# big-nacho/patolette

Measured on AMD Instinct MI355X. Metric: Mpixels/sec quantized (256-color ICtCp + KMeans) at 1 GPU; palette ΔE vs ref, higher is better.
Workload: dtype f64

## Files before the change

### patolette_amd/csrc/kmeans.h

```cpp
#pragma once

#include "common.h"
#include "devutil.h"

namespace pamd {

constexpr int kKMeansMaxK = 4096;

struct KmSamples { float *x, *y, *z, *w; };

struct KMeansWork {
    DevBuf<float> sx, sy, sz, sw;
    DevBuf<int> assign;
    DevBuf<float4> sorted;
    DevBuf<unsigned int> table, rowtot, ticket;
    DevBuf<unsigned int> flags;
    DevBuf<unsigned int> rowbase;
    DevBuf<float> hs;
    DevBuf<float> cent, hassign;
    DevBuf<float4> c4;
    DevBuf<int> perm;
    DevBuf<struct DevMT> mt;
    bool mt_seeded = false;
    DevBuf<unsigned char> lut, grid, clist;
    DevBuf<unsigned int> mid;
    DevBuf<unsigned int> bkeys;
    DevBuf<unsigned long long> fsum;
    void reserve(size_t nx, int k);
};

void kmeans_gather(const double *d_planar, size_t N, bool weighted, const int *d_perm, size_t nx, KMeansWork &w, hipStream_t s);
void kmeans_gather_slice(const double *d_planar, size_t n_local, bool weighted, const int *d_perm, size_t nx, size_t begin,
                         KMeansWork &w, hipStream_t s);
struct KmSums { double bound_x, bound_w; };
void kmeans_iterate(KMeansWork &w, size_t nx, int k, bool weighted, int niter, hipStream_t s, size_t expect_longest = 0,
                    const KmSums *sums = nullptr);

}
```

### patolette_amd/csrc/kmeans.hip

```cpp
#include "kmeans.h"

namespace pamd {

typedef __attribute__((address_space(1))) const void gvoid_t;
typedef __attribute__((address_space(3))) void lvoid_t;

template <bool W>
__global__ __launch_bounds__(256) void k_km_gather(const double *__restrict__ planar, size_t N, const int *__restrict__ perm,
                                                   size_t nx, KmSamples s) {
    const size_t stride = (size_t)gridDim.x * blockDim.x;
    for (size_t i = (size_t)blockIdx.x * blockDim.x + threadIdx.x; i < nx; i += stride) {
        size_t p = perm ? (size_t)perm[i] : i;
        s.x[i] = (float)planar[p]; s.y[i] = (float)planar[N + p]; s.z[i] = (float)planar[2 * N + p];
        if constexpr (W) s.w[i] = (float)planar[3 * N + p];
    }
}

template <bool W>
__global__ __launch_bounds__(256) void k_km_gather_slice(const double *__restrict__ planar, size_t n_local, const int *__restrict__ perm,
                                                         size_t nx, size_t begin, KmSamples s) {
    const size_t stride = (size_t)gridDim.x * blockDim.x;
    for (size_t i = (size_t)blockIdx.x * blockDim.x + threadIdx.x; i < nx; i += stride) {
        const size_t g = perm ? (size_t)perm[i] : i;
        const bool mine = g >= begin && g - begin < n_local;
        const size_t p = mine ? g - begin : 0;
        s.x[i] = mine ? (float)planar[p] : 0.0f; s.y[i] = mine ? (float)planar[n_local + p] : 0.0f;
        s.z[i] = mine ? (float)planar[2 * n_local + p] : 0.0f;
        if constexpr (W) s.w[i] = mine ? (float)planar[3 * n_local + p] : 0.0f;
    }
}

__device__ __forceinline__ float4 make_c4(float v0, float v1, float v2) {
    return make_float4(v0, v1, v2, __builtin_fmaf(v2, v2, __builtin_fmaf(v0, v0, v1 * v1)));
}

__device__ __forceinline__ void km_store_c4(float4 *c4, const int k, const int j, const float v0, const float v1, const float v2) {
    const float4 r = make_c4(v0, v1, v2);
    float *q = reinterpret_cast<float *>(c4 + j);
    __hip_atomic_store(q, r.x, __ATOMIC_RELAXED, __HIP_MEMORY_SCOPE_AGENT);
    __hip_atomic_store(q + 1, r.y, __ATOMIC_RELAXED, __HIP_MEMORY_SCOPE_AGENT);
    __hip_atomic_store(q + 2, r.z, __ATOMIC_RELAXED, __HIP_MEMORY_SCOPE_AGENT);
    __hip_atomic_store(q + 3, r.w, __ATOMIC_RELAXED, __HIP_MEMORY_SCOPE_AGENT);
    float *pp = reinterpret_cast<float *>(c4 + k) + 8 * (j >> 1) + (j & 1);
    __hip_atomic_store(pp, r.x, __ATOMIC_RELAXED, __HIP_MEMORY_SCOPE_AGENT);
    __hip_atomic_store(pp + 2, r.y, __ATOMIC_RELAXED, __HIP_MEMORY_SCOPE_AGENT);
    __hip_atomic_store(pp + 4, r.z, __ATOMIC_RELAXED, __HIP_MEMORY_SCOPE_AGENT);
    __hip_atomic_store(pp + 6, r.w, __ATOMIC_RELAXED, __HIP_MEMORY_SCOPE_AGENT);
}
constexpr int kKmFlagWords = 2 + 256;
__global__ void k_km_prep(const float *__restrict__ cent, int k, float4 *c4, unsigned int *flags) {
    int j = blockIdx.x * blockDim.x + threadIdx.x;
    if (j < k) km_store_c4(c4, k, j, cent[3 * j], cent[3 * j + 1], cent[3 * j + 2]);
    if (flags && j < kKmFlagWords) flags[j] = j == 0 ? 0u : 1u;
}

typedef float f4_t __attribute__((ext_vector_type(4)));
typedef const __attribute__((address_space(4))) f4_t *scalar_c4_t;

template <typename TabT>
__device__ __forceinline__ int km_assign_one(const float x0, const float x1, const float x2, const TabT c4, const int k) {
    const float m0 = -2 * x0, m1 = -2 * x1, m2 = -2 * x2;
    const float xn = __builtin_fmaf(x2, x2, __builtin_fmaf(x0, x0, x1 * x1));
    float ld[8]; unsigned li[8];
    int lb[8];
#pragma unroll
    for (int l = 0; l < 8; l++) { ld[l] = 3.402823466e+38F - xn; lb[l] = -l; }
    const int ny_p = (k / 8) * 8;
    for (int j = 0; j < ny_p; j += 8) {
#pragma unroll
        for (int l = 0; l < 8; l++) {
            const auto y = c4[j + l];
            float dp = m0 * y.x;
            dp = __builtin_fmaf(m1, y.y, dp);
            dp = __builtin_fmaf(m2, y.z, dp);
            dp = dp + y.w;
            if (dp < ld[l]) { ld[l] = dp; lb[l] = j; }
        }
    }
#pragma unroll
    for (int l = 0; l < 8; l++) li[l] = (unsigned)(lb[l] + l);
    float cur_d = 3.402823466e+38F; unsigned cur_i = 0xFFFFFFFFu;
#pragma unroll
    for (int l = 0; l < 8; l++) {
        float cand = ld[l] + xn;
        if (cand < 0) cand = 0;
        if (cur_d > cand) { cur_d = cand; cur_i = li[l]; }
        else if (cur_d == cand && cur_i > li[l]) cur_i = li[l];
    }
    for (int j0 = ny_p; j0 < k; j0++) {
        const auto y = c4[j0];
        float dp = __builtin_fmaf(x2, y.z, __builtin_fmaf(x1, y.y, x0 * y.x));
        float d = xn + y.w - 2 * dp;
        if (d < 0) d = 0;
        if (cur_d > d) { cur_d = d; cur_i = (unsigned)j0; }
    }
    return (int)cur_i;
}

__device__ __forceinline__ unsigned long long match_mask(int key, int nbits, unsigned long long valid) {
    unsigned long long m = valid;
    for (int b = 0; b < nbits; b++) {
        const bool bit = (key >> b) & 1;
        unsigned long long bm = __ballot(bit);
        m &= bit ? bm : ~bm;
    }
    return m;
}

template <bool BIG>
__global__ __launch_bounds__(256) void k_km_assign_count(KmSamples s, size_t nx, const float4 *__restrict__ c4, int k, int nbits,
                                                         int chunk_len, int nchunks, int *__restrict__ assign,
                                                         unsigned int *table ) {
    extern __shared__ unsigned int lds_u[];
    const int lane = threadIdx.x & 63, wid = threadIdx.x >> 6;
    unsigned int *cnt = lds_u + 4 * (size_t)k + (size_t)wid * k;
    if constexpr (!BIG) {
        for (int j = lane; j < k; j += 64) cnt[j] = 0u;
        __syncthreads();
    }
    const int chunk = blockIdx.x * 4 + wid;
    if (chunk >= nchunks) return;
    const size_t lo = (size_t)chunk * chunk_len;
    const size_t hi = lo + chunk_len < nx ? lo + chunk_len : nx;
    for (size_t base = lo; base < hi; base += 64) {
        const size_t i = base + lane;
        const bool v = i < hi;
        int a = 0;
        if (v) { a = km_assign_one(s.x[i], s.y[i], s.z[i], (scalar_c4_t)(unsigned long long)c4, k); assign[i] = a; }
        const unsigned long long valid = __ballot(v);
        const unsigned long long m = match_mask(a, nbits, valid);
        if (v && (m & ((1ULL << lane) - 1ULL)) == 0ULL) {
            if constexpr (BIG) (void)atomicAdd(&table[(size_t)a * nchunks + chunk], (unsigned)__popcll(m));
            else cnt[a] += (unsigned)__popcll(m);
        }
    }
    if constexpr (!BIG) for (int j = lane; j < k; j += 64) table[(size_t)j * nchunks + chunk] = cnt[j];
}

__global__ __launch_bounds__(256) void k_km_rowbase(const unsigned int *__restrict__ rowtot, int k, unsigned int *rowbase) {
    __shared__ unsigned int wsum[4];
    const int lane = threadIdx.x & 63, wid = threadIdx.x >> 6;
    const int per = (k + 255) / 256;
    const int j0 = threadIdx.x * per, j1 = (j0 + per < k) ? j0 + per : k;
    unsigned sum = 0;
    for (int j = j0; j < j1; j++) sum += rowtot[j];
    unsigned inc = sum;
#pragma unroll
    for (int o = 1; o < 64; o <<= 1) { unsigned t = __shfl_up(inc, o, 64); if (lane >= o) inc += t; }
    if (lane == 63) wsum[wid] = inc;
    __syncthreads();
    unsigned pre = 0;
    for (int w = 0; w < wid; w++) pre += wsum[w];
    unsigned run = pre + inc - sum;
    for (int j = j0; j < j1; j++) { rowbase[j] = run; run += rowtot[j]; }
}

template <bool W>
__global__ __launch_bounds__(256) void k_km_scatter_big(KmSamples s, const int *__restrict__ assign, size_t nx, int nbits, int chunk_len,
                                                        int nchunks, unsigned int *table, const unsigned int *__restrict__ rowbase,
                                                        float4 *sorted) {
    const int lane = threadIdx.x & 63, wid = threadIdx.x >> 6;
    const int chunk = blockIdx.x * 4 + wid;
    if (chunk >= nchunks) return;
    const size_t lo = (size_t)chunk * chunk_len;
    const size_t hi = lo + chunk_len < nx ? lo + chunk_len : nx;
    const unsigned long long lt = (1ULL << lane) - 1ULL;
    for (size_t base = lo; base < hi; base += 64) {
        const size_t i = base + lane;
        const bool v = i < hi;
        const int a = v ? assign[i] : 0;
        const unsigned long long valid = __ballot(v);
        const unsigned long long m = match_mask(a, nbits, valid);
        const unsigned r = (unsigned)__popcll(m & lt);
        unsigned cur = 0;
        if (v && r == 0) cur = atomicAdd(&table[(size_t)a * nchunks + chunk], (unsigned)__popcll(m));
        const int leader = (v && m) ? __ffsll((long long)m) - 1 : lane;
        cur = (unsigned)__shfl((int)cur, leader, 64);
        if (v) {
            float w = 1.0f;
            if constexpr (W) w = s.w[i];
            sorted[(size_t)rowbase[a] + cur + r] = make_float4(s.x[i], s.y[i], s.z[i], w);
        }
    }
}

__global__ __launch_bounds__(256) void k_km_rowscan(unsigned int *table, int nchunks, unsigned int *rowtot) {
    constexpr int IT = 16;
    __shared__ unsigned int sw[4];
    __shared__ unsigned int carry;
    unsigned int *row = table + (size_t)blockIdx.x * nchunks;
    if (threadIdx.x == 0) carry = 0u;
    __syncthreads();
    const int lane = threadIdx.x & 63, wid = threadIdx.x >> 6;
    for (int c0 = 0; c0 < nchunks; c0 += 256 * IT) {
        const int base = c0 + (int)threadIdx.x * IT;
        unsigned v[IT];
        if (base + IT <= nchunks && (((size_t)blockIdx.x * nchunks + base) & 3) == 0) {
#pragma unroll
            for (int q = 0; q < IT / 4; q++) {
                const uint4 u = *reinterpret_cast<const uint4 *>(row + base + 4 * q);
                v[4 * q] = u.x; v[4 * q + 1] = u.y; v[4 * q + 2] = u.z; v[4 * q + 3] = u.w;
            }
        } else {
#pragma unroll
            for (int q = 0; q < IT; q++) v[q] = base + q < nchunks ? row[base + q] : 0u;
        }
        unsigned tot = 0;
#pragma unroll
        for (int q = 0; q < IT; q++) { const unsigned x = v[q]; v[q] = tot; tot += x; }
        unsigned inc = tot;
#pragma unroll
        for (int o = 1; o < 64; o <<= 1) { unsigned t = __shfl_up(inc, o, 64); if (lane >= o) inc += t; }
        if (lane == 63) sw[wid] = inc;
        __syncthreads();
        unsigned pre = 0;
        for (int w = 0; w < wid; w++) pre += sw[w];
        const unsigned cr = carry;
        const unsigned off = cr + pre + inc - tot;
#pragma unroll
        for (int q = 0; q < IT; q++) if (base + q < nchunks) row[base + q] = off + v[q];
        __syncthreads();
        if (threadIdx.x == 255) carry = cr + pre + inc;
        __syncthreads();
    }
    if (threadIdx.x == 0) rowtot[blockIdx.x] = carry;
}

struct KmGridDev { float lo[3], hi[3]; };

__device__ __forceinline__ unsigned f32_key(float f) {
    const unsigned u = __float_as_uint(f);
    return (u & 0x80000000u) ? ~u : (u | 0x80000000u);
}
__device__ __forceinline__ float key_f32(unsigned k) { return __uint_as_float((k & 0x80000000u) ? (k & 0x7fffffffu) : ~k); }

constexpr int kKmSlots = 32;
__global__ __launch_bounds__(256) void k_km_bounds(KmSamples s, size_t nx, unsigned int *keys ) {
    float mn[3] = {INFINITY, INFINITY, INFINITY}, mx[3] = {-INFINITY, -INFINITY, -INFINITY};
    const size_t stride = (size_t)gridDim.x * blockDim.x;
    for (size_t i = (size_t)blockIdx.x * blockDim.x + threadIdx.x; i < nx; i += stride) {
        const float v[3] = {s.x[i], s.y[i], s.z[i]};
#pragma unroll
        for (int a = 0; a < 3; a++) { mn[a] = fminf(mn[a], v[a]); mx[a] = fmaxf(mx[a], v[a]); }
    }
#pragma unroll
    for (int a = 0; a < 3; a++) {
        float lo = mn[a], hi = mx[a];
#pragma unroll
        for (int o = 32; o > 0; o >>= 1) { lo = fminf(lo, __shfl_down(lo, o, 64)); hi = fmaxf(hi, __shfl_down(hi, o, 64)); }
        if ((threadIdx.x & 63) == 0 && lo <= hi) {
            unsigned int *k6 = keys + (blockIdx.x & (kKmSlots - 1)) * 6;
            atomicMin(&k6[a], f32_key(lo)); atomicMax(&k6[3 + a], f32_key(hi));
        }
    }
}
__global__ void k_km_bounds_init(unsigned int *keys) {
    const int t = threadIdx.x;
    if (t < kKmSlots * 6) keys[t] = (t % 6) < 3 ? 0xFFFFFFFFu : 0u;
}
__global__ void k_km_bounds_fold(const unsigned int *keys, KmGridDev *g) {
    const int a = threadIdx.x;
    if (a >= 3) return;
    unsigned lo = 0xFFFFFFFFu, hi = 0u;
    for (int sl = 0; sl < kKmSlots; sl++) { lo = min(lo, keys[sl * 6 + a]); hi = max(hi, keys[sl * 6 + 3 + a]); }
    g->lo[a] = key_f32(lo); g->hi[a] = key_f32(hi);
}

__device__ __forceinline__ int km_cell(float x0, float x1, float x2, const KmGridDev &g, int G) {
    int idx[3];
    const float v[3] = {x0, x1, x2};
#pragma unroll
    for (int a = 0; a < 3; a++) {
        const double r = (double)g.hi[a] - (double)g.lo[a];
        const double inv = r > 0 ? (double)G / r : 0.0;
        int q = (int)(((double)v[a] - (double)g.lo[a]) * inv);
        idx[a] = q < 0 ? 0 : (q >= G ? G - 1 : q);
    }
    return (idx[2] * G + idx[1]) * G + idx[0];
}

struct KmBox { double cl[3], ch[3], cellnorm2; };
__device__ __forceinline__ KmBox km_box(const KmGridDev &g, int G, const int idx[3], int span) {
    KmBox b; b.cellnorm2 = 0;
#pragma unroll
    for (int a = 0; a < 3; a++) {
        const double r = (double)g.hi[a] - (double)g.lo[a], cw = r / G, m = 1e-5 * r + 1e-30;
        b.cl[a] = (double)g.lo[a] + idx[a] * cw - m;
        b.ch[a] = (double)g.lo[a] + (idx[a] + span) * cw + m;
        const double f = fmax(fabs(b.cl[a]), fabs(b.ch[a]));
        b.cellnorm2 += f * f;
    }
    return b;
}
__device__ __forceinline__ double km_maxd2(const KmBox &b, const float4 y) {
    const double p[3] = {(double)y.x, (double)y.y, (double)y.z};
    double mx = 0;
#pragma unroll
    for (int a = 0; a < 3; a++) { const double d = fmax(fabs(p[a] - b.cl[a]), fabs(p[a] - b.ch[a])); mx += d * d; }
    return mx;
}
__device__ __forceinline__ double km_mind2(const KmBox &b, const float4 y) {
    const double p[3] = {(double)y.x, (double)y.y, (double)y.z};
    double mn = 0;
#pragma unroll
    for (int a = 0; a < 3; a++) { const double d = fmax(fmax(b.cl[a] - p[a], p[a] - b.ch[a]), 0.0); mn += d * d; }
    return mn;
}
__device__ __forceinline__ double km_threshold(const KmBox &b, double U, double cn2) {
    const double rr = sqrt(b.cellnorm2) + sqrt(cn2);
    return U * (1.0 + 1e-12) + 4.0 * (16.0 * 0x1.0p-24) * rr * rr + 1e-300;
}

constexpr int kKmCoarseMax = 96;
__global__ __launch_bounds__(64) void k_km_lut_coarse(const float4 *__restrict__ c4, int k, const KmGridDev *__restrict__ gp, int G,
                                                      unsigned char *__restrict__ clist ,
                                                      double *__restrict__ cn2_out ) {
    const KmGridDev g = *gp;
    const int Gc = G / 4, cell = (int)blockIdx.x, lane = (int)threadIdx.x;
    const int idx[3] = {4 * (cell % Gc), 4 * ((cell / Gc) % Gc), 4 * (cell / (Gc * Gc))};
    const KmBox b = km_box(g, G, idx, 4);
    double U = INFINITY, cn2 = 0;
    for (int j = lane; j < k; j += 64) {
        const float4 y = c4[j];
        U = fmin(U, km_maxd2(b, y));
        cn2 = fmax(cn2, ((double)y.x * y.x + (double)y.y * y.y) + (double)y.z * y.z);
    }
#pragma unroll
    for (int o = 32; o > 0; o >>= 1) { U = fmin(U, __shfl_xor(U, o, 64)); cn2 = fmax(cn2, __shfl_xor(cn2, o, 64)); }
    const double thr = km_threshold(b, U, cn2);
    if (lane == 0) *cn2_out = cn2;
    unsigned char *out = clist + (size_t)cell * (2 + kKmCoarseMax);
    int cnt = 0;
    const int ny_p = (k / 8) * 8;
    auto sweep = [&](int j, bool valid) {
        const bool keep = valid && km_mind2(b, c4[valid ? j : 0]) <= thr;
        const unsigned long long m = __ballot(keep);
        const int pos = cnt + (int)__popcll(m & ((1ULL << lane) - 1ULL));
        if (keep && pos < kKmCoarseMax) out[2 + pos] = (unsigned char)j;
        cnt += (int)__popcll(m);
    };
    for (int l = 0; l < 8; l++)
        for (int q0 = 0; l + 8 * q0 < ny_p; q0 += 64) { const int j = l + 8 * (q0 + lane); sweep(j, j < ny_p); }
    for (int j0 = ny_p; j0 < k; j0 += 64) sweep(j0 + lane, j0 + lane < k);
    if (lane == 0) { out[0] = (unsigned char)(cnt <= kKmCoarseMax ? cnt : 0); out[1] = (unsigned char)(cnt <= kKmCoarseMax ? 0 : 1); }
}

constexpr int kKmMidSurv = 48;
constexpr unsigned kKmMidOverflow = 0x00000001u;
__device__ __forceinline__ bool km_mid_is_overflow(unsigned e) { return e == kKmMidOverflow; }

__device__ __forceinline__ void km_mid_entries(const float4 *__restrict__ c4, const int k, const KmGridDev &g, const int G,
                                               const unsigned char *__restrict__ cand, const double cn2, const int c0, const int c1, const int c2,
                                               unsigned int *__restrict__ mid) {
    const int lane = (int)threadIdx.x, m = lane >> 3, sl = lane & 7;
    const int midx[3] = {2 * c0 + (m & 1), 2 * c1 + ((m >> 1) & 1), 2 * c2 + (m >> 2)};
    const int idx[3] = {2 * midx[0], 2 * midx[1], 2 * midx[2]};
// ... 931 lines not shown
            for (int q = 0; 4 * q < cnt; q++) {
                const float4 x = s4[q];
                float4 w = make_float4(0, 0, 0, 0);
                if (wx) w = w4[q];
                const float xs[4] = {x.x, x.y, x.z, x.w}, ws[4] = {w.x, w.y, w.z, w.w};
#pragma unroll
                for (int e = 0; e < 4; e++) {
                    if (4 * q + e < cnt) {
                        if (wx) acc = __builtin_fmaf(xs[e], ws[e], acc);
                        else acc += xs[e];
                    }
                }
            }
        }
    }
}
__device__ __forceinline__ void km_block_step(const float *blk, const float *wblk, const bool wx, const unsigned len, float &acc, const int lane) {
    if (km_block_exact(blk, wblk, wx, 0, 4, acc, lane)) return;
    if (len == 1024u) {
        for (int q = 0; q < 4; q++)
            if (!km_block_exact(blk, wblk, wx, q, 1, acc, lane)) km_block_replay(blk, wblk, wx, (unsigned)q * 256u, (unsigned)(q + 1) * 256u, acc);
        return;
    }
    km_block_replay(blk, wblk, wx, 0u, len, acc);
}

template <bool W>
__device__ __forceinline__ float km_chain_coop(const float4 *__restrict__ sorted, size_t lo, size_t hi, float *coop, int lane, int wid) {
    constexpr int K = 16;
    constexpr size_t BS = (size_t)64 * K, SS = 4 * BS;
    const bool wx = W && wid < 3;
    const bool chain = W || wid < 3;
    const float *mine = coop + (size_t)wid * SS, *wts = coop + 3 * SS;
    float acc = 0.f;
    float4 reg[K];
    auto fetch = [&](const size_t p0) {
#pragma unroll
        for (int j = 0; j < K; j++) {
            const size_t i = p0 + (size_t)wid * BS + (size_t)j * 64 + lane;
            reg[j] = make_float4(0, 0, 0, 0);
            if (i < hi) reg[j] = sorted[i];
        }
    };
    fetch(lo);
    for (size_t p0 = lo; p0 < hi; p0 += SS) {
#pragma unroll
        for (int j = 0; j < K; j++) {
            const int o = wid * (int)BS + j * 64 + lane;
            coop[o] = reg[j].x; coop[SS + o] = reg[j].y; coop[2 * SS + o] = reg[j].z; coop[3 * SS + o] = reg[j].w;
        }
        if (p0 + SS < hi) fetch(p0 + SS);
        __syncthreads();
        if (chain) {
            for (int d = 0; d < 4; d++) {
                const size_t pos = p0 + (size_t)d * BS;
                if (pos >= hi) break;
                const size_t bend = pos + BS < hi ? pos + BS : hi;
                const float *blk = mine + d * (int)BS, *wblk = wts + d * (int)BS;
                km_block_step(blk, wblk, wx, (unsigned)(bend - pos), acc, lane);
            }
        }
        __syncthreads();
    }
    return acc;
}

template <bool W>
__device__ __forceinline__ float km_coop_lds(const float *mine, const float *wts, const unsigned n, const bool wx, float acc, const int lane) {
    constexpr unsigned BS = 1024;
    for (unsigned pos = 0; pos < n; pos += BS)
        km_block_step(mine + pos, wts + pos, wx, pos + BS < n ? BS : n - pos, acc, lane);
    return acc;
}

template <bool W, int HS>
__device__ __forceinline__ void km_update_finish(const int kidx, const int k, const unsigned long long nx, const size_t cnt, const float *res,
                                                 int *s_last, float *cent, float *hassign, float4 *c4, unsigned int *ticket, DevMT *mt,
                                                 float *hs_mem = nullptr, unsigned int *flags = nullptr, const bool clean = false) {
    const int lane = threadIdx.x & 63, wid = threadIdx.x >> 6;
    float c0 = res[0], c1 = res[1], c2 = res[2], h = res[3];
    if constexpr (!W) {
        h = cnt < (size_t)16777216 ? (float)cnt : 16777216.0f;
    }
    if (threadIdx.x == 0) {
        if (!clean) {
        if (h != 0.f) { const float norm = 1 / h; c0 *= norm; c1 *= norm; c2 *= norm; }
        __hip_atomic_store(&cent[3 * kidx], c0, __ATOMIC_RELAXED, __HIP_MEMORY_SCOPE_AGENT);
        __hip_atomic_store(&cent[3 * kidx + 1], c1, __ATOMIC_RELAXED, __HIP_MEMORY_SCOPE_AGENT);
        __hip_atomic_store(&cent[3 * kidx + 2], c2, __ATOMIC_RELAXED, __HIP_MEMORY_SCOPE_AGENT);
        __hip_atomic_store(&hassign[kidx], h, __ATOMIC_RELAXED, __HIP_MEMORY_SCOPE_AGENT);
        km_store_c4(c4, k, kidx, c0, c1, c2);
        }
        asm volatile("s_waitcnt vmcnt(0)" ::: "memory");
        const unsigned tk = __hip_atomic_fetch_add(ticket, 1u, __ATOMIC_RELAXED, __HIP_MEMORY_SCOPE_AGENT);
        *s_last = (tk == (unsigned)k - 1u) ? 1 : 0;
    }
    __syncthreads();
    if (!*s_last || wid != 0) return;
    bool mine_empty = false, mine_dirty = false;
    for (int cb = 0; cb < k; cb += 256) {
        float hv[4]; unsigned fv[4];
#pragma unroll
        for (int q = 0; q < 4; q++) {
            const int ci = cb + 64 * q + lane;
            hv[q] = 1.f; fv[q] = 0u;
            if (ci < k) {
                hv[q] = __hip_atomic_load(&hassign[ci], __ATOMIC_RELAXED, __HIP_MEMORY_SCOPE_AGENT);
                if (flags) fv[q] = __hip_atomic_load(&flags[1 + ci], __ATOMIC_RELAXED, __HIP_MEMORY_SCOPE_AGENT);
            }
        }
#pragma unroll
        for (int q = 0; q < 4; q++) {
            const int ci = cb + 64 * q + lane;
            mine_empty = mine_empty || hv[q] == 0.f;
            mine_dirty = mine_dirty || fv[q] != 0u;
            if (flags && ci < k) __hip_atomic_store(&flags[1 + ci], 0u, __ATOMIC_RELAXED, __HIP_MEMORY_SCOPE_AGENT);
        }
    }
    const bool any = __ballot(mine_empty) != 0ULL;
    if (lane == 0) __hip_atomic_store(ticket, 0u, __ATOMIC_RELAXED, __HIP_MEMORY_SCOPE_AGENT);
    if (flags) {
        const bool any_dirty = __ballot(mine_dirty) != 0ULL;
        if (!any_dirty && !any && lane == 0) __hip_atomic_store(&flags[0], 1u, __ATOMIC_RELAXED, __HIP_MEMORY_SCOPE_AGENT);
    }
    if (!any) return;
    {
        asm volatile("s_waitcnt vmcnt(0)" ::: "memory");
        __shared__ unsigned s_mt[624];
        __builtin_amdgcn_fence(__ATOMIC_ACQUIRE, "agent");
        if constexpr (HS > 0) {
            __shared__ float s_hs[HS];
            km_split_clusters_wave<false>(cent, hassign, k, nx, mt, s_mt, s_hs, lane, flags);
        } else km_split_clusters_wave<true>(cent, hassign, k, nx, mt, s_mt, hs_mem, lane);
        __builtin_amdgcn_fence(__ATOMIC_RELEASE, "agent");
        asm volatile("s_waitcnt vmcnt(0)" ::: "memory");
    }
    for (int j = lane; j < k; j += 64) {
        const float v0 = __hip_atomic_load(&cent[3 * j], __ATOMIC_RELAXED, __HIP_MEMORY_SCOPE_AGENT);
        const float v1 = __hip_atomic_load(&cent[3 * j + 1], __ATOMIC_RELAXED, __HIP_MEMORY_SCOPE_AGENT);
        const float v2 = __hip_atomic_load(&cent[3 * j + 2], __ATOMIC_RELAXED, __HIP_MEMORY_SCOPE_AGENT);
        km_store_c4(c4, k, j, v0, v1, v2);
    }
}

template <bool W, bool BIGK = false>
__global__ __launch_bounds__(256) void k_km_update(const float4 *__restrict__ sorted, const unsigned int *__restrict__ rowtot, int k,
                                                  unsigned long long nx, float *cent, float *hassign, float4 *c4,
                                                  unsigned int *ticket, DevMT *mt, unsigned long long long_min, float *hs_mem) {
    __shared__ float4 stage[4][2][64];
    extern __shared__ __attribute__((aligned(16))) float coop[];
    __shared__ float res[4];
    __shared__ int s_last;
    const int kidx = blockIdx.x, lane = threadIdx.x & 63, wid = threadIdx.x >> 6;
    unsigned pre = 0;
    for (int j = lane; j < kidx; j += 64) pre += rowtot[j];
    pre = wave_sum_u32(pre);
    pre = __shfl(pre, 0, 64);
    const size_t lo = pre, hi = lo + rowtot[kidx];
    float acc = 0.f;
    if ((size_t)(hi - lo) >= long_min) {
        acc = km_chain_coop<W>(sorted, lo, hi, coop, lane, wid);
    } else {
        if (wid == 0) acc = km_chain<W, 0>(sorted, lo, hi, stage[0], lane);
        else if (wid == 1) acc = km_chain<W, 1>(sorted, lo, hi, stage[1], lane);
        else if (wid == 2) acc = km_chain<W, 2>(sorted, lo, hi, stage[2], lane);
        else if (W) acc = km_chain<W, 3>(sorted, lo, hi, stage[3], lane);
    }
    if (lane == 0) res[wid] = acc;
    __syncthreads();
    km_update_finish<W, BIGK ? 0 : kKMeansMaxK>(kidx, k, nx, hi - lo, res, &s_last, cent, hassign, c4, ticket, mt, hs_mem);
}

constexpr int kKmDirectCap = 4096;
constexpr int kKmSortBlock = 1024;

__device__ __forceinline__ unsigned block_scan_incl_u32(const unsigned v, unsigned *wsum, unsigned *total) {
    const int lane = threadIdx.x & 63, wid = threadIdx.x >> 6, nw = (int)(blockDim.x >> 6);
    const unsigned inc = wave_scan_incl_u32(v);
    __syncthreads();
    if (lane == 63) wsum[wid] = inc;
    __syncthreads();
    unsigned pre = 0, all = 0;
    for (int w = 0; w < nw; w++) { const unsigned t = wsum[w]; all += t; pre += w < wid ? t : 0u; }
    *total = all;
    return pre + inc;
}

typedef float f2_t __attribute__((ext_vector_type(2)));
typedef float f8_t __attribute__((ext_vector_type(8)));
typedef const __attribute__((address_space(4))) f8_t *scalar_c8_t;

__device__ __forceinline__ float km_min3(const float a, const float b, const float c) {
    float r;
    asm("v_min3_f32 %0, %1, %2, %3" : "=v"(r) : "v"(a), "v"(b), "v"(c));
    return r;
}
__device__ __forceinline__ int km_assign_min3(const float x0, const float x1, const float x2, const scalar_c4_t c4,
                                              const scalar_c8_t c8, const float4 *c4s, const int k) {
    const f2_t m0 = {-2 * x0, -2 * x0}, m1 = {-2 * x1, -2 * x1}, m2 = {-2 * x2, -2 * x2};
    const float xn = __builtin_fmaf(x2, x2, __builtin_fmaf(x0, x0, x1 * x1));
    float ld[8]; int lc[8];
#pragma unroll
    for (int l = 0; l < 8; l++) { ld[l] = 3.402823466e+38F - xn; lc[l] = -1; }
    const int ny_p = (k / 8) * 8;
    const int U = ny_p >> 4;
    const int CUN = (U + 3) >> 2;
    auto pair_dp = [&](const f8_t y) {
        const f2_t y0 = {y[0], y[1]}, y1 = {y[2], y[3]}, y2 = {y[4], y[5]}, yw = {y[6], y[7]};
        f2_t dp = m0 * y0;
        dp = __builtin_elementwise_fma(m1, y1, dp);
        dp = __builtin_elementwise_fma(m2, y2, dp);
        return dp + yw;
    };
    for (int c = 0; c < 4; c++) {
        const int u0 = c * CUN, u1 = u0 + CUN < U ? u0 + CUN : U;
        if (u0 >= u1) break;
        float snap[8];
#pragma unroll
        for (int l = 0; l < 8; l++) snap[l] = ld[l];
        for (int u = u0; u < u1; u++) {
            const int p0 = u << 3;
            typedef float f16_t __attribute__((ext_vector_type(16)));
            typedef const __attribute__((address_space(4))) f16_t *scalar_c16_t;
            const scalar_c16_t c16 = (scalar_c16_t)c8;
            const f16_t q0 = c16[p0 >> 1], q1 = c16[(p0 >> 1) + 1], q2 = c16[(p0 >> 1) + 2], q3 = c16[(p0 >> 1) + 3];
            auto half = [](const f16_t q, const int h) { return h ? f8_t{q[8], q[9], q[10], q[11], q[12], q[13], q[14], q[15]} : f8_t{q[0], q[1], q[2], q[3], q[4], q[5], q[6], q[7]}; };
#pragma unroll
            for (int l = 0; l < 8; l += 2) {
                const f8_t ya = half(l < 4 ? q0 : q1, (l >> 1) & 1), yb = half(l < 4 ? q2 : q3, (l >> 1) & 1);
                const f2_t a = pair_dp(ya), b = pair_dp(yb);
                ld[l] = km_min3(ld[l], a[0], b[0]);
                ld[l + 1] = km_min3(ld[l + 1], a[1], b[1]);
            }
        }
#pragma unroll
        for (int l = 0; l < 8; l++) lc[l] = ld[l] < snap[l] ? c : lc[l];
    }
    if (ny_p & 8) {
        const int p0 = U << 3;
#pragma unroll
        for (int l = 0; l < 8; l += 2) {
            const f2_t a = pair_dp(c8[p0 + (l >> 1)]);
            if (a[0] < ld[l]) { ld[l] = a[0]; lc[l] = 4; }
            if (a[1] < ld[l + 1]) { ld[l + 1] = a[1]; lc[l + 1] = 4; }
        }
    }
    float cand[8];
    float cur_d = 3.402823466e+38F;
#pragma unroll
    for (int l = 0; l < 8; l++) { float cd = ld[l] + xn; if (cd < 0) cd = 0; cand[l] = cd; cur_d = cd < cur_d ? cd : cur_d; }
    unsigned tm = 0u;
#pragma unroll
    for (int l = 0; l < 8; l++) tm |= cand[l] == cur_d ? (1u << l) : 0u;
    unsigned cur_i = 0xFFFFFFFFu;
    while (__any(tm != 0u)) {
        if (tm) {
            const int l = __ffs((int)tm) - 1;
            tm &= tm - 1u;
            float target = ld[0]; int c = lc[0];
#pragma unroll
            for (int q = 1; q < 8; q++) { target = l == q ? ld[q] : target; c = l == q ? lc[q] : c; }
            unsigned idx = 0u;
            if (c == 4) idx = (unsigned)((U << 4) + l);
            else if (c >= 0) {
                const int u0 = c * CUN, u1 = u0 + CUN < U ? u0 + CUN : U;
                const int base = (u0 << 4) + l, lim = u1 << 4;
                for (int q = 2 * CUN - 1; q >= 0; q--) {
                    const int j = base + 8 * q;
                    if (j < lim) {
                        const float4 y = c4s[j];
                        float dp = (-2 * x0) * y.x;
                        dp = __builtin_fmaf(-2 * x1, y.y, dp);
                        dp = __builtin_fmaf(-2 * x2, y.z, dp);
                        dp = dp + y.w;
                        if (dp == target) idx = (unsigned)j;
                    }
                }
            }
            cur_i = idx < cur_i ? idx : cur_i;
        }
    }
    for (int j0 = ny_p; j0 < k; j0++) {
        const auto y = c4[j0];
        float dp = __builtin_fmaf(x2, y.z, __builtin_fmaf(x1, y.y, x0 * y.x));
        float d = xn + y.w - 2 * dp;
        if (d < 0) d = 0;
        if (cur_d > d) { cur_d = d; cur_i = (unsigned)j0; }
    }
    return cur_i < (unsigned)k ? (int)cur_i : 0;
}

#ifdef PAMD_KM_TRACE
__device__ unsigned long long g_km_trace[2][256][32];
#define KM_TRACE(kern, slot) do { if ((threadIdx.x & 63) == 0) g_km_trace[kern][blockIdx.x & 255][slot] = wall_clock64(); } while (0)
#define KM_TRACE0(kern, slot) do { if (threadIdx.x == 0) g_km_trace[kern][blockIdx.x & 255][slot] = wall_clock64(); } while (0)
#else
#define KM_TRACE(kern, slot) do { } while (0)
#define KM_TRACE0(kern, slot) do { } while (0)
#endif

__global__ __launch_bounds__(1024) void k_km_assign_sort(KmSamples s, size_t nx, const float4 *__restrict__ c4, int k, const bool weighted,
                                                         float4 *__restrict__ sorted_rec, unsigned short *__restrict__ offs,
                                                         unsigned char *__restrict__ prev, unsigned int *flags) {
    if (flags[0]) return;
    __shared__ unsigned char cnt[16][256];
    __shared__ unsigned short stepbase[16][256];
    __shared__ unsigned int wsum[16];
    __shared__ float4 c4s[256];
    const int lane = threadIdx.x & 63, step = threadIdx.x >> 6;
    KM_TRACE0(0, 0);
    for (int i = threadIdx.x; i < 16 * 256 / 4; i += 1024) reinterpret_cast<unsigned int *>(&cnt[0][0])[i] = 0u;
    if ((int)threadIdx.x < k) c4s[threadIdx.x] = c4[threadIdx.x];
    __syncthreads();
    KM_TRACE0(0, 1);
    const scalar_c4_t t4 = (scalar_c4_t)(unsigned long long)c4;
    const scalar_c8_t t8 = (scalar_c8_t)(unsigned long long)(c4 + k);
    const size_t blk0 = (size_t)blockIdx.x * kKmSortBlock;
    const size_t i = blk0 + (size_t)step * 64 + lane;
    const bool v = i < nx;
    float4 rec = make_float4(0.f, 0.f, 0.f, 0.f);
    if (v) { rec.x = s.x[i]; rec.y = s.y[i]; rec.z = s.z[i]; if (weighted) rec.w = s.w[i]; }
#ifdef PAMD_KM_TRACE
    asm volatile("s_waitcnt vmcnt(0)" ::: "memory");
    KM_TRACE0(0, 2);
    if (threadIdx.x == 0) g_km_trace[0][blockIdx.x & 255][24] = clock64();
#endif
    int a = km_assign_min3(rec.x, rec.y, rec.z, t4, t8, c4s, k);
    if (!v) a = 0;
    if (v) {
        const int old = prev[i];
        if (old != a) { prev[i] = (unsigned char)a; flags[1 + old] = 1u; flags[1 + a] = 1u; }
    }
    const unsigned long long m = match_mask(a, 8, __ballot(v));
    const unsigned rk = (unsigned)__popcll(m & ((1ULL << lane) - 1ULL));
    if (v && rk == 0u) cnt[step][a] = (unsigned char)__popcll(m);
#ifdef PAMD_KM_TRACE
    if (lane == 0) g_km_trace[0][blockIdx.x & 255][8 + step] = wall_clock64();
    if (threadIdx.x == 0) g_km_trace[0][blockIdx.x & 255][25] = clock64();
#endif
    __syncthreads();
    KM_TRACE0(0, 3);
    unsigned tot = 0;
    unsigned short pre[16];
    if (threadIdx.x < 256) {
#pragma unroll
        for (int st = 0; st < 16; st++) { pre[st] = (unsigned short)tot; tot += cnt[st][threadIdx.x]; }
    }
    unsigned total = 0;
    const unsigned start = block_scan_incl_u32(tot, wsum, &total) - tot;
    if (threadIdx.x < 256) {
#pragma unroll
        for (int st = 0; st < 16; st++) stepbase[st][threadIdx.x] = (unsigned short)(start + pre[st]);
        unsigned short *ob = offs + (size_t)blockIdx.x * 257;
        ob[threadIdx.x] = (unsigned short)start;
        if (threadIdx.x == 255) ob[256] = (unsigned short)total;
    }
    __syncthreads();
    KM_TRACE0(0, 4);
    if (v) sorted_rec[blk0 + (unsigned)stepbase[step][a] + rk] = rec;
#ifdef PAMD_KM_TRACE
    asm volatile("s_waitcnt vmcnt(0)" ::: "memory");
    KM_TRACE0(0, 5);
#endif
}

template <bool W>
__global__ __launch_bounds__(256) void k_km_update_lists(const float4 *__restrict__ sorted_rec, const unsigned short *__restrict__ offs,
                                                        unsigned long long nx, int k, float *cent, float *hassign, float4 *c4,
                                                        unsigned int *ticket, DevMT *mt, unsigned int *flags) {
    if (flags[0]) return;
    __shared__ float4 stage[4][2][64];
    extern __shared__ __attribute__((aligned(16))) float members[];
    __shared__ float res[4];
    __shared__ int s_last;
    __shared__ unsigned int wsum[16];
    __shared__ unsigned int n_long, long_src[256], long_lo[256], long_nb[256];
    const int kidx = blockIdx.x, lane = threadIdx.x & 63, wid = threadIdx.x >> 6;
    float *const mx = members, *const my = members + kKmDirectCap, *const mz = members + 2 * kKmDirectCap, *const mw = members + 3 * kKmDirectCap;
    unsigned int *const srcidx = reinterpret_cast<unsigned int *>(members + 4 * kKmDirectCap);
    float acc = 0.f;
    size_t total = 0;
    unsigned fill = 0;
    KM_TRACE0(1, 0);
    bool long_list = false;
    auto replay = [&]() {
        const unsigned n = fill;
        if (n == (unsigned)kKmDirectCap || long_list) {
            const unsigned padded = (n + 1023u) & ~1023u;
            for (unsigned i = n + threadIdx.x; i < padded; i += 256) { mx[i] = 0.f; my[i] = 0.f; mz[i] = 0.f; mw[i] = 0.f; }
            __syncthreads();
            if ((W || wid < 3) && n) acc = km_coop_lds<W>(members + (size_t)wid * kKmDirectCap, mw, n, W && wid < 3, acc, lane);
            long_list = true;
            return;
        }
        auto rec = [&](const size_t i) { return make_float4(mx[i], my[i], mz[i], mw[i]); };
        if (wid == 0) acc = km_chain_over<W, 0>(rec, n, stage[0], lane, acc);
        else if (wid == 1) acc = km_chain_over<W, 1>(rec, n, stage[1], lane, acc);
        else if (wid == 2) acc = km_chain_over<W, 2>(rec, n, stage[2], lane, acc);
        else if (W) acc = km_chain_over<W, 3>(rec, n, stage[3], lane, acc);
    };
    const bool clean = flags[1 + kidx] == 0u;
    const unsigned long long nblocks = clean ? 0ULL : (nx + kKmSortBlock - 1) / kKmSortBlock;
    for (unsigned long long c0 = 0; c0 < nblocks; c0 += 256) {
        const unsigned long long b = c0 + threadIdx.x;
        unsigned o0 = 0, nb = 0;
        if (b < nblocks) { o0 = offs[b * 257 + kidx]; nb = (unsigned)offs[b * 257 + kidx + 1] - o0; }
        unsigned chunk_total = 0;
        const unsigned excl = block_scan_incl_u32(nb, wsum, &chunk_total) - nb;
        constexpr unsigned kLongRun = 32;
        const bool is_long = nb > kLongRun;
        if (threadIdx.x == 0) n_long = 0u;
        __syncthreads();
        if (is_long) { const unsigned e = atomicAdd(&n_long, 1u); long_src[e] = (unsigned)(b * kKmSortBlock) + o0; long_lo[e] = excl; long_nb[e] = nb; }
        __syncthreads();
        const unsigned nl = n_long;
        unsigned done = 0;
        while (done < chunk_total) {
            const unsigned take = min((unsigned)kKmDirectCap - fill, chunk_total - done);
            if (!is_long) {
                const unsigned lo = max(excl, done), hi = min(excl + nb, done + take);
                const float4 *src = sorted_rec + b * kKmSortBlock + o0;
                for (unsigned q = lo; q < hi; q += 4) {
                    float4 r4[4];
#pragma unroll
                    for (int u = 0; u < 4; u++) r4[u] = q + u < hi ? src[q + u - excl] : make_float4(0.f, 0.f, 0.f, 0.f);
#pragma unroll
                    for (int u = 0; u < 4; u++) if (q + u < hi) { const unsigned i = fill + q + u - done; mx[i] = r4[u].x; my[i] = r4[u].y; mz[i] = r4[u].z; mw[i] = r4[u].w; }
                }
            }
            if (nl) {
                for (unsigned i = threadIdx.x; i < take; i += 256) srcidx[fill + i] = ~0u;
                __syncthreads();
                for (unsigned e = 0; e < nl; e++) {
                    const unsigned ex0 = long_lo[e], lo = max(ex0, done), hi = min(ex0 + long_nb[e], done + take);
                    for (unsigned q = lo + threadIdx.x; q < hi; q += 256) srcidx[fill + q - done] = long_src[e] + (q - ex0);
                }
                __syncthreads();
                for (unsigned i0 = threadIdx.x; i0 < take; i0 += 256 * 8) {
                    unsigned ix[8]; float4 r[8];
#pragma unroll
                    for (int u = 0; u < 8; u++) { const unsigned i = i0 + 256u * u; ix[u] = i < take ? srcidx[fill + i] : ~0u; }
#pragma unroll
                    for (int u = 0; u < 8; u++) r[u] = ix[u] != ~0u ? sorted_rec[ix[u]] : make_float4(0.f, 0.f, 0.f, 0.f);
#pragma unroll
                    for (int u = 0; u < 8; u++) if (ix[u] != ~0u) { const unsigned i = fill + i0 + 256u * u; mx[i] = r[u].x; my[i] = r[u].y; mz[i] = r[u].z; mw[i] = r[u].w; }
                }
            }
            fill += take; done += take;
            __syncthreads();
            if (fill == (unsigned)kKmDirectCap) { replay(); fill = 0; __syncthreads(); }
        }
        total += chunk_total;
    }
    __syncthreads();
    KM_TRACE0(1, 1);
    replay();
#ifdef PAMD_KM_TRACE
    if (lane == 0) g_km_trace[1][blockIdx.x & 255][8 + wid] = wall_clock64();
#endif
    if (lane == 0) res[wid] = acc;
    __syncthreads();
    KM_TRACE0(1, 2);
    km_update_finish<W, 256>(kidx, k, nx, total, res, &s_last, cent, hassign, c4, ticket, mt, nullptr, flags, clean);
    KM_TRACE0(1, 3);
}

struct KmFix { double magic_x, quantum_x, magic_w, quantum_w; };
__device__ __forceinline__ long long km_fix_quant(const double v, const double magic) {
    return __double_as_longlong(v + magic) - __double_as_longlong(magic);
}
template <bool W, typename AT>
__global__ __launch_bounds__(256) void k_km_accum(KmSamples s, const AT *__restrict__ assign, size_t nx, int k, KmFix f,
                                                  unsigned long long *gsum ) {
    extern __shared__ unsigned long long acc64[];
    for (int i = threadIdx.x; i < 4 * k; i += 256) acc64[i] = 0ULL;
    __syncthreads();
    auto add = [&](const unsigned a, const float x, const float y, const float z, const float w) {
        const double wd = W ? (double)w : 1.0;
        unsigned long long *r = acc64 + 4 * (size_t)a;
        atomicAdd(r, (unsigned long long)km_fix_quant((double)x * wd, f.magic_x));
        atomicAdd(r + 1, (unsigned long long)km_fix_quant((double)y * wd, f.magic_x));
        atomicAdd(r + 2, (unsigned long long)km_fix_quant((double)z * wd, f.magic_x));
        atomicAdd(r + 3, W ? (unsigned long long)km_fix_quant(wd, f.magic_w) : 1ULL);
    };
    const size_t stride = (size_t)gridDim.x * 1024;
    for (size_t base = ((size_t)blockIdx.x * 256 + threadIdx.x) * 4; base < nx; base += stride) {
        if (base + 4 <= nx) {
            const float4 vx = *reinterpret_cast<const float4 *>(s.x + base), vy = *reinterpret_cast<const float4 *>(s.y + base),
                         vz = *reinterpret_cast<const float4 *>(s.z + base);
            float4 vw = make_float4(1.f, 1.f, 1.f, 1.f);
            if constexpr (W) vw = *reinterpret_cast<const float4 *>(s.w + base);
            unsigned a0, a1, a2, a3;
            if constexpr (sizeof(AT) == 1) {
                const unsigned pk = *reinterpret_cast<const unsigned int *>(assign + base);
                a0 = pk & 0xffu; a1 = (pk >> 8) & 0xffu; a2 = (pk >> 16) & 0xffu; a3 = pk >> 24;
            } else {
                const int4 pk = *reinterpret_cast<const int4 *>(assign + base);
                a0 = (unsigned)pk.x; a1 = (unsigned)pk.y; a2 = (unsigned)pk.z; a3 = (unsigned)pk.w;
            }
            add(a0, vx.x, vy.x, vz.x, vw.x); add(a1, vx.y, vy.y, vz.y, vw.y);
            add(a2, vx.z, vy.z, vz.z, vw.z); add(a3, vx.w, vy.w, vz.w, vw.w);
        } else {
            for (size_t i = base; i < nx; i++) add((unsigned)assign[i], s.x[i], s.y[i], s.z[i], W ? s.w[i] : 1.f);
        }
    }
    __syncthreads();
    for (int i = threadIdx.x; i < 4 * k; i += 256) { const unsigned long long v = acc64[i]; if (v) atomicAdd(&gsum[i], v); }
}

template <bool W>
__global__ __launch_bounds__(256) void k_km_update_sums(unsigned long long *gsum, int k, unsigned long long nx, KmFix f, float *cent,
                                                        float *hassign, float4 *c4, DevMT *mt) {
    __shared__ int s_empty;
    if (threadIdx.x == 0) s_empty = 0;
    __syncthreads();
    for (int j = threadIdx.x; j < k; j += 256) {
        const double sx = (double)(long long)gsum[4 * j] * f.quantum_x, sy = (double)(long long)gsum[4 * j + 1] * f.quantum_x,
                     sz = (double)(long long)gsum[4 * j + 2] * f.quantum_x;
        float h;
        if constexpr (W) h = (float)((double)(long long)gsum[4 * j + 3] * f.quantum_w);
        else h = (float)gsum[4 * j + 3];
        float c0 = (float)sx, c1 = (float)sy, c2 = (float)sz;
        if (h != 0.f) { const float norm = 1 / h; c0 *= norm; c1 *= norm; c2 *= norm; }
        else s_empty = 1;
        cent[3 * j] = c0; cent[3 * j + 1] = c1; cent[3 * j + 2] = c2; hassign[j] = h;
        gsum[4 * j] = 0ULL; gsum[4 * j + 1] = 0ULL; gsum[4 * j + 2] = 0ULL; gsum[4 * j + 3] = 0ULL;
    }
    __threadfence();
    __syncthreads();
    if (s_empty && threadIdx.x < 64) {
        __shared__ unsigned s_mt[624];
        __shared__ float s_hs[kKMeansMaxK];
        km_split_clusters_wave(cent, hassign, k, nx, mt, s_mt, s_hs, (int)threadIdx.x);
        __threadfence();
    }
    __syncthreads();
    for (int j = threadIdx.x; j < k; j += 256) km_store_c4(c4, k, j, cent[3 * j], cent[3 * j + 1], cent[3 * j + 2]);
}

static int chunk_len_for(size_t nx) {
    size_t c = ceil_div(nx, 4096);
    c = ceil_div(c, 64) * 64;
    if (c < 64) c = 64;
    return (int)c;
}

void KMeansWork::reserve(size_t nx, int k) {
    sx.reserve(nx); sy.reserve(nx); sz.reserve(nx); sw.reserve(nx);
    assign.reserve(nx); sorted.reserve(nx);
    const int nchunks = (int)ceil_div(nx, (size_t)chunk_len_for(nx));
    table.reserve(std::max((size_t)k * (size_t)(nchunks > 0 ? nchunks : 1),
                           (ceil_div(nx, (size_t)1024) * 257 + 1) / 2 + 1));
    rowtot.reserve(k);
    if (k > kKMeansMaxK) { rowbase.reserve(k); hs.reserve(k); }
    cent.reserve(3 * (size_t)k); hassign.reserve(k); c4.reserve(2 * (size_t)k + 2);
    perm.reserve(nx);
    if (!mt.p) { mt.reserve(1); mt_seeded = false; }
    if (!ticket.p) { ticket.reserve(1); HIP_CHECK(hipMemset(ticket.p, 0, sizeof(unsigned int))); }
    flags.reserve(2 + 256);
}

void kmeans_gather(const double *d_planar, size_t N, bool weighted, const int *d_perm, size_t nx, KMeansWork &w, hipStream_t s) {
    KmSamples ks{w.sx.p, w.sy.p, w.sz.p, w.sw.p};
    size_t g = ceil_div(nx, 256);
    if (g > 4096) g = 4096;
    if (g < 1) g = 1;
    KTIME("k_km_gather", s, (weighted ? 48.0 : 36.0) * nx);
    if (weighted) hipLaunchKernelGGL(k_km_gather<true>, (int)g, 256, 0, s, d_planar, N, d_perm, nx, ks);
    else hipLaunchKernelGGL(k_km_gather<false>, (int)g, 256, 0, s, d_planar, N, d_perm, nx, ks);
    HIP_CHECK(hipGetLastError());
}

void kmeans_gather_slice(const double *d_planar, size_t n_local, bool weighted, const int *d_perm, size_t nx, size_t begin,
                         KMeansWork &w, hipStream_t s) {
    KmSamples ks{w.sx.p, w.sy.p, w.sz.p, w.sw.p};
    size_t g = ceil_div(nx, 256);
    if (g > 4096) g = 4096;
    if (g < 1) g = 1;
    KTIME("k_km_gather", s, (weighted ? 48.0 : 36.0) * nx);
    if (weighted) hipLaunchKernelGGL(k_km_gather_slice<true>, (int)g, 256, 0, s, d_planar, n_local, d_perm, nx, begin, ks);
    else hipLaunchKernelGGL(k_km_gather_slice<false>, (int)g, 256, 0, s, d_planar, n_local, d_perm, nx, begin, ks);
    HIP_CHECK(hipGetLastError());
}

void kmeans_iterate(KMeansWork &w, size_t nx, int k, bool weighted, int niter, hipStream_t s, size_t expect_longest, const KmSums *sums) {
    KmSamples ks{w.sx.p, w.sy.p, w.sz.p, w.sw.p};
    KmFix fix{};
    int ablocks = 1;
    if (sums && k > kKMeansMaxK) sums = nullptr;
    if (sums) {
        int ex = 0, ew = 0, P = 1;
        (void)frexp(std::max(sums->bound_x, 1e-300) * (weighted ? std::max(sums->bound_w, 1e-300) : 1.0), &ex);
        (void)frexp(std::max(sums->bound_w, 1e-300), &ew);
        while (((size_t)1 << P) < nx) P++;
        P = std::max(P + 1, 12);
        fix.quantum_x = ldexp(1.0, ex + P - 62); fix.magic_x = ldexp(1.5, 52 + ex + P - 62);
        fix.quantum_w = ldexp(1.0, ew + P - 62); fix.magic_w = ldexp(1.5, 52 + ew + P - 62);
        w.fsum.reserve(4 * (size_t)k);
        HIP_CHECK(hipMemsetAsync(w.fsum.p, 0, 4 * (size_t)k * sizeof(unsigned long long), s));
        ablocks = (int)std::min<size_t>(std::max<size_t>(ceil_div(nx, (size_t)4096), 1), 2048);
        static PerDeviceOnce attr5;
        attr5.once([&] {
            HIP_CHECK(hipFuncSetAttribute((const void *)k_km_accum<true, int>, hipFuncAttributeMaxDynamicSharedMemorySize, 32 * kKMeansMaxK));
            HIP_CHECK(hipFuncSetAttribute((const void *)k_km_accum<false, int>, hipFuncAttributeMaxDynamicSharedMemorySize, 32 * kKMeansMaxK));
            HIP_CHECK(hipFuncSetAttribute((const void *)k_km_accum<true, unsigned char>, hipFuncAttributeMaxDynamicSharedMemorySize, 32 * kKMeansMaxK));
            HIP_CHECK(hipFuncSetAttribute((const void *)k_km_accum<false, unsigned char>, hipFuncAttributeMaxDynamicSharedMemorySize, 32 * kKMeansMaxK));
        });
    }
    auto update_sums = [&](const bool a8) {
        {
            KTIME("k_km_accum", s, ((weighted ? 16.0 : 12.0) + (a8 ? 1.0 : 4.0)) * nx);
            const size_t lds = (size_t)32 * k;
            if (a8) {
                if (weighted) hipLaunchKernelGGL((k_km_accum<true, unsigned char>), ablocks, 256, lds, s, ks, (const unsigned char *)w.assign.p, nx, k, fix, w.fsum.p);
                else hipLaunchKernelGGL((k_km_accum<false, unsigned char>), ablocks, 256, lds, s, ks, (const unsigned char *)w.assign.p, nx, k, fix, w.fsum.p);
            } else {
                if (weighted) hipLaunchKernelGGL((k_km_accum<true, int>), ablocks, 256, lds, s, ks, (const int *)w.assign.p, nx, k, fix, w.fsum.p);
                else hipLaunchKernelGGL((k_km_accum<false, int>), ablocks, 256, lds, s, ks, (const int *)w.assign.p, nx, k, fix, w.fsum.p);
            }
        }
        KTIME("k_km_update", s, 32.0 * k);
        if (weighted) hipLaunchKernelGGL(k_km_update_sums<true>, 1, 256, 0, s, w.fsum.p, k, (unsigned long long)nx, fix, w.cent.p, w.hassign.p, w.c4.p, w.mt.p);
        else hipLaunchKernelGGL(k_km_update_sums<false>, 1, 256, 0, s, w.fsum.p, k, (unsigned long long)nx, fix, w.cent.p, w.hassign.p, w.c4.p, w.mt.p);
    };
    int nbits = 0;
    while ((1 << nbits) < k) nbits++;
    const int chunk_len = chunk_len_for(nx);
    const int nchunks = (int)ceil_div(nx, (size_t)chunk_len);
    const int cblocks = (nchunks + 3) / 4;
    const bool bigk = k > kKMeansMaxK;
    const size_t lds_cnt = bigk ? 0 : (size_t)8 * k * sizeof(unsigned int);
    const size_t lds_sct = (size_t)5 * k * sizeof(unsigned int);
    const size_t lds_sct_pair = (size_t)9 * k * sizeof(unsigned int) + (size_t)4 * (k + 64) * sizeof(float4);
    static PerDeviceOnce attr;
    attr.once([&] {
        HIP_CHECK(hipFuncSetAttribute((const void *)k_km_assign_count<false>, hipFuncAttributeMaxDynamicSharedMemorySize, 8 * kKMeansMaxK * 4));
        HIP_CHECK(hipFuncSetAttribute((const void *)k_km_scatter<true, int>, hipFuncAttributeMaxDynamicSharedMemorySize, 5 * kKMeansMaxK * 4));
        HIP_CHECK(hipFuncSetAttribute((const void *)k_km_scatter<false, int>, hipFuncAttributeMaxDynamicSharedMemorySize, 5 * kKMeansMaxK * 4));
        HIP_CHECK(hipFuncSetAttribute((const void *)k_km_scatter<true, unsigned char>, hipFuncAttributeMaxDynamicSharedMemorySize, 5 * kKMeansMaxK * 4));
        HIP_CHECK(hipFuncSetAttribute((const void *)k_km_scatter<false, unsigned char>, hipFuncAttributeMaxDynamicSharedMemorySize, 5 * kKMeansMaxK * 4));
        HIP_CHECK(hipFuncSetAttribute((const void *)k_km_update<true, false>, hipFuncAttributeMaxDynamicSharedMemorySize, 4 * 4096 * 4));
        HIP_CHECK(hipFuncSetAttribute((const void *)k_km_update<false, false>, hipFuncAttributeMaxDynamicSharedMemorySize, 4 * 4096 * 4));
    });
    if (!w.mt_seeded) { hipLaunchKernelGGL(k_km_mt_seed, 1, 1, 0, s, w.mt.p); w.mt_seeded = true; }
    { KTIME("k_km_prep", s, 28.0 * k); hipLaunchKernelGGL(k_km_prep, (std::max(k, kKmFlagWords) + 255) / 256, 256, 0, s, w.cent.p, k, w.c4.p, w.flags.p); }
    const size_t lut_min = getenv("PAMD_KM_LUT_MIN") ? (size_t)atoll(getenv("PAMD_KM_LUT_MIN")) : ((size_t)1 << 21);
    const bool use_lut = nx >= lut_min && k >= 16 && k <= 256;
    const size_t g64_min = getenv("PAMD_KM_G64_MIN") ? (size_t)atoll(getenv("PAMD_KM_G64_MIN")) : ((size_t)1 << 23);
    const int G = nx >= g64_min ? 64 : 32;
    if (use_lut) {
        static PerDeviceOnce attr2;
        attr2.once([&] {
            HIP_CHECK(hipFuncSetAttribute((const void *)k_km_assign_lut, hipFuncAttributeMaxDynamicSharedMemorySize, 8 * kKMeansMaxK * 4));
        });
        w.lut.reserve((size_t)G * G * G * 16); w.bkeys.reserve(kKmSlots * 6); w.grid.reserve(64 + sizeof(double));
        w.clist.reserve((size_t)(G * G * G / 64) * (2 + kKmCoarseMax));
        hipLaunchKernelGGL(k_km_bounds_init, 1, 256, 0, s, w.bkeys.p);
        { KTIME("k_km_bounds", s, 12.0 * nx); hipLaunchKernelGGL(k_km_bounds, (int)std::min<size_t>(ceil_div(nx, 256), 2048), 256, 0, s, ks, nx, w.bkeys.p); }
        hipLaunchKernelGGL(k_km_bounds_fold, 1, 64, 0, s, w.bkeys.p, (KmGridDev *)w.grid.p);
    }
    constexpr size_t direct_max = (size_t)1 << 19;
    const size_t list_longest = getenv("PAMD_KM_LIST_LONGEST") ? (size_t)atoll(getenv("PAMD_KM_LIST_LONGEST")) : (size_t)16384;
    const bool use_direct = !sums && !use_lut && k <= 256 && nx <= direct_max && nx < ((size_t)1 << 32) && expect_longest < list_longest;
    if (use_direct) {
        HIP_CHECK(hipMemsetAsync(w.assign.p, 0, nx, s));
        static PerDeviceOnce attr4;
        attr4.once([&] {
            HIP_CHECK(hipFuncSetAttribute((const void *)k_km_update_lists<true>, hipFuncAttributeMaxDynamicSharedMemorySize, kKmDirectCap * 20));
            HIP_CHECK(hipFuncSetAttribute((const void *)k_km_update_lists<false>, hipFuncAttributeMaxDynamicSharedMemorySize, kKmDirectCap * 20));
        });
    }
    const bool use_mid = use_lut && G == 64 && k % 8 == 0;
    if (use_mid) w.mid.reserve(32 * 32 * 32);
    const unsigned long long long_min = getenv("PAMD_KM_LONG_MIN") ? (unsigned long long)atoll(getenv("PAMD_KM_LONG_MIN")) : 8192ULL;
    for (int it = 0; it < niter; it++) {
        if (use_direct) {
            unsigned short *offs = (unsigned short *)w.table.p;
            const int sblocks = (int)ceil_div(nx, (size_t)kKmSortBlock);
            {
                KTIME("k_km_assign", s, (weighted ? 32.0 : 28.0) * nx);
                hipLaunchKernelGGL(k_km_assign_sort, sblocks, 1024, 0, s, ks, nx, w.c4.p, k, weighted, w.sorted.p, offs, (unsigned char *)w.assign.p, w.flags.p);
            }
            {
                KTIME("k_km_update", s, 16.0 * nx);
                if (weighted) hipLaunchKernelGGL(k_km_update_lists<true>, k, 256, kKmDirectCap * 20, s, (const float4 *)w.sorted.p, (const unsigned short *)offs,
                                                 (unsigned long long)nx, k, w.cent.p, w.hassign.p, w.c4.p, w.ticket.p, w.mt.p, w.flags.p);
                else hipLaunchKernelGGL(k_km_update_lists<false>, k, 256, kKmDirectCap * 20, s, (const float4 *)w.sorted.p, (const unsigned short *)offs,
                                        (unsigned long long)nx, k, w.cent.p, w.hassign.p, w.c4.p, w.ticket.p, w.mt.p, w.flags.p);
            }
            continue;
        }
        if (use_lut) {
            {
                KTIME("k_km_lut_build", s, 16.0 * G * G * G);
                const int ncoarse = G * G * G / 64;
                double *cn2 = (double *)(w.grid.p + 64);
                hipLaunchKernelGGL(k_km_lut_coarse, ncoarse, 64, 0, s, w.c4.p, k, (const KmGridDev *)w.grid.p, G, w.clist.p, cn2);
                hipLaunchKernelGGL(k_km_lut_build, ncoarse, 64, 0, s, w.c4.p, k, (const KmGridDev *)w.grid.p, G, (const unsigned char *)w.clist.p,
                                   (const double *)cn2, w.lut.p, use_mid ? w.mid.p : (unsigned int *)nullptr);
            }
            if (use_mid) {
                const int nmid = 32 * 32 * 32;
                const size_t lds_mid = ((size_t)nmid + 4 * 256 + 16 * 256) * 4 + (size_t)16 * kKmQueue * 16;
                static PerDeviceOnce attr3;
                attr3.once([&] {
                    HIP_CHECK(hipFuncSetAttribute((const void *)k_km_assign_mid, hipFuncAttributeMaxDynamicSharedMemorySize, (int)lds_mid));
                });
                const int mblocks = std::min(num_cus(), (nchunks + 15) / 16);
                KTIME("k_km_assign", s, 16.0 * nx);
                hipLaunchKernelGGL(k_km_assign_mid, mblocks, 1024, lds_mid, s, ks, nx, w.c4.p, k, chunk_len, nchunks, (unsigned char *)w.assign.p, w.table.p,
                                   (const KmGridDev *)w.grid.p, (const unsigned int *)w.mid.p, (const unsigned char *)w.lut.p);
            } else {
            KTIME("k_km_assign", s, 16.0 * nx);
            hipLaunchKernelGGL(k_km_assign_lut, cblocks, 256, lds_cnt, s, ks, nx, w.c4.p, k, nbits, chunk_len, nchunks, w.assign.p, w.table.p,
                               (const KmGridDev *)w.grid.p, G, w.lut.p);
            }
        } else {
            KTIME("k_km_assign", s, 16.0 * nx);
            if (bigk) {
                HIP_CHECK(hipMemsetAsync(w.table.p, 0, (size_t)k * nchunks * sizeof(unsigned int), s));
                hipLaunchKernelGGL(k_km_assign_count<true>, cblocks, 256, 0, s, ks, nx, w.c4.p, k, nbits, chunk_len, nchunks, w.assign.p, w.table.p);
            } else hipLaunchKernelGGL(k_km_assign_count<false>, cblocks, 256, lds_cnt, s, ks, nx, w.c4.p, k, nbits, chunk_len, nchunks, w.assign.p, w.table.p);
        }
        if (sums) { update_sums(use_lut && use_mid); continue; }
        if (bigk) {
            { KTIME("k_km_rowscan", s, 8.0 * k * nchunks); hipLaunchKernelGGL(k_km_rowscan, k, 256, 0, s, w.table.p, nchunks, w.rowtot.p); }
            hipLaunchKernelGGL(k_km_rowbase, 1, 256, 0, s, (const unsigned int *)w.rowtot.p, k, w.rowbase.p);
            {
                KTIME("k_km_scatter", s, (weighted ? 36.0 : 32.0) * nx);
                if (weighted) hipLaunchKernelGGL(k_km_scatter_big<true>, cblocks, 256, 0, s, ks, (const int *)w.assign.p, nx, nbits, chunk_len, nchunks, w.table.p, (const unsigned int *)w.rowbase.p, w.sorted.p);
                else hipLaunchKernelGGL(k_km_scatter_big<false>, cblocks, 256, 0, s, ks, (const int *)w.assign.p, nx, nbits, chunk_len, nchunks, w.table.p, (const unsigned int *)w.rowbase.p, w.sorted.p);
            }
            {
                KTIME("k_km_update", s, 16.0 * nx);
                const bool coop_on = nx >= long_min;
                const size_t lds_up = coop_on ? (size_t)4 * 4096 * sizeof(float) : 0;
                const unsigned long long lm = coop_on ? long_min : ~0ULL;
                static PerDeviceOnce attr6;
                attr6.once([&] {
                    HIP_CHECK(hipFuncSetAttribute((const void *)k_km_update<true, true>, hipFuncAttributeMaxDynamicSharedMemorySize, 4 * 4096 * 4));
                    HIP_CHECK(hipFuncSetAttribute((const void *)k_km_update<false, true>, hipFuncAttributeMaxDynamicSharedMemorySize, 4 * 4096 * 4));
                });
                if (weighted) hipLaunchKernelGGL((k_km_update<true, true>), k, 256, lds_up, s, w.sorted.p, w.rowtot.p, k, (unsigned long long)nx, w.cent.p, w.hassign.p, w.c4.p, w.ticket.p, w.mt.p, lm, w.hs.p);
                else hipLaunchKernelGGL((k_km_update<false, true>), k, 256, lds_up, s, w.sorted.p, w.rowtot.p, k, (unsigned long long)nx, w.cent.p, w.hassign.p, w.c4.p, w.ticket.p, w.mt.p, lm, w.hs.p);
            }
            continue;
        }
        { KTIME("k_km_rowscan", s, 8.0 * k * nchunks); hipLaunchKernelGGL(k_km_rowscan, k, 256, 0, s, w.table.p, nchunks, w.rowtot.p); }
        {
            KTIME("k_km_scatter", s, (weighted ? 36.0 : 32.0) * nx - (use_mid ? 3.0 : 0.0) * nx);
            const unsigned char *a8 = (const unsigned char *)w.assign.p;
            if (use_mid && chunk_len >= 4096 && k <= 256) {
                constexpr size_t lds_ls = (size_t)(512 + 1024 + 4096 / 4 + 4 * 4096) * sizeof(unsigned int);
                static PerDeviceOnce attr5;
                attr5.once([&] {
                    HIP_CHECK(hipFuncSetAttribute((const void *)k_km_scatter_lds<true>, hipFuncAttributeMaxDynamicSharedMemorySize, (int)lds_ls));
                    HIP_CHECK(hipFuncSetAttribute((const void *)k_km_scatter_lds<false>, hipFuncAttributeMaxDynamicSharedMemorySize, (int)lds_ls));
                });
                if (weighted) hipLaunchKernelGGL(k_km_scatter_lds<true>, nchunks, 256, lds_ls, s, ks, a8, nx, k, chunk_len, nchunks, w.table.p, w.rowtot.p, w.sorted.p);
                else hipLaunchKernelGGL(k_km_scatter_lds<false>, nchunks, 256, lds_ls, s, ks, a8, nx, k, chunk_len, nchunks, w.table.p, w.rowtot.p, w.sorted.p);
            } else if (use_mid && chunk_len >= 2 * k) {
                static PerDeviceOnce attr3;
                attr3.once([&] {
                    HIP_CHECK(hipFuncSetAttribute((const void *)k_km_scatter<true, unsigned char, true>, hipFuncAttributeMaxDynamicSharedMemorySize, 9 * 256 * 4 + 4 * (256 + 64) * 16));
                    HIP_CHECK(hipFuncSetAttribute((const void *)k_km_scatter<false, unsigned char, true>, hipFuncAttributeMaxDynamicSharedMemorySize, 9 * 256 * 4 + 4 * (256 + 64) * 16));
                });
                if (weighted) hipLaunchKernelGGL((k_km_scatter<true, unsigned char, true>), cblocks, 256, lds_sct_pair, s, ks, a8, nx, k, nbits, chunk_len, nchunks, w.table.p, w.rowtot.p, w.sorted.p);
                else hipLaunchKernelGGL((k_km_scatter<false, unsigned char, true>), cblocks, 256, lds_sct_pair, s, ks, a8, nx, k, nbits, chunk_len, nchunks, w.table.p, w.rowtot.p, w.sorted.p);
            } else if (use_mid) {
                if (weighted) hipLaunchKernelGGL((k_km_scatter<true, unsigned char>), cblocks, 256, lds_sct, s, ks, a8, nx, k, nbits, chunk_len, nchunks, w.table.p, w.rowtot.p, w.sorted.p);
                else hipLaunchKernelGGL((k_km_scatter<false, unsigned char>), cblocks, 256, lds_sct, s, ks, a8, nx, k, nbits, chunk_len, nchunks, w.table.p, w.rowtot.p, w.sorted.p);
            } else {
                if (weighted) hipLaunchKernelGGL((k_km_scatter<true, int>), cblocks, 256, lds_sct, s, ks, (const int *)w.assign.p, nx, k, nbits, chunk_len, nchunks, w.table.p, w.rowtot.p, w.sorted.p);
                else hipLaunchKernelGGL((k_km_scatter<false, int>), cblocks, 256, lds_sct, s, ks, (const int *)w.assign.p, nx, k, nbits, chunk_len, nchunks, w.table.p, w.rowtot.p, w.sorted.p);
            }
        }
        {
            KTIME("k_km_update", s, 16.0 * nx);
            const bool coop_on = nx >= long_min;
            const size_t lds_up = coop_on ? (size_t)4 * 4096 * sizeof(float) : 0;
            const unsigned long long lm = coop_on ? long_min : ~0ULL;
            if (weighted) hipLaunchKernelGGL((k_km_update<true, false>), k, 256, lds_up, s, w.sorted.p, w.rowtot.p, k, (unsigned long long)nx, w.cent.p, w.hassign.p, w.c4.p, w.ticket.p, w.mt.p, lm, (float *)nullptr);
            else hipLaunchKernelGGL((k_km_update<false, false>), k, 256, lds_up, s, w.sorted.p, w.rowtot.p, k, (unsigned long long)nx, w.cent.p, w.hassign.p, w.c4.p, w.ticket.p, w.mt.p, lm, (float *)nullptr);
        }
    }
    HIP_CHECK(hipGetLastError());
}

}

#ifdef PAMD_KM_TRACE
extern "C" int patolette_amd_debug_km_trace(unsigned long long *out) {
    return hipMemcpyFromSymbol(out, HIP_SYMBOL(pamd::g_km_trace), sizeof(pamd::g_km_trace)) == hipSuccess ? 0 : -1;
}
#endif
```

### patolette_amd/csrc/pipeline.hip

```cpp
#include <algorithm>
#include <functional>
#include <chrono>
#include <cmath>
#include <atomic>
#include <memory>
#include <mutex>
#include <thread>
#include <future>
#include <type_traits>

#include "color_device.h"
#include "common.h"
#include "host_math.h"
#include "kmeans.h"
#include "map.h"
#include "ordered.h"
#include "delta.h"
#include "measure.h"
#include "lzw.h"
#include "saliency.h"
#include "quant.h"
#include "rgba.h"
#include "compact.h"
#include "split_frontier.h"
#include "given.h"

namespace pamd {

void launch_convert(int which, const double *src, double *dst, size_t n, ConvertStats *stats, hipStream_t s, BinK sumk = BinK{0.0, 0.0},
                    BinK momk = BinK{0.0, 0.0}, size_t begin = 0, size_t end = ~(size_t)0, bool init_stats = true);
void launch_convert_rows(int which, const double *rows, double *dst, size_t n, ConvertStats *stats, hipStream_t s,
                         BinK sumk = BinK{0.0, 0.0}, BinK momk = BinK{0.0, 0.0}, size_t begin = 0, size_t end = ~(size_t)0,
                         bool init_stats = true);
void launch_convert_u8(int which, const unsigned char *pixels, int channels, double *dst, size_t n, ConvertStats *stats,
                       hipStream_t s, BinK sumk = BinK{0.0, 0.0}, BinK momk = BinK{0.0, 0.0}, size_t begin = 0, size_t end = ~(size_t)0,
                       bool init_stats = true);
void launch_reconstruct(const void *map, int map_elem, size_t n, const unsigned char *pal_u8, int k, unsigned char *out,
                        hipStream_t s);
void launch_weight_stats(const double *w, size_t n, ConvertStats *stats, hipStream_t s);
void launch_pow(const double *x, double y, double *out, size_t n, hipStream_t s);
void launch_fill_image(double *d, size_t n, uint64_t seed, hipStream_t s);
void launch_fill_weights(double *d, size_t n, uint64_t seed, hipStream_t s);

KernelTimer &ktimer() { static thread_local KernelTimer *t = new KernelTimer; return *t; }

std::atomic<int> g_debug_ws{getenv("PAMD_DEBUG_WORKSPACE") ? atoi(getenv("PAMD_DEBUG_WORKSPACE")) & (kWsPoison | kWsCount | kWsLog) : 0};
std::atomic<unsigned long long> g_late_growths{0};
WsStreams &ws_streams() { static thread_local WsStreams w; return w; }
void ws_growth(size_t bytes, const char *file, int line) {
    const int dbg = g_debug_ws.load(std::memory_order_relaxed);
    if (!(dbg & (kWsCount | kWsLog))) return;
    bool queued = false;
    for (const hipStream_t *sp : ws_streams().s)
        if (sp && *sp && hipStreamQuery(*sp) == hipErrorNotReady) queued = true;
    if (!queued) return;
    g_late_growths.fetch_add(1);
    if (dbg & kWsLog) fprintf(stderr, "patolette_amd: workspace growth to %zu bytes while work is queued (%s:%d)\n", bytes, file, line);
}
void ws_poison_dev(void *p, size_t bytes) {
    if (!bytes) return;
    HIP_CHECK(hipMemsetAsync(p, 0xFF, bytes, nullptr));
    HIP_CHECK(hipStreamSynchronize(nullptr));
}
void ws_poison_dev_rows(void *p, size_t pitch, size_t width, size_t rows) {
    if (!width || !rows) return;
    HIP_CHECK(hipMemset2DAsync(p, pitch, 0xFF, width, rows, nullptr));
    HIP_CHECK(hipStreamSynchronize(nullptr));
}
int KernelTimer::id_of(const char *name) {
    for (size_t i = 0; i < names.size(); i++) if (names[i] == name) return (int)i;
    names.emplace_back(name); total_ms.push_back(0); total_bytes.push_back(0); launches.push_back(0);
    return (int)names.size() - 1;
}
hipEvent_t KernelTimer::get_event() {
    if (!pool.empty()) { hipEvent_t e = pool.back(); pool.pop_back(); return e; }
    hipEvent_t e; HIP_CHECK(hipEventCreate(&e)); return e;
}
void KernelTimer::begin(int id, hipStream_t s, double bytes, const double *src) {
    Rec r; r.id = id; r.bytes = bytes; r.src = src; r.a = get_event(); r.b = get_event();
    HIP_CHECK(hipEventRecord(r.a, s));
    pending.push_back(r);
}
void KernelTimer::end(hipStream_t s) { HIP_CHECK(hipEventRecord(pending.back().b, s)); }
void KernelTimer::collect() {
    for (auto &r : pending) {
        float ms = 0;
        if (hipEventSynchronize(r.b) == hipSuccess && hipEventElapsedTime(&ms, r.a, r.b) == hipSuccess && !(r.src && *r.src == 0.0)) {
            total_ms[r.id] += ms; total_bytes[r.id] += r.src ? r.bytes * *r.src : r.bytes; launches[r.id] += 1;
        }
        pool.push_back(r.a); pool.push_back(r.b);
    }
    pending.clear();
}
void KernelTimer::reset() { collect(); names.clear(); total_ms.clear(); total_bytes.clear(); launches.clear(); }

__global__ __launch_bounds__(256) void k_gq_prepare(Tile *tA, int ntA, Tile *tP, int ntP, unsigned long long N, int *round_nodes, int *node_tile0,
                                                    double *hist, unsigned long long nhist, unsigned long long *hsize, unsigned int *hcount) {
    const unsigned long long stride = (unsigned long long)gridDim.x * blockDim.x, t0 = (unsigned long long)blockIdx.x * blockDim.x + threadIdx.x;
    for (unsigned long long i = t0; i < (unsigned long long)ntA; i += stride) {
        const unsigned long long o = i * (unsigned long long)kTileA;
        tA[i] = Tile{o, (unsigned)(N - o < (unsigned long long)kTileA ? N - o : (unsigned long long)kTileA), 0u};
    }
    for (unsigned long long i = t0; i < (unsigned long long)ntP; i += stride) {
        const unsigned long long o = i * (unsigned long long)kTileP;
        tP[i] = Tile{o, (unsigned)(N - o < (unsigned long long)kTileP ? N - o : (unsigned long long)kTileP), 0u};
    }
    for (unsigned long long i = t0; i < nhist; i += stride) hist[i] = 0.0;
    for (unsigned long long i = t0; i < (unsigned long long)kBuckets; i += stride) { hsize[i] = 0ULL; hcount[i] = 0u; }
    if (t0 == 0) { round_nodes[0] = 0; node_tile0[0] = 0; node_tile0[1] = ntP; }
}

__global__ void k_put_nodes(NodeDev *table, const NodeIn *stage, const int *ids, int n) {
    int i = blockIdx.x * blockDim.x + threadIdx.x;
    if (i >= n) return;
    const NodeIn in = stage[i];
    NodeDev &d = table[ids[i]];
    d.begin = in.begin; d.n = in.n; d.gn = in.gn; d.buf = in.buf; d.slot = in.slot; d.child0 = in.child0; d.nchild = in.nchild;
    for (int j = 0; j < 3; j++) { d.axis[j] = in.axis[j]; d.mean[j] = in.mean[j]; }
    d.sw = in.sw; d.klin = in.klin; d.kquad = in.kquad;
    node_reset_outputs(d);
    d.split = in.split; d.psplit = -1;
}
__global__ void k_put_node1(NodeDev *table, const int id, const NodeIn in) {
    NodeDev &d = table[id];
    d.begin = in.begin; d.n = in.n; d.gn = in.gn; d.buf = in.buf; d.slot = in.slot; d.child0 = in.child0; d.nchild = in.nchild;
    for (int j = 0; j < 3; j++) { d.axis[j] = in.axis[j]; d.mean[j] = in.mean[j]; }
    d.sw = in.sw; d.klin = in.klin; d.kquad = in.kquad;
    node_reset_outputs(d);
    d.split = in.split; d.psplit = -1;
}
__global__ void k_get_nodes(const NodeDev *table, NodeOut *stage, const int *ids, int n) {
    int i = blockIdx.x * blockDim.x + threadIdx.x;
    if (i >= n) return;
    const NodeDev &d = table[ids[i]];
    NodeOut o;
    o.begin = d.begin; o.n = d.n; o.gn = d.gn; o.buf = d.buf; o.degenerate = d.degenerate; o.split = d.split; o.psplit = d.psplit;
    o.sw = d.sw;
    for (int j = 0; j < 3; j++) o.mean[j] = d.mean[j];
    for (int q = 0; q < 7; q++) {
        double s0 = 0, s1 = 0;
        for (int k = 0; k < kSlots; k++) { s0 += d.acc[k][q][0]; s1 += d.acc[k][q][1]; }
        o.acc[q][0] = s0; o.acc[q][1] = s1;
    }
    stage[i] = o;
}

struct RoundSetup {
    const NodeIn *recs; const int *ids; const int *tA0; const int *tP0;
    int nr, ntA, ntP;
    Tile *tilesA, *tilesP;
    double *hist; size_t nhist;
    unsigned long long *hsize; unsigned int *hcount; size_t nbk;
};
__device__ __forceinline__ int node_of_tile(const int *t0, int nr, int t) {
    int lo = 0, hi = nr;
    while (hi - lo > 1) { const int mid = (lo + hi) >> 1; if (t0[mid] <= t) lo = mid; else hi = mid; }
    return lo;
}
__global__ __launch_bounds__(256) void k_round_setup(NodeDev *table, RoundSetup a) {
    const size_t tid = (size_t)blockIdx.x * blockDim.x + threadIdx.x, stride = (size_t)gridDim.x * blockDim.x;
    for (size_t i = tid; i < (size_t)a.nr; i += stride) {
        const NodeIn in = a.recs[i];
        NodeDev &d = table[a.ids[i]];
        d.begin = in.begin; d.n = in.n; d.gn = in.gn; d.buf = in.buf; d.slot = in.slot; d.child0 = in.child0; d.nchild = in.nchild;
        for (int j = 0; j < 3; j++) { d.axis[j] = in.axis[j]; d.mean[j] = in.mean[j]; }
        d.sw = in.sw; d.klin = in.klin; d.kquad = in.kquad;
    }
    for (size_t i = tid; i < (size_t)a.nr * kNodeResetElems; i += stride)
        node_reset_element(table[a.ids[i / kNodeResetElems]], (int)(i % kNodeResetElems));
    for (size_t t = tid; t < (size_t)a.ntA; t += stride) {
        const int r = node_of_tile(a.tA0, a.nr, (int)t);
        const unsigned long long o = (unsigned long long)((int)t - a.tA0[r]) * kTileA, n = a.recs[r].n;
        a.tilesA[t] = Tile{a.recs[r].begin + o, (unsigned)(n - o < (unsigned long long)kTileA ? n - o : kTileA), (unsigned)a.ids[r]};
    }
    for (size_t t = tid; t < (size_t)a.ntP; t += stride) {
        const int r = node_of_tile(a.tP0, a.nr, (int)t);
        const unsigned long long o = (unsigned long long)((int)t - a.tP0[r]) * kTileP, n = a.recs[r].n;
        a.tilesP[t] = Tile{a.recs[r].begin + o, (unsigned)(n - o < (unsigned long long)kTileP ? n - o : kTileP), (unsigned)a.ids[r]};
    }
    for (size_t i = tid; i < a.nhist; i += stride) a.hist[i] = 0.0;
    for (size_t i = tid; i < a.nbk; i += stride) { a.hsize[i] = 0ULL; a.hcount[i] = 0u; }
}


struct GqOut { int kbase, error, pad[2]; int cuts[16]; unsigned long long ticks[8]; };

constexpr int kLqDevMaxK = 256;
constexpr int kLqNodeCap = 16 * kLqDevMaxK + 256;
constexpr int kLqRoundCap = 512;
constexpr int kLqMaxRounds = 96;

struct LqCen { double mean[3]; double gn; };
struct LqHead {
    int done, error, rounds, nnodes, neval, pad;
    unsigned long long split_evals, split_px;
    double tau;
    double round_px[kLqMaxRounds], round_nr[kLqMaxRounds];
};
struct LqCtl {
    LqHead h;
    int K, M, nleaves, pad;
    int ncids[2];
    RoundDyn dyn;
    int leaves[kLqNodeCap];
    int round_ids[kLqRoundCap];
    int cids[2][2 * kLqRoundCap];
    int tA0[kLqRoundCap + 1], tP0[kLqRoundCap + 1];
    int nparent[kLqNodeCap];
    double np[kLqNodeCap];
    LqRec nrec[kLqNodeCap];
    LqCen ncen[kLqNodeCap];
};
template <> struct WsPoison<LqCtl> {
    static void dev(LqCtl *p, size_t a, size_t b) {
        for (size_t i = a; i < b; i++) {
            char *c = reinterpret_cast<char *>(p + i);
            ws_poison_dev(c + offsetof(LqCtl, h) + offsetof(LqHead, tau), sizeof(double) * (1 + 2 * kLqMaxRounds));
            ws_poison_dev(c + offsetof(LqCtl, np), sizeof(LqCtl::np));
            ws_poison_dev_rows(c + offsetof(LqCtl, nrec), sizeof(LqRec), sizeof(double), kLqNodeCap);
            ws_poison_dev(c + offsetof(LqCtl, ncen), sizeof(LqCtl::ncen));
        }
    }
    static void host(LqCtl *, size_t, size_t) {}
};

template <int CTRL, int ROW_MASK>
__device__ __forceinline__ double dpp_max_f64(const double v) {
    const int lo = __double2loint(v), hi = __double2hiint(v);
    const int tlo = __builtin_amdgcn_update_dpp(lo, lo, CTRL, ROW_MASK, 0xf, false);
    const int thi = __builtin_amdgcn_update_dpp(hi, hi, CTRL, ROW_MASK, 0xf, false);
    return fmax(v, __hiloint2double(thi, tlo));
}

__global__ __launch_bounds__(256) void k_lq_children(NodeDev *nodes, LqCtl *c, const int call, int init_kbase,
                                                     const int init_first, int init_nnodes, const int init_K, const GqOut *gq) {
    const bool init = init_kbase > 0;
    if (!init && c->h.done) return;
    if (init && gq) { init_kbase = gq->kbase; init_nnodes = init_first + init_kbase; }
    const int ncids = init ? init_kbase : c->ncids[call & 1];
    const int wave = (int)blockIdx.x * 4 + (int)(threadIdx.x >> 6), lane = threadIdx.x & 63;
    if (init && blockIdx.x == 0 && threadIdx.x == 0) {
        c->K = init_K; c->M = init_K - init_kbase; c->nleaves = 0; c->ncids[0] = init_kbase; c->dyn = RoundDyn{0, 0, 0, 0};
        c->h.done = 0; c->h.error = 0; c->h.rounds = 0; c->h.nnodes = init_nnodes; c->h.neval = 0; c->h.split_evals = 0ULL; c->h.split_px = 0ULL;
        c->h.tau = 0.0;
        for (int r = 0; r < kLqMaxRounds; r++) { c->h.round_px[r] = 0.0; c->h.round_nr[r] = 0.0; }
        if (gq && gq->error) { c->h.done = 1; c->h.error = 3; c->ncids[0] = 0; }
        for (int i = 0; i < init_first; i++) { c->nrec[i] = LqRec{0.0, -1, 1}; c->np[i] = 0.0; c->nparent[i] = -1; }
    }
    if (init && gq && gq->error) return;
    if (wave >= ncids) return;
    const int id = init ? init_first + wave : c->cids[call & 1][wave];
    if (init && lane == 0) c->cids[0][wave] = id;
    NodeDev &d = nodes[id];
    const double *acc = &d.acc[0][0][0];
    double sum = 0;
    if (lane < 14) {
        double v[kSlots];
#pragma unroll
        for (int k = 0; k < kSlots; k++) v[k] = acc[k * 14 + lane];
#pragma unroll
        for (int k = 0; k < kSlots; k++) sum += v[k];
    }
    const double pair = sum + __shfl_down(sum, 1, 64);
    double cov[7];
#pragma unroll
    for (int q = 0; q < 7; q++)
        cov[q] = __hiloint2double(__builtin_amdgcn_readlane(__double2hiint(pair), 2 * q), __builtin_amdgcn_readlane(__double2loint(pair), 2 * q));
    if (lane != 0) return;
    double ub = cov[6];
    const bool single = d.gn <= 1ULL;
    const double sw = d.sw;
    if (single || !(sw > 0)) ub = 0;
    else {
        double c6[6];
        for (int q = 0; q < 6; q++) c6[q] = cov[q] / sw;
        const double b = hm::lambda_max_bound(c6) * sw * (1.0 + 1e-9) + 1e-9 * cov[6];
        if (b == b && b < ub) ub = b;
    }
    for (int q = 0; q < 6; q++) d.cov6[q] = cov[q];
    d.dist = cov[6]; d.ub = ub; d.axis_state = 0;
    c->nrec[id] = LqRec{single ? 0.0 : ub, -1, single ? 1 : 0};
    c->nparent[id] = init ? -1 : c->round_ids[wave >> 1];
    c->ncen[id] = LqCen{{d.mean[0], d.mean[1], d.mean[2]}, (double)d.gn};
    c->leaves[(init ? 0 : c->nleaves) + wave] = id;
}

__device__ __forceinline__ int block_excl_scan_256(const int v, int *sw , int &total) {
    const int lane = threadIdx.x & 63, wid = threadIdx.x >> 6;
    const int inc = (int)wave_scan_incl_u32((unsigned)v);
    __syncthreads();
    if (lane == 63) sw[wid] = inc;
    __syncthreads();
    int base = 0;
    for (int w = 0; w < wid; w++) base += sw[w];
    total = sw[0] + sw[1] + sw[2] + sw[3];
    return base + inc - v;
}

__device__ __forceinline__ unsigned long long lq_key(const double p) { return p > 0.0 ? (unsigned long long)__double_as_longlong(p) : 0ULL; }

constexpr double kSpecBeta = 0.25;

__global__ __launch_bounds__(256) void k_lq_select(NodeDev *nodes, LqCtl *c, const int call, const int e_lin, const int e_quad) {
    if (c->h.done) return;
    const int tid = threadIdx.x, lane = tid & 63;
    const int cur = call & 1, nxt = cur ^ 1;
    const int ncids = c->ncids[cur];
    if (blockIdx.x > 0) {
        const int w = ((int)blockIdx.x - 1) * 4 + (tid >> 6);
        if (w >= ncids) return;
        NodeDev &d = nodes[c->cids[cur][w]];
        if (d.gn <= 1ULL || !(d.sw > 0)) { if (lane == 0) d.axis_state = d.gn <= 1ULL ? 0 : -1; return; }
        double c6[6];
        for (int q = 0; q < 6; q++) c6[q] = d.cov6[q] / d.sw;
        double a[9] = {c6[0], c6[1], c6[2], c6[1], c6[3], c6[4], c6[2], c6[4], c6[5]};
        double wv[3];
        const int info = hm::eigen_sym3(a, wv);
        if (lane == 0) {
            if (info != 0) d.axis_state = -1;
            else { d.axis[0] = a[6]; d.axis[1] = a[7]; d.axis[2] = a[8]; d.axis_state = 1; }
        }
        return;
    }
    __shared__ int sw[5];
    __shared__ unsigned int hist[256];
    __shared__ unsigned long long s_prefix, s_px;
    __shared__ int s_need, s_neval, s_first;
    __shared__ double s_umax[4];
    const int M = c->M;
    const int nn = c->h.nnodes;
    const int nr_prev = c->dyn.nr;
    int evald = 0;
    for (int i = tid; i < nr_prev; i += 256) {
        const int id = c->round_ids[i];
        const NodeDev &d = nodes[id];
        if (d.axis_state < 0) { c->nrec[id] = LqRec{0.0, -1, 1}; c->np[id] = 0.0; continue; }
        const int l = d.child0;
        const double b = d.dist - (nodes[l].dist + nodes[l + 1].dist);
        const int par = c->nparent[id];
        const double pp = par < 0 ? INFINITY : c->np[par];
        c->nrec[id].val = b; c->nrec[id].kn = 1;
        c->np[id] = b < pp ? b : pp;
        evald++;
    }
    if (tid == 0) { s_neval = 0; s_px = 0ULL; }
    __syncthreads();
    if (evald) atomicAdd(&s_neval, evald);
    __syncthreads();
    const int neval = c->h.neval + s_neval;
    double tau = 0.0;
    if (neval >= M && M > 0) {
        unsigned long long prefix = 0ULL;
        int need = M;
        for (int pass = 0; pass < 3; pass++) {
            const int shift = 56 - 8 * pass;
            hist[tid] = 0u;
            __syncthreads();
            for (int i = tid; i < nn; i += 256) {
                const LqRec r = c->nrec[i];
                if (r.kn && r.left >= 0) {
                    const unsigned long long k = lq_key(c->np[i]);
                    if (pass == 0 || (k >> (shift + 8)) == (prefix >> (shift + 8))) atomicAdd(&hist[(k >> shift) & 255ULL], 1u);
                }
            }
            __syncthreads();
            {
                const int mine = (int)hist[255 - tid];
                int total;
                const int excl = block_excl_scan_256(mine, sw, total);
                if (tid == 0) s_first = 256;
                __syncthreads();
                if (excl + mine >= need && tid <= 254) atomicMin(&s_first, tid);
                __syncthreads();
                const int f = s_first;
                if (f < 256) { if (tid == f) { s_need = need - excl; s_prefix = prefix | ((unsigned long long)(255 - f) << shift); } }
                else if (tid == 254) { s_need = need - (excl + mine); s_prefix = prefix; }
            }
            __syncthreads();
            need = s_need; prefix = s_prefix;
        }
        tau = __longlong_as_double((long long)prefix);
    }
    const double thr = fmax(kDelta, tau * (1.0 - 1e-9));
    const int nleaves = c->nleaves + ncids;
    auto leaf_prio = [&](const int id) -> double {
        const LqRec r = c->nrec[id];
        const int par = c->nparent[id];
        if (r.kn || (par >= 0 && nodes[par].axis_state < 0)) return -1.0;
        const double pp = par < 0 ? INFINITY : c->np[par];
        return r.val < pp ? r.val : pp;
    };
    double thr2 = thr;
    if (c->h.rounds < 48) {
        double u = -1.0;
        for (int i = tid; i < nleaves; i += 256) { const double pr = leaf_prio(c->leaves[i]); u = pr > u ? pr : u; }
#pragma unroll
        for (int o = 32; o > 0; o >>= 1) { const double v = __shfl_xor(u, o, 64); u = v > u ? v : u; }
        __syncthreads();
        if (lane == 0) s_umax[tid >> 6] = u;
        __syncthreads();
        u = fmax(fmax(s_umax[0], s_umax[1]), fmax(s_umax[2], s_umax[3]));
        if (kSpecBeta * u > thr2) thr2 = kSpecBeta * u;
    }
    int nkeep = 0, nr = 0;
    for (int base = 0; base < nleaves; base += 256) {
        const int i = base + tid;
        int id = -1, sel = 0, keep = 0;
        if (i < nleaves) {
            id = c->leaves[i];
            const double pr = leaf_prio(id);
            sel = pr >= thr2 ? 1 : 0;
            keep = (!sel && pr >= thr) ? 1 : 0;
        }
        int tsel, tkeep;
        const int psel = block_excl_scan_256(sel, sw, tsel);
        if (nr + tsel > kLqRoundCap && sel && nr + psel >= kLqRoundCap) { sel = 0; keep = 1; }
        const int pkeep = block_excl_scan_256(keep, sw, tkeep);
        if (sel) c->round_ids[nr + psel] = id;
        __syncthreads();
        if (keep) c->leaves[nkeep + pkeep] = id;
        nr = min(nr + tsel, kLqRoundCap);
        nkeep += tkeep;
        __syncthreads();
    }
    if (nr == 0) {
        if (tid == 0) { c->h.done = 1; c->h.neval = neval; c->h.tau = tau; c->nleaves = 0; c->ncids[nxt] = 0; c->dyn = RoundDyn{0, 0, 0, 0}; }
        return;
    }
    if (nn + 2 * nr > kLqNodeCap) {
        if (tid == 0) { c->h.done = 1; c->h.error = 2; c->dyn = RoundDyn{0, 0, 0, 0}; }
        return;
    }
    int runA = 0, runP = 0;
    for (int base = 0; base < nr; base += 256) {
        const int r = base + tid;
        int ta = 0, tp = 0;
        unsigned long long n = 0ULL;
        if (r < nr) {
            const int id = c->round_ids[r];
            NodeDev &d = nodes[id];
            d.slot = r; d.child0 = nn + 2 * r; d.nchild = 2;
            int P = 1;
            while ((1ULL << P) < (d.gn > 1ULL ? d.gn : 2ULL)) P++;
            d.klin = make_bink(e_lin, P); d.kquad = make_bink(e_quad, P);
            c->nrec[id].left = nn + 2 * r;
            c->cids[nxt][2 * r] = nn + 2 * r; c->cids[nxt][2 * r + 1] = nn + 2 * r + 1;
            n = d.n;
            ta = (int)((n + kTileA - 1) / kTileA); tp = (int)((n + kTileP - 1) / kTileP);
        }
        int totA, totP;
        const int pa = block_excl_scan_256(ta, sw, totA);
        const int pp = block_excl_scan_256(tp, sw, totP);
        if (r < nr) { c->tA0[r] = runA + pa; c->tP0[r] = runP + pp; }
        runA += totA; runP += totP;
        for (int o = 32; o > 0; o >>= 1) n += __shfl_xor(n, o, 64);
        if (lane == 0 && n) atomicAdd(&s_px, n);
    }
    __syncthreads();
    if (tid == 0) {
        const int round = c->h.rounds;
        const unsigned long long rpx = s_px;
        c->tA0[nr] = runA; c->tP0[nr] = runP;
        c->nleaves = nkeep; c->ncids[nxt] = 2 * nr;
        c->dyn = RoundDyn{nr, runA, runP, 0};
        c->h.nnodes = nn + 2 * nr; c->h.neval = neval; c->h.tau = tau;
        c->h.split_evals += (unsigned long long)nr; c->h.split_px += rpx; c->h.rounds = round + 1;
        if (round < kLqMaxRounds) { c->h.round_px[round] = (double)rpx; c->h.round_nr[round] = (double)nr; }
    }
}

__global__ __launch_bounds__(256) void k_lq_export(const LqCtl *c, LqHead *head, LqRec *rec, LqCen *cen) {
    const int nn = c->h.nnodes;
    const int t = blockIdx.x * blockDim.x + threadIdx.x, stride = gridDim.x * blockDim.x;
    for (int i = t; i < nn; i += stride) { rec[i] = c->nrec[i]; cen[i] = c->ncen[i]; }
    const double *src = reinterpret_cast<const double *>(&c->h);
    double *dst = reinterpret_cast<double *>(head);
    for (int i = t; i < (int)(sizeof(LqHead) / sizeof(double)); i += stride) dst[i] = src[i];
}

__global__ void k_lq_trace(const NodeDev *nodes, const LqCommit *commits, int n, patolette_amd__SplitRecord *out) {
    const int t = blockIdx.x * blockDim.x + threadIdx.x;
    if (t >= n) return;
    const LqCommit cm = commits[t];
    const NodeDev &h = nodes[cm.node], &hl = nodes[cm.left], &hr = nodes[cm.left + 1];
    patolette_amd__SplitRecord tr;
    tr.row = cm.row; tr.new_row = cm.new_row;
    tr.split = hl.psplit < 0 ? -1 : (hl.psplit & 0xffff); tr.degenerate = hl.psplit < 0 ? 0 : (hl.psplit >> 16) & 1;
    tr.n = h.gn; tr.n_left = hl.gn; tr.n_right = hr.gn; tr.sw = h.sw;
    for (int j = 0; j < 3; j++) tr.axis[j] = h.axis[j];
    for (int q = 0; q < 6; q++) tr.cov6[q] = h.cov6[q] / h.sw;
    tr.dist = h.dist; tr.dist_left = hl.dist; tr.dist_right = hr.dist; tr.benefit = h.dist - (hl.dist + hr.dist);
    out[t] = tr;
}

__global__ __launch_bounds__(256) void k_round_setup_dyn(NodeDev *table, const LqCtl *c, Tile *tilesA, Tile *tilesP, double *hist,
                                                         unsigned long long *hsize, unsigned int *hcount, const size_t lqs) {
    const int nr = c->dyn.nr;
    if (nr == 0) return;
    const int ntA = c->dyn.ntA, ntP = c->dyn.ntP;
    const size_t tid = (size_t)blockIdx.x * blockDim.x + threadIdx.x, stride = (size_t)gridDim.x * blockDim.x;
    for (size_t i = tid; i < (size_t)nr * kNodeResetElems; i += stride)
        node_reset_element(table[c->round_ids[i / kNodeResetElems]], (int)(i % kNodeResetElems));
    for (size_t t = tid; t < (size_t)ntA; t += stride) {
        const int r = node_of_tile(c->tA0, nr, (int)t);
        const NodeDev &d = table[c->round_ids[r]];
        const unsigned long long o = (unsigned long long)((int)t - c->tA0[r]) * kTileA, n = d.n;
        tilesA[t] = Tile{d.begin + o, (unsigned)(n - o < (unsigned long long)kTileA ? n - o : kTileA), (unsigned)c->round_ids[r]};
    }
    for (size_t t = tid; t < (size_t)ntP; t += stride) {
        const int r = node_of_tile(c->tP0, nr, (int)t);
        const NodeDev &d = table[c->round_ids[r]];
        const unsigned long long o = (unsigned long long)((int)t - c->tP0[r]) * kTileP, n = d.n;
        tilesP[t] = Tile{d.begin + o, (unsigned)(n - o < (unsigned long long)kTileP ? n - o : kTileP), (unsigned)c->round_ids[r]};
    }
    for (size_t i = tid; i < lqs * (size_t)nr; i += stride) hist[i] = 0.0;
    for (size_t i = tid; i < (size_t)nr * kBuckets; i += stride) { hsize[i] = 0ULL; hcount[i] = 0u; }
}

struct GqTab {
    unsigned long long w0[kBuckets + 1];
    double t[10][kBuckets + 9];
    __device__ double distortion(int a, int b) const {
        if (w0[a] == w0[b]) return 0;
        const double q0 = t[0][b] - t[0][a], q1 = t[1][b] - t[1][a], q2 = t[2][b] - t[2][a];
        return t[3][b] - t[3][a] - (q0 * q0 + q1 * q1 + q2 * q2) / (double)(w0[b] - w0[a]);
    }
    __device__ double vcov(int a, int b, int r, int s) const {
        if (w0[a] == w0[b]) return 0;
        const double cnt = (double)(w0[b] - w0[a]);
        const int rs = 4 + s * (s + 1) / 2 + r;
        return (t[rs][b] - t[rs][a]) / cnt - (t[r][b] - t[r][a]) * (t[s][b] - t[s][a]) / (cnt * cnt);
    }
    __device__ bool axis(int a, int b, double ax[3]) const {
        double m[9] = {0, 0, 0, 0, 0, 0, 0, 0, 0};
        for (int s = 0; s < 3; s++) for (int r = 0; r <= s; r++) m[s * 3 + r] = vcov(a, b, r, s);
        m[0 * 3 + 2] = m[2 * 3 + 0]; m[0 * 3 + 1] = m[1 * 3 + 0]; m[1 * 3 + 2] = m[2 * 3 + 1];
        double w[3];
        if (hm::eigen_sym3(m, w) != 0) return false;
        ax[0] = m[6]; ax[1] = m[7]; ax[2] = m[8];
        return true;
    }
    __device__ static double norm3(const double a[3]) { double s = 0; for (int i = 0; i < 3; i++) s += a[i] * a[i]; return sqrt(s); }
    __device__ double bias(int a, int b, const double ax[3]) const {
        double ca[3];
        if (!axis(a, b, ca)) return -1;
        const double norms = norm3(ax) * norm3(ca);
        if (norms < 1e-16) return 0;
        const double dot = (ca[0] * ax[0] + ca[1] * ax[1] + ca[2] * ax[2]);
        return fmin(1.0, fabs(dot / norms));
    }
};

__device__ __forceinline__ void gq_dp_entry(const GqTab &c, const double *Ep, const int k, const int n, const int lane, double &e_out, int &cut_out) {
    double best = INFINITY; int bt = -1;
    for (int t = n - 2 - lane; t >= k - 1; t -= 64) {
        const double v = Ep[t] + c.distortion(t, n);
        if (v < best) { best = v; bt = t; }
    }
#pragma unroll
    for (int o = 32; o > 0; o >>= 1) {
        const double v2 = __shfl_down(best, o, 64); const int t2 = __shfl_down(bt, o, 64);
        if (t2 >= 0 && (bt < 0 || v2 < best || (v2 == best && t2 > bt))) { best = v2; bt = t2; }
    }
    double e = Ep[n - 1]; int cut = n - 1;
    if (bt >= 0 && best < e) { e = best; cut = bt; }
    e_out = e; cut_out = cut;
}

__global__ __launch_bounds__(1024) void k_gq_control(const double *__restrict__ hist, const unsigned int *__restrict__ hcount, GqDpDev *g,
                                                     const int palette_size, const int weighted, NodeDev *nodes, const int base0,
                                                     unsigned char *lut, GqOut *out, GqOut *out_host) {
    __shared__ GqTab c;
    __shared__ double E[2][kBuckets + 1];
    __shared__ int s_q[16], s_nq, s_stop, s_err, s_top;
    __shared__ double s_ax[3], s_cd[16], s_cb[16];
    __shared__ unsigned char s_lut[kBuckets];
    __shared__ double s_part[kGqMaxK][4][2];
    __shared__ unsigned long long s_cnt[kGqMaxK];
    const int tid = threadIdx.x, lane = tid & 63, wv = tid >> 6;
    __shared__ unsigned long long s_ticks[8];
    if (tid == 0) { for (int i = 0; i < 8; i++) s_ticks[i] = 0; s_ticks[0] = wall_clock64(); }
    for (int i = tid; i < 10 * kBuckets; i += 1024) {
        const int hq = i / kBuckets, b = i - hq * kBuckets;
        c.t[hq][b + 1] = hist[(size_t)(hq * 2 + 0) * kBuckets + b] + hist[(size_t)(hq * 2 + 1) * kBuckets + b];
    }
    for (int b = tid; b < kBuckets; b += 1024) c.w0[b + 1] = hcount[b];
    if (tid < 10) c.t[tid][0] = 0;
    if (tid == 10) c.w0[0] = 0;
    __syncthreads();
    if (tid == 0) s_ticks[5] = wall_clock64();
    if (wv < 10) {
        double *t = c.t[wv];
        double v[8];
#pragma unroll
        for (int u = 0; u < 8; u++) v[u] = t[1 + lane * 8 + u];
        double carry = 0, cin = 0;
        for (int l = 0; l < 64; l++) {
            double a = carry;
#pragma unroll
            for (int u = 0; u < 8; u++) a = v[u] + a;
            cin = lane == l ? carry : cin;
            carry = __hiloint2double(__builtin_amdgcn_readlane(__double2hiint(a), l), __builtin_amdgcn_readlane(__double2loint(a), l));
        }
        double a = cin;
#pragma unroll
        for (int u = 0; u < 8; u++) { a = v[u] + a; t[1 + lane * 8 + u] = a; }
    }
    if (wv == 10) {
        unsigned long long v[8], run = 0;
#pragma unroll
        for (int u = 0; u < 8; u++) { run += c.w0[1 + lane * 8 + u]; v[u] = run; }
        unsigned long long inc = run;
#pragma unroll
        for (int o = 1; o < 64; o <<= 1) { const unsigned long long t = __shfl_up(inc, o, 64); if (lane >= o) inc += t; }
        const unsigned long long before = inc - run;
#pragma unroll
        for (int u = 0; u < 8; u++) c.w0[1 + lane * 8 + u] = before + v[u];
    }
    __syncthreads();
    if (tid == 0) s_ticks[1] = wall_clock64();
    for (int i = tid; i < (kGqMaxK + 1) * (kBuckets + 1); i += 1024) { const int r = i / (kBuckets + 1), n = i - r * (kBuckets + 1); g->cut[r][n] = r == n ? r : 0; }
    for (int i = tid; i <= kBuckets; i += 1024) E[1][i] = i >= 1 ? c.distortion(0, i) : 0.0;
    if (tid == 0) {
        double ax[3] = {0, 0, 0};
        s_err = c.axis(0, kBuckets, ax) ? 0 : 1;
        s_ax[0] = ax[0]; s_ax[1] = ax[1]; s_ax[2] = ax[2];
        s_q[0] = 0; s_q[1] = kBuckets; s_nq = 2; s_stop = 0;
    }
    __syncthreads();
    const int kmax = palette_size < kGqMaxK ? palette_size : kGqMaxK;
    if (tid == 0) s_ticks[2] = wall_clock64();
    for (int k = 2; k <= kmax && !s_err; k++) {
        const int cells = s_nq - 1;
        if (lane == 0 && wv < cells) {
            const double ax[3] = {s_ax[0], s_ax[1], s_ax[2]};
            s_cd[wv] = c.distortion(s_q[wv], s_q[wv + 1]);
            if (cells == 1) {
                const double norms = GqTab::norm3(ax) * GqTab::norm3(ax);
                s_cb[wv] = norms < 1e-16 ? 0.0 : fmin(1.0, fabs((ax[0] * ax[0] + ax[1] * ax[1] + ax[2] * ax[2]) / norms));
            } else s_cb[wv] = c.bias(s_q[wv], s_q[wv + 1], ax);
        }
        __syncthreads();
        if (tid == 0) {
            double distortion = 0;
            for (int j = 0; j < cells; j++) distortion += s_cd[j];
            int stop = 0;
            if (distortion < 1e-16) stop = 1;
            else {
                double bias = 0;
                for (int i = 0; i < cells; i++) {
                    const double cd = s_cd[i], cb = s_cb[i];
                    if (cb < 0) { stop = 1; break; }
                    if (cb < 0.9) continue;
                    bias += (cd / distortion) * cb;
                }
                if (!stop) stop = bias < 0.1 ? 1 : 0;
            }
            s_stop = stop;
        }
        __syncthreads();
        if (s_stop) break;
        if (k > 2) {
            const int kk = k - 1;
            const double *Ep = E[(kk - 1) & 1];
            double *En = E[kk & 1];
            for (int n = wv; n <= kBuckets; n += 16) {
                if (n < kk + 1) { if (lane == 0) En[n] = Ep[n]; continue; }
                double e; int cut;
                gq_dp_entry(c, Ep, kk, n, lane, e, cut);
                if (lane == 0) { En[n] = e; g->cut[kk][n] = cut; }
            }
            __syncthreads();
        }
        if (wv == 0) {
            double e; int cut;
            gq_dp_entry(c, E[(k - 1) & 1], k, kBuckets, lane, e, cut);
            if (lane == 0) s_top = cut;
        }
        __syncthreads();
        if (tid == 0) {
            int t = s_top;
            s_q[k - 1] = t;
            for (int j = k - 2; j >= 1; j--) { t = g->cut[j + 1][t]; s_q[j] = t; }
            s_q[0] = 0; s_q[k] = kBuckets; s_nq = k + 1;
        }
        __syncthreads();
    }
    const int kbase = s_nq - 1;
    if (tid == 0) s_ticks[3] = wall_clock64();
    for (int b = tid; b < kBuckets; b += 1024) {
        int j = 0;
        while (j < kbase - 1 && !(b + 1 <= s_q[j + 1])) j++;
        s_lut[b] = (unsigned char)j;
        lut[b] = (unsigned char)j;
    }
    __syncthreads();
    const int nq = weighted ? 4 : 3;
    if (wv < 2 * nq) {
        const int q = wv >> 1, part = wv & 1, qi = weighted ? 10 + q : q;
        const double *h = hist + (size_t)(qi * 2 + part) * kBuckets + lane * 8;
        double v[8];
#pragma unroll
        for (int u = 0; u < 8; u++) v[u] = h[u];
        for (int j = 0; j < kbase; j++) {
            double a = 0;
#pragma unroll
            for (int u = 0; u < 8; u++) a += s_lut[lane * 8 + u] == j ? v[u] : 0.0;
#pragma unroll
            for (int o = 32; o > 0; o >>= 1) a += __shfl_xor(a, o, 64);
            if (lane == 0) s_part[j][q][part] = a;
        }
    } else if (wv == 8) {
        unsigned long long v[8];
#pragma unroll
        for (int u = 0; u < 8; u++) v[u] = hcount[lane * 8 + u];
        for (int j = 0; j < kbase; j++) {
            unsigned long long a = 0;
#pragma unroll
            for (int u = 0; u < 8; u++) a += s_lut[lane * 8 + u] == j ? v[u] : 0ULL;
#pragma unroll
            for (int o = 32; o > 0; o >>= 1) a += __shfl_xor(a, o, 64);
            if (lane == 0) s_cnt[j] = a;
        }
    }
    __syncthreads();
    if (tid < kbase) {
        const int j = tid;
        unsigned long long pos = 0;
        for (int i = 0; i < j; i++) pos += s_cnt[i];
        const unsigned long long cnt = s_cnt[j];
        NodeDev &ch = nodes[base0 + j];
        ch.begin = pos; ch.n = cnt; ch.gn = cnt; ch.buf = 1; ch.slot = -1; ch.child0 = -1; ch.nchild = 0;
        const double sw = weighted ? (s_part[j][3][0] + s_part[j][3][1]) : (double)cnt;
        const double inv = 1 / sw;
        for (int q = 0; q < 3; q++) { ch.axis[q] = 0; ch.mean[q] = (s_part[j][q][0] + s_part[j][q][1]) * inv; }
        ch.sw = sw; ch.klin = nodes[0].klin; ch.kquad = nodes[0].kquad;
        node_reset_outputs(ch);
        ch.split = -1; ch.psplit = -1;
    }
    if (tid == 64) {
        NodeDev &root = nodes[0];
        root.child0 = base0; root.nchild = kbase;
        root.split = kbase == 2 ? s_q[1] - 1 : -1;
        GqOut o;
        o.kbase = kbase; o.error = s_err; o.pad[0] = o.pad[1] = 0;
        for (int j = 0; j < 16; j++) o.cuts[j] = j <= kbase ? s_q[j] : 0;
        for (int j = 0; j < 8; j++) o.ticks[j] = s_ticks[j];
        o.ticks[4] = wall_clock64();
        *out = o;
        *out_host = o;
    }
}

__global__ void k_eigen_batch(const double *a9, size_t count, double *w3, double *z9, int *info) {
    const size_t i = (size_t)blockIdx.x * blockDim.x + threadIdx.x;
    if (i >= count) return;
    double a[9], w[3];
    for (int j = 0; j < 9; j++) a[j] = a9[i * 9 + j];
    info[i] = hm::eigen_sym3(a, w);
    for (int j = 0; j < 3; j++) w3[i * 3 + j] = w[j];
    for (int j = 0; j < 9; j++) z9[i * 9 + j] = a[j];
}

// ... 833 lines not shown
    void lap(double &acc) { if (on) { const double t = now_ms(); acc += t - mark; mark = t; } }
};
struct LqHostLoop {
    SplitFrontier F;
    std::vector<int> leaves;
    LqLaps laps;
};

static void absorb_child(HNode &c, const NodeOut &d) {
    c.begin = d.begin; c.n = d.n; c.gn = d.gn; c.buf = d.buf; c.sw = d.sw; c.psplit = d.psplit;
    for (int j = 0; j < 3; j++) c.mean[j] = d.mean[j];
    absorb_moments(c, d);
    leaf_bound(c);
}

static double lq_round_threshold(const SplitFrontier &F, size_t K) {
    double thr = std::max(kDelta, kSpecBeta * F.reference_benefit());
    const size_t R = K - F.count;
    std::vector<double> kb;
    F.known_values(kb);
    if (kb.size() >= R && R > 0) {
        std::nth_element(kb.begin(), kb.begin() + (R - 1), kb.end(), std::greater<double>());
        thr = std::max(thr, kb[R - 1] * (1.0 - 1e-9));
    }
    return thr;
}

static void lq_host_round(QuantCall &C, LqHostLoop &L) {
    Engine &E = C.E;
    hipStream_t s = E.stream;
    std::vector<HNode> &hn = C.hn;
    LqLaps &laps = L.laps;
    const HnRec rec{hn};
    const double thr = lq_round_threshold(L.F, C.K);
    laps.lap(laps.greedy);
    std::vector<int> round;
    {
        std::vector<int> keep;
        for (int id : L.leaves) {
            HNode &h = hn[id];
            if (hn_known(h)) continue;
            if (h.ub >= thr) round.push_back(id); else keep.push_back(id);
        }
        L.leaves.swap(keep);
    }
    if (round.empty()) {
        throw HipError("patolette_amd: split loop blocked without candidates");
    }
    laps.lap(laps.select);
    HIP_CHECK(hipStreamSynchronize(s));
    E.nodes.grow(hn.size() + 2 * round.size() + 2, hn.size());
    std::vector<int> todo;
    std::vector<NodeIn> recs;
    for (int id : round) {
        double ax[3];
        if (!node_axis(hn[id], ax)) { hn[id].nosplit = true; continue; }
        NodeIn d = make_nodedev(hn[id], C.bnd);
        for (int j = 0; j < 3; j++) d.axis[j] = ax[j];
        d.slot = (int)todo.size();
        d.child0 = (int)hn.size(); d.nchild = 2;
        hn[id].left = (int)hn.size(); hn[id].right = (int)hn.size() + 1;
        hn.push_back(HNode()); hn.push_back(HNode());
        todo.push_back(id); recs.push_back(d);
    }
    L.F.reload(rec);
    laps.lap(laps.axes);
    if (todo.empty()) return;
    const int nr = (int)todo.size();
    size_t rpx = 0;
    for (int id : todo) rpx += hn[id].n;
    static const bool lq_trace = getenv("PAMD_LQ_TRACE") != nullptr;
    if (lq_trace) fprintf(stderr, "patolette_amd: split round %zu: %d nodes, %zu pixels (%.2f of the image), %zu of %zu colours committed\n",
                          E.stats.lq_rounds + 1, nr, rpx, (double)rpx / (double)(C.N ? C.N : 1), L.F.count, C.K);
    std::vector<int> cids;
    for (int id : todo) { cids.push_back(hn[id].left); cids.push_back(hn[id].right); }
    std::vector<int> tAg = {0}, tPg = {0};
    for (int id : todo) {
        const unsigned long long n = hn[id].n;
        tAg.push_back(tAg.back() + (int)((n + kTileA - 1) / kTileA)); tPg.push_back(tPg.back() + (int)((n + kTileP - 1) / kTileP));
    }
    const int ntA = tAg[nr], ntP = tPg[nr];
    const size_t o_recs = 0, o_ids = o_recs + (size_t)nr * sizeof(NodeIn), o_cids = o_ids + (size_t)nr * sizeof(int),
                 o_tA = o_cids + cids.size() * sizeof(int), o_tP = o_tA + tAg.size() * sizeof(int),
                 pk_bytes = o_tP + tPg.size() * sizeof(int);
    E.h_packet.reserve(pk_bytes); E.packet.reserve(pk_bytes);
    const size_t lqs = (size_t)kNQ_LQ * 2 * kBuckets;
    reserve_quant_tables(E, QuantSizes(C.N, C.weighted ? 4 : 3, (size_t)nr));
    E.h_stage_out.reserve(cids.size());
    std::memcpy(E.h_packet.p + o_recs, recs.data(), (size_t)nr * sizeof(NodeIn));
    std::memcpy(E.h_packet.p + o_ids, todo.data(), (size_t)nr * sizeof(int));
    std::memcpy(E.h_packet.p + o_cids, cids.data(), cids.size() * sizeof(int));
    std::memcpy(E.h_packet.p + o_tA, tAg.data(), tAg.size() * sizeof(int));
    std::memcpy(E.h_packet.p + o_tP, tPg.data(), tPg.size() * sizeof(int));
    laps.lap(laps.packet);
    HIP_CHECK(hipMemcpyAsync(E.packet.p, E.h_packet.p, pk_bytes, hipMemcpyHostToDevice, s));
    const bool rev = E.stats.lq_rounds % 2 == 1;
    const int *d_ids = (const int *)(E.packet.p + o_ids), *d_cids = (const int *)(E.packet.p + o_cids);
    const int *d_tA0 = (const int *)(E.packet.p + o_tA), *d_tP0 = (const int *)(E.packet.p + o_tP);
    RoundSetup rs{(const NodeIn *)(E.packet.p + o_recs), d_ids, d_tA0, d_tP0, nr, ntA, ntP,
                  E.tilesA.p, E.tilesP.p, E.hist.p, lqs * nr, E.hsize.p, E.hcount.p, (size_t)nr * kBuckets};
    {
        const size_t work = std::max<size_t>(std::max<size_t>(std::max<size_t>(ntP, lqs * nr / 4), (size_t)nr * kNodeResetElems), 256);
        hipLaunchKernelGGL(k_round_setup, (unsigned)std::min<size_t>((work + 255) / 256, 2048), 256, 0, s, E.nodes.p, rs);
        HIP_CHECK(hipGetLastError());
    }
    launch_minmax(C.qlq, E.tilesA.p, ntA, rpx, E.nodes.p, s, rev);
    if (C.sh) shard_exchange_keys(E, d_ids, nr);
    launch_hist(C.qlq, false, E.tilesA.p, ntA, rpx, E.nodes.p, E.hist.p, E.hsize.p, E.hcount.p, s, !rev);
    if (C.sh) {
        comm_sum_dev(E, E.hist.p, lqs * nr, 0);
        if (C.weighted) comm_sum_dev(E, E.hsize.p, (size_t)nr * kBuckets, 1);
        comm_sum_dev(E, E.hcount.p, (size_t)nr * kBuckets, 2);
    }
    launch_cut(C.weighted, E.nodes.p, d_ids, nr, E.hist.p, E.hsize.p, E.hcount.p, E.lut.p, s);
    launch_partition(C.qlq, E.tilesP.p, ntP, rpx, d_ids, d_tP0, nr, E.nodes.p, E.lut.p, E.tilecnt.p, E.tileoff.p, true, s, C.inv_sums, rev);
    if (C.sh) {
        hipLaunchKernelGGL(k_shard_children_local, (nr + 63) / 64, 64, 0, s, E.nodes.p, d_ids, nr);
        HIP_CHECK(hipGetLastError());
        shard_exchange_acc(E, d_cids, 2 * nr);
    }
    laps.lap(laps.enqueue);
    get_nodes_dev(E, d_cids, (int)cids.size(), C.got);
    laps.lap(laps.wait);
    for (size_t i = 0; i < cids.size(); i++) absorb_child(hn[cids[i]], C.got[i]);
    for (int id : todo) { hn[id].split_done = true; E.stats.split_evals++; E.stats.split_px += hn[id].n; }
    for (int id : cids) L.leaves.push_back(id);
    L.F.reload(rec);
    E.stats.lq_rounds++;
    laps.lap(laps.children);
}

static void lq_host_loop(QuantCall &C, LqHostLoop &L) {
    Engine &E = C.E;
    const std::vector<HNode> &hn = C.hn;
    const HnRec rec{hn};
    SplitFrontier &F = L.F;
    E.stats.split_evals = 0; E.stats.split_px = 0; E.stats.lq_rounds = 0;
    if (F.count >= C.K) return;
    while (F.count < C.K) {
        const SplitFrontier::Step st = F.step(rec, g_debug_fault.load(std::memory_order_relaxed));
        if (st.status == SplitFrontier::kBlocked) { lq_host_round(C, L); continue; }
        if (st.status == SplitFrontier::kStopped) { E.trace_hdr.stopped_early = 1; break; }
        const HNode &h = hn[st.commit.node];
        const int l = st.commit.left, r = l + 1;
        patolette_amd__SplitRecord tr{};
        tr.row = st.commit.row; tr.new_row = st.commit.new_row;
        tr.split = hn[l].psplit < 0 ? -1 : (hn[l].psplit & 0xffff); tr.degenerate = hn[l].psplit < 0 ? 0 : (hn[l].psplit >> 16) & 1;
        tr.n = h.gn; tr.n_left = hn[l].gn; tr.n_right = hn[r].gn; tr.sw = h.sw;
        for (int j = 0; j < 3; j++) tr.axis[j] = h.axis[j];
        for (int q = 0; q < 6; q++) tr.cov6[q] = h.cov6[q] / h.sw;
        tr.dist = h.dist; tr.dist_left = hn[l].dist; tr.dist_right = hn[r].dist; tr.benefit = st.benefit;
        E.trace.push_back(tr);
        if (C.verbose) { printf("patolette ======== Processed colors: %zu\r", F.count); fflush(stdout); }
    }
    const LqLaps &t = L.laps;
    if (t.on) fprintf(stderr, "patolette_amd: split loop host ms: greedy %.3f select %.3f axes %.3f packet %.3f enqueue %.3f wait(gpu) %.3f children %.3f\n",
                      t.greedy, t.select, t.axes, t.packet, t.enqueue, t.wait, t.children);
}

static void lq_host_epilogue(QuantCall &C, const SplitFrontier &F) {
    Engine &E = C.E;
    const std::vector<HNode> &hn = C.hn;
    const size_t len = C.len = F.count;
    C.centers.assign(3 * len, 0.0);
    for (size_t i = 0; i < len; i++) for (int j = 0; j < 3; j++) C.centers[(size_t)j * len + i] = hn[F.result[i]].mean[j];
    if (C.max_members) { *C.max_members = 0; for (size_t i = 0; i < len; i++) *C.max_members = std::max(*C.max_members, hn[F.result[i]].gn); }
    E.stats.n_clusters = len;
    E.trace_hdr.n_clusters = (int32_t)len; E.trace_hdr.n_records = (int32_t)E.trace.size();
    E.cluster_centers = C.centers;
    E.stats.ms_lq = now_ms() - C.t0;
}

static int quantize_clusters_run(Engine &E, size_t N, size_t K, bool weighted, const Bounds &bnd,
                                 std::vector<double> &centers, size_t &len, bool verbose, unsigned long long *max_members, bool allow_device) {
    const size_t planes = weighted ? 4 : 3;
    const Shard *sh = E.shard;
    if (E.prep_N != N || E.prep_planes != planes) gq_prepare(E, N, weighted);
    E.prep_N = 0;
    const bool dev_eligible = lq_device_eligible(E, N, K, verbose, allow_device);
    E.nodes.reserve(std::max<size_t>(4 * K + 64, dev_eligible ? (size_t)kLqNodeCap : 0));
    const QuantSizes root(N, planes, 1);
    QuantCall C{E, N, sh ? sh->total : N, K, weighted, sh || E.invariant, verbose, dev_eligible, sh, bnd, centers, len, max_members,
                QuantBuffers{{E.cvt.p, E.bufA.p}, E.bkt.p, N, weighted}, QuantBuffers{{E.bufB.p, E.bufA.p}, E.bkt.p, N, weighted},
                (int)root.tilesA, (int)root.tilesP, hist_slot_doubles(), now_ms()};
    C.hn.reserve(4 * K + 64);

    gq_root_mean(C);
    gq_root_covariance(C);
    if (!gq_root_histogram(C)) return -1;
    const bool gq_dev = g_gq_device.load(std::memory_order_relaxed) != 0 && !sh && !verbose && K > (size_t)kGqMaxK;
    const int rc = gq_dev ? gq_device_turn(C) : gq_host_turn(C);
    if (rc != kHostLoop) return rc;
    E.stats.n_base_clusters = (size_t)C.kbase;
    if (verbose) printf("patolette ======== Base cluster count: %zu\n", (size_t)C.kbase);
    E.stats.ms_gq = now_ms() - C.t0;
    C.t0 = now_ms();

    LqHostLoop L{SplitFrontier(K, C.kbase, C.base_ids[0], kDelta, HnRec{C.hn}), C.base_ids, LqLaps{}};
    lq_host_loop(C, L);
    lq_host_epilogue(C, L.F);
    return 0;
}

static int quantize_clusters(Engine &E, size_t N, size_t K, bool weighted, const Bounds &bnd,
                             std::vector<double> &centers, size_t &len, bool verbose = false, unsigned long long *max_members = nullptr) {
    WsGuard wg(&E.stream, &E.stream2);
    int rc = quantize_clusters_run(E, N, K, weighted, bnd, centers, len, verbose, max_members, true);
    if (rc == -2) {
        E.prep_N = 0;
        rc = quantize_clusters_run(E, N, K, weighted, bnd, centers, len, verbose, max_members, false);
    }
    return rc;
}

std::atomic<int> g_km_update{-1};
std::atomic<int> g_perm_cache{1};

static void subsample_start(Engine &E, size_t Nt, size_t K, size_t max_samples) {
    if (E.perm_job.valid()) {
        try { E.perm_job.get(); } catch (...) { E.hperm_N = 0; E.hperm_nx = 0; }
    }
    const size_t ms = std::max(max_samples, (size_t)(256 * 256));
    if (K == 0 || Nt < K) return;
    const size_t nxK = K * (size_t)(int)(ms / K);
    if (!(Nt > nxK)) return;
    const size_t take = std::min(ms, Nt);
    if (!g_perm_cache.load(std::memory_order_relaxed)) { E.perm_N = 0; E.perm_nx = 0; E.hperm_N = 0; E.hperm_nx = 0; }
    if (E.perm_N == Nt && E.perm_nx >= nxK) return;
    if (E.hperm_N == Nt && E.hperm_nx >= nxK) return;
    E.h_perm.reserve(take);
    E.hperm_N = 0; E.hperm_nx = 0;
    int32_t *dst = E.h_perm.p;
    hm::PermScratch *ws = &E.perm_ws;
    E.perm_job = std::async(std::launch::async, [dst, Nt, take, ws] { hm::rand_perm_prefix(Nt, take, 1234u, dst, *ws); });
    E.hperm_N = Nt; E.hperm_nx = take;
}
static const int *subsample_list(Engine &E, size_t Nt, size_t nx, hipStream_t s) {
    if (E.perm_job.valid()) {
        try { E.perm_job.get(); } catch (...) { E.hperm_N = 0; E.hperm_nx = 0; throw; }
    }
    if (E.perm_N == Nt && E.perm_nx >= nx) return E.perm_dev.p;
    if (!(E.hperm_N == Nt && E.hperm_nx >= nx)) {
        E.h_perm.reserve(nx);
        hm::rand_perm_prefix(Nt, nx, 1234u, E.h_perm.p, E.perm_ws);
        E.hperm_N = Nt; E.hperm_nx = nx;
    }
    E.perm_dev.reserve(E.hperm_nx);
    HIP_CHECK(hipMemcpyAsync(E.perm_dev.p, E.h_perm.p, E.hperm_nx * sizeof(int), hipMemcpyHostToDevice, s));
    E.perm_N = Nt; E.perm_nx = E.hperm_nx;
    return E.perm_dev.p;
}
static bool km_update_order_free() {
    static const bool env = getenv("PAMD_KMEANS_UPDATE") && atoi(getenv("PAMD_KMEANS_UPDATE")) != 0;
    const int v = g_km_update.load(std::memory_order_relaxed);
    return v < 0 ? env : v != 0;
}
static void kmeans_refine(Engine &E, size_t N, bool weighted, std::vector<double> &centers, size_t k, int niter, size_t max_samples,
                          bool nonfinite, unsigned long long largest_cluster, double bound_x, double bound_w) {
    hipStream_t s = E.stream;
    const KmSums sums_v{bound_x, bound_w};
    const KmSums *sums = km_update_order_free() ? &sums_v : nullptr;
    std::vector<float> cent(3 * k);
    for (size_t i = 0; i < k; i++) for (int j = 0; j < 3; j++) cent[3 * i + j] = (float)centers[(size_t)j * k + i];
    const size_t min_samples = 256 * 256;
    const size_t ms = std::max(max_samples, min_samples);
    const int mppc = (int)(ms / k);
    const Shard *sh = E.shard;
    const size_t Nt = sh ? sh->total : N;
    auto expect_longest = [&](size_t nx_) { return (size_t)((double)largest_cluster / (double)(Nt ? Nt : 1) * (double)nx_); };
    bool ok = Nt >= k && !nonfinite;
    size_t nx = Nt;
    E.stats.kmeans_samples = 0;
    if (ok) {
        const bool sub = Nt > k * (size_t)mppc;
        if (sub) nx = k * (size_t)mppc;
        E.km.reserve(nx, (int)k);
        const int *dperm = nullptr;
        if (sub) dperm = subsample_list(E, Nt, nx, s);
        if (sh) {
            kmeans_gather_slice(E.cvt.p, N, weighted, dperm, nx, sh->begin, E.km, s);
            comm_sum_dev(E, E.km.sx.p, nx, 2); comm_sum_dev(E, E.km.sy.p, nx, 2); comm_sum_dev(E, E.km.sz.p, nx, 2);
            if (weighted) comm_sum_dev(E, E.km.sw.p, nx, 2);
            if (nx == k) {
                std::vector<float> f(3 * k);
                HIP_CHECK(hipMemcpy(f.data(), E.km.sx.p, k * sizeof(float), hipMemcpyDeviceToHost));
                HIP_CHECK(hipMemcpy(f.data() + k, E.km.sy.p, k * sizeof(float), hipMemcpyDeviceToHost));
                HIP_CHECK(hipMemcpy(f.data() + 2 * k, E.km.sz.p, k * sizeof(float), hipMemcpyDeviceToHost));
                for (size_t i = 0; i < k; i++) for (int j = 0; j < 3; j++) cent[3 * i + j] = f[(size_t)j * k + i];
            } else {
                HIP_CHECK(hipMemcpyAsync(E.km.cent.p, cent.data(), 3 * k * sizeof(float), hipMemcpyHostToDevice, s));
                HIP_CHECK(hipStreamSynchronize(s));
                kmeans_iterate(E.km, nx, (int)k, weighted, niter, s, expect_longest(nx), sums);
                HIP_CHECK(hipMemcpyAsync(cent.data(), E.km.cent.p, 3 * k * sizeof(float), hipMemcpyDeviceToHost, s));
                E.sync();
                E.stats.kmeans_samples = nx;
            }
        } else if (nx == k) {
            std::vector<double> first(3 * k);
            for (int j = 0; j < 3; j++) HIP_CHECK(hipMemcpy(first.data() + (size_t)j * k, E.cvt.p + (size_t)j * N, k * sizeof(double), hipMemcpyDeviceToHost));
            for (size_t i = 0; i < k; i++) for (int j = 0; j < 3; j++) cent[3 * i + j] = (float)first[(size_t)j * k + i];
        } else {
            kmeans_gather(E.cvt.p, N, weighted, dperm, nx, E.km, s);
            E.h_cent.reserve(3 * k);
            std::memcpy(E.h_cent.p, cent.data(), 3 * k * sizeof(float));
            HIP_CHECK(hipMemcpyAsync(E.km.cent.p, E.h_cent.p, 3 * k * sizeof(float), hipMemcpyHostToDevice, s));
            kmeans_iterate(E.km, nx, (int)k, weighted, niter, s, expect_longest(nx), sums);
            HIP_CHECK(hipMemcpyAsync(E.h_cent.p, E.km.cent.p, 3 * k * sizeof(float), hipMemcpyDeviceToHost, s));
            E.sync();
            std::memcpy(cent.data(), E.h_cent.p, 3 * k * sizeof(float));
            E.stats.kmeans_samples = nx;
        }
    }
    for (size_t i = 0; i < k; i++) for (int j = 0; j < 3; j++) centers[(size_t)j * k + i] = (double)cent[3 * i + j];
}

static void palette_rows(std::vector<double> &pal, size_t len, void (*f)(double[3])) {
    for (size_t i = 0; i < len; i++) {
        double c[3] = {pal[i], pal[len + i], pal[2 * len + i]};
        f(c);
        pal[i] = c[0]; pal[len + i] = c[1]; pal[2 * len + i] = c[2];
    }
}

static void upload_palette(Engine &E, const std::vector<double> &pal, size_t rows) {
    std::memcpy(E.h_pal.p, pal.data(), 3 * rows * sizeof(double));
    HIP_CHECK(hipMemcpyAsync(E.dpal.p, E.h_pal.p, 3 * rows * sizeof(double), hipMemcpyHostToDevice, E.stream));
}

static Bounds read_bounds(Engine &E, bool weighted, const std::function<void()> &between_copy_and_wait = nullptr) {
    E.h_cstats.reserve(1);
    HIP_CHECK(hipMemcpyAsync(E.h_cstats.p, E.cstats.p, sizeof(ConvertStats), hipMemcpyDeviceToHost, E.stream));
    if (between_copy_and_wait) {
        if (!E.ev_stats) HIP_CHECK(hipEventCreateWithFlags(&E.ev_stats, hipEventDisableTiming));
        HIP_CHECK(hipEventRecord(E.ev_stats, E.stream));
        between_copy_and_wait();
        HIP_CHECK(hipEventSynchronize(E.ev_stats));
    } else E.sync();
    const ConvertStats &cs = *E.h_cstats.p;
    Bounds b;
    b.cmax = 0; b.range = 0;
    unsigned long long kmin[3], kmax[3], kw = 0ULL, nonfinite = cs.nonfinite_f32 != 0u ? 1ULL : 0ULL;
    double parts[3][2];
    for (int p = 0; p < 3; p++) {
        kmin[p] = ~0ULL; kmax[p] = 0ULL;
        for (int t = 0; t < kStatSlots; t++) { kmin[p] = std::min(kmin[p], cs.minkey[t][p]); kmax[p] = std::max(kmax[p], cs.maxkey[t][p]); }
        parts[p][0] = 0; parts[p][1] = 0;
        for (int t = 0; t < kStatSlots; t++) { parts[p][0] += cs.sum[t][p][0]; parts[p][1] += cs.sum[t][p][1]; }
    }
    for (int t = 0; t < kStatSlots; t++) kw = std::max(kw, cs.wmaxkey[t]);
    if (E.shard) {
        const unsigned long long mine[8] = {kmin[0], kmin[1], kmin[2], kmax[0], kmax[1], kmax[2], kw, nonfinite};
        const std::vector<unsigned long long> all = comm_gather_u64(E, mine, 8);
        for (int r = 0; r < E.shard->comm.size; r++) {
            const unsigned long long *row = all.data() + (size_t)r * 8;
            for (int p = 0; p < 3; p++) { kmin[p] = std::min(kmin[p], row[p]); kmax[p] = std::max(kmax[p], row[3 + p]); }
            kw = std::max(kw, row[6]); nonfinite |= row[7];
        }
        comm_sum_host(E, &parts[0][0], 6, 0);
    }
    for (int p = 0; p < 3; p++) {
        const unsigned long long ka = kmin[p], kb = kmax[p];
        double mn = key_f64(ka), mx = key_f64(kb);
        if (!(mn <= mx)) { mn = 0; mx = 0; }
        b.lo[p] = mn; b.hi[p] = mx;
        b.cmax = std::max(b.cmax, std::max(std::fabs(mn), std::fabs(mx)));
        b.range = std::max(b.range, mx - mn);
    }
    b.wmax = weighted ? std::max(1.0, key_f64(kw)) : 1.0;
    const double lin = b.wmax * std::max(b.cmax, 1.0);
    const double quad = 3.0 * b.wmax * std::max(std::max(b.range, b.cmax), 1e-300) * std::max(std::max(b.range, b.cmax), 1e-300);
    b.e_lin = exp_bound(lin);
    b.e_quad = exp_bound(std::max(quad, 1e-300));
    for (int p = 0; p < 3; p++) { b.sum[p] = parts[p][0] + parts[p][1]; b.sum2[p][0] = parts[p][0]; b.sum2[p][1] = parts[p][1]; }
    for (int q = 0; q < 6; q++)
        for (int t = 0; t < kStatSlots; t++) { b.mom2[q][0] += cs.mom[t][q][0]; b.mom2[q][1] += cs.mom[t][q][1]; }
    b.nonfinite = nonfinite != 0ULL;
    return b;
}

struct DitherMask { size_t width, height; const int *cpos; };
struct Frames { size_t count, width, height; };

struct Pixels {
    const double *f64 = nullptr;
    const unsigned char *u8 = nullptr;
    int channels = 3;
    bool rows = false;
    bool converted = false;
};

struct ConvertPlan { int which; BinK sumk, momk; };
static ConvertPlan convert_plan(const Engine &E, const patolette__QuantizationOptions *opt, size_t N) {
    ConvertPlan p{PAMD_COPY, BinK{0.0, 0.0}, BinK{0.0, 0.0}};
    if (opt->color_space == patolette__CIELuv) p.which = PAMD_SRGB_TO_CIELUV;
    else if (opt->color_space == patolette__ICtCp) p.which = PAMD_SRGB_TO_ICTCP;
    const size_t Nt = E.shard ? E.shard->total : N;
    int rootP = 1; while ((1ULL << rootP) < (Nt > 1 ? Nt : 2)) rootP++;
    if (p.which == PAMD_SRGB_TO_ICTCP) p.sumk = make_bink(1, rootP);
    else if (p.which == PAMD_SRGB_TO_CIELUV) p.sumk = make_bink(8, rootP);
    if (!E.shard) {
        if (p.which == PAMD_SRGB_TO_ICTCP) p.momk = make_bink(1, rootP);
        else if (p.which == PAMD_SRGB_TO_CIELUV) p.momk = make_bink(16, rootP);
    }
    return p;
}

static void copy_dither_stats(Engine &E) {
    E.stats.dither_segments = E.nn.dither_segments; E.stats.dither_repairs = E.nn.dither_repairs; E.stats.dither_rounds = E.nn.dither_rounds;
    E.stats.dither_through = E.nn.dither_through; E.stats.dither_jumps = E.nn.dither_jumps; E.stats.dither_solo = E.nn.dither_solo;
}
static bool map_touched(bool dither, size_t width, size_t height) { return !(dither && std::max(width, height) <= 1); }

static void run_device(Engine &E, size_t width, size_t height, Pixels px, const double *d_weights, size_t K,
                       const patolette__QuantizationOptions *opt, double *palette, void *d_map, int map_elem, const DitherMask *mask = nullptr,
                       const Frames *frames = nullptr) {
    hipStream_t s = E.stream;
    const size_t N = width * height;
    const bool weighted = d_weights != nullptr;
    const double t_start = now_ms();
    WsGuard wg(&E.stream, &E.stream2);
    E.stats = patolette_amd__Stats{};
    E.prep_N = 0;
    ws_prepare(E, N, K, weighted, opt->verbose);
    if (opt->kmeans_niter > 0) subsample_start(E, E.shard ? E.shard->total : N, K, opt->kmeans_max_samples);
    double t0 = now_ms();
    E.cvt.reserve((weighted ? 4 : 3) * N);
    E.cstats.reserve(1);
    if (E.shard && opt->dither && !opt->palette_only)
        throw HipError("patolette_amd: dithering walks the whole image along one curve; it is not available per slice");
    const ConvertPlan cp = convert_plan(E, opt, N);
    const int which = cp.which;
    const BinK sumk = cp.sumk, momk = cp.momk;
    if (px.converted) {  }
    else if (px.u8) launch_convert_u8(which, px.u8, px.channels, E.cvt.p, N, E.cstats.p, s, sumk, momk);
    else if (px.rows) launch_convert_rows(which, px.f64, E.cvt.p, N, E.cstats.p, s, sumk, momk);
    else launch_convert(which, px.f64, E.cvt.p, N, E.cstats.p, s, sumk, momk);
    if (weighted) {
        HIP_CHECK(hipMemcpyAsync(E.cvt.p + 3 * N, d_weights, N * sizeof(double), hipMemcpyDeviceToDevice, s));
        launch_weight_stats(d_weights, N, E.cstats.p, s);
    }
    Bounds bnd = read_bounds(E, weighted, [&] { gq_prepare(E, N, weighted); });
    bnd.have_sum = sumk.M0 != 0.0;
    bnd.have_mom = momk.M0 != 0.0;
    E.stats.ms_convert = now_ms() - t0;

    if (opt->verbose) printf("patolette ======== Palette generation \n");
    std::vector<double> pal;
    size_t len = 0;
    unsigned long long largest_cluster = 0;
    if (quantize_clusters(E, N, K, weighted, bnd, pal, len, opt->verbose, &largest_cluster) != 0) throw HipError("internal quantization error");

    t0 = now_ms();
    if (opt->kmeans_niter > 0) {
        if (opt->verbose) printf("patolette ======== KMeans refinement\n");
        kmeans_refine(E, N, weighted, pal, len, opt->kmeans_niter, opt->kmeans_max_samples, bnd.nonfinite, largest_cluster, bnd.cmax, bnd.wmax);
    }
    E.stats.ms_kmeans = now_ms() - t0;

    t0 = now_ms();
    if (!opt->palette_only) {
        E.dpal.reserve(3 * len);
        if (opt->verbose) printf(opt->dither ? "patolette ======== Dithering\n" : "patolette ======== NN mapping\n");
        if (opt->dither) {
            int pix = PAMD_SRGB_TO_REC2020;
            void (*pf)(double[3]) = hm::color::srgb_to_rec2020;
            if (opt->color_space == patolette__CIELuv) { pix = PAMD_CIELUV_TO_REC2020; pf = hm::color::cieluv_to_rec2020; }
            else if (opt->color_space == patolette__ICtCp) { pix = PAMD_ICTCP_TO_REC2020; pf = hm::color::ictcp_to_rec2020; }
            palette_rows(pal, len, pf);
            E.map_palette = pal;
            if (d_map) {
                HIP_CHECK(hipMemcpyAsync(E.dpal.p, pal.data(), 3 * len * sizeof(double), hipMemcpyHostToDevice, s));
                HIP_CHECK(hipStreamSynchronize(s));
                auto dither = [&](const double *img, int which, int layout) {
                    if (mask) launch_dither_masked(img, N, which, mask->width, mask->height, mask->cpos, N, E.dpal.p, pal.data(), (int)len, d_map,
                                                   map_elem, E.nn, s, layout);
                    else if (frames) launch_dither_frames(img, N, which, frames->count, frames->width, frames->height, E.dpal.p, pal.data(), (int)len,
                                                          d_map, map_elem, E.nn, s, layout);
                    else launch_dither(img, N, which, width, height, E.dpal.p, pal.data(), (int)len, d_map, map_elem, E.nn, s, layout);
                };
                if (frames ? dither_frames_lane_layout(frames->count, frames->width, frames->height, (int)len)
                           : dither_lane_layout(width, height, (int)len)) {
                    dither(E.cvt.p, pix, 1);
                } else {
                    E.aux.reserve(3 * N);
                    launch_convert(pix, E.cvt.p, E.aux.p, N, nullptr, s);
                    dither(E.aux.p, PAMD_COPY, 0);
                }
                copy_dither_stats(E);
            }
            palette_rows(pal, len, hm::color::rec2020_to_srgb);
        } else {
            const double *pixels = E.cvt.p;
            const double *blo = bnd.lo, *bhi = bnd.hi;
            Bounds b2;
            if (opt->color_space == patolette__CIELuv) {
                if (d_map) {
                    E.aux.reserve(3 * N);
                    launch_convert(PAMD_CIELUV_TO_ICTCP, E.cvt.p, E.aux.p, N, E.cstats.p, s);
                    b2 = read_bounds(E, false);
                    blo = b2.lo; bhi = b2.hi;
                    pixels = E.aux.p;
                }
                palette_rows(pal, len, hm::color::cieluv_to_rec2020);
                palette_rows(pal, len, hm::color::rec2020_to_srgb);
                palette_rows(pal, len, hm::color::srgb_to_ictcp);
            }
            E.map_palette = pal;
            if (d_map) {
                E.h_pal.reserve(3 * len);
                upload_palette(E, pal, len);
                launch_nn_map(pixels, N, N, E.dpal.p, (int)len, d_map, map_elem, blo, bhi, E.nn, s);
            }
            palette_rows(pal, len, hm::color::ictcp_to_rec2020);
            palette_rows(pal, len, hm::color::rec2020_to_srgb);
        }
        E.sync();
    }
    E.stats.ms_map = now_ms() - t0;
    for (size_t j = 0; j < K * 3; j++) palette[j] = -1.0;
    for (int j = 0; j < 3; j++) for (size_t i = 0; i < len; i++) palette[K * (size_t)j + i] = pal[(size_t)j * len + i];
    E.stats.ms_total = now_ms() - t_start;
}

struct CodeError : std::runtime_error {
    int code;
    CodeError(int c, const char *m) : std::runtime_error(m), code(c) {}
};

static const double *derive_weights(Engine &E, const double *d_f64, const unsigned char *d_u8, int channels, size_t width,
                                    size_t height, double tile_size, size_t frames = 1) {
    const size_t n = width * height;
    E.wsal.reserve(frames * n);
    const double t0 = now_ms();
    int rc = kSalOk;
    for (size_t f = 0; f < frames && rc == kSalOk; f++)
        rc = saliency_weights(E.sal, d_f64, d_u8 ? d_u8 + f * n * (size_t)channels : nullptr, channels, width, height, tile_size, E.wsal.p + f * n,
                              E.stream);
    if (ktimer().enabled) ktimer().collect();
    E.ms_saliency = now_ms() - t0;
    if (rc == kSalBadShape) throw CodeError(-5, "saliency weights: image shape not supported");
    if (rc == kSalSingular) throw CodeError(-6, "saliency weights: singular border covariance");
    if (rc == kSalDegenerate) throw CodeError(-7, "saliency weights: degenerate saliency map");
    return E.wsal.p;
}

static int validate(size_t width, size_t height, size_t K) {
    const size_t px = width * height;
    if (px == 0) return -2;
    if (K < 1) return -3;
    if (px > (size_t)40000 * 40000) return -4;
    return 0;
}

static int map_elem_for(size_t K) { return K <= 256 ? 1 : 4; }

static void download_map_widened(Engine &E, const void *d_map, int me, size_t N, size_t *out) {
    if (N == 0) return;
    const size_t chunk = (size_t)2 << 20;
    const size_t nchunks = ceil_div(N, chunk);
    E.h_mapstage.reserve(2 * chunk * (size_t)me);
    const int T = (int)std::max<size_t>(1, std::min<size_t>({(size_t)8, (size_t)std::thread::hardware_concurrency(), ceil_div(N, (size_t)1 << 18)}));
    std::atomic<size_t> ready{0};
    std::vector<std::atomic<int>> done(nchunks);
    for (auto &d : done) d.store(0);
    std::atomic<bool> failed{false};
    auto worker = [&](int tid) {
        for (size_t c = 0; c < nchunks; c++) {
            while (ready.load(std::memory_order_acquire) <= c) {
                if (failed.load(std::memory_order_relaxed)) return;
                std::this_thread::yield();
            }
            const size_t lo = c * chunk, cnt = std::min(chunk, N - lo);
            const size_t a = cnt * (size_t)tid / (size_t)T, b = cnt * (size_t)(tid + 1) / (size_t)T;
            const unsigned char *src = E.h_mapstage.p + (c & 1) * chunk * (size_t)me;
            given_elems_out(src, me, out + lo, 8, a, b);
            done[c].fetch_add(1, std::memory_order_release);
        }
    };
    std::vector<std::thread> pool;
    for (int t = 1; t < T; t++) pool.emplace_back(worker, t);
    auto issue = [&](size_t c) {
        const size_t lo = c * chunk, cnt = std::min(chunk, N - lo);
        HIP_CHECK(hipMemcpyAsync(E.h_mapstage.p + (c & 1) * chunk * (size_t)me, (const unsigned char *)d_map + lo * (size_t)me, cnt * (size_t)me,
                                 hipMemcpyDeviceToHost, E.stream));
    };
    try {
        issue(0);
        for (size_t c = 0; c < nchunks; c++) {
            HIP_CHECK(hipStreamSynchronize(E.stream));
            ready.store(c + 1, std::memory_order_release);
            if (c + 1 < nchunks) {
                if (c >= 1) while (done[c - 1].load(std::memory_order_acquire) < T) std::this_thread::yield();
                issue(c + 1);
            }
            {
                const size_t lo = c * chunk, cnt = std::min(chunk, N - lo);
                const size_t b = cnt / (size_t)T;
                const unsigned char *src = E.h_mapstage.p + (c & 1) * chunk * (size_t)me;
                given_elems_out(src, me, out + lo, 8, 0, b);
                done[c].fetch_add(1, std::memory_order_release);
            }
        }
    } catch (...) {
        failed.store(true);
        for (auto &th : pool) th.join();
        throw;
    }
    for (auto &th : pool) th.join();
}
// ... 1497 lines not shown
```

### patolette_amd/csrc/quant.hip

```cpp
#include "quant.h"

#include <atomic>

#include <type_traits>

namespace pamd {

template <typename T>
__device__ __forceinline__ T block_scan_incl(T v, T *smem) {
    const int lane = threadIdx.x & 63, wid = threadIdx.x >> 6, nw = blockDim.x >> 6;
#pragma unroll
    for (int o = 1; o < 64; o <<= 1) {
        T t = __shfl_up(v, o, 64);
        if (lane >= o) v += t;
    }
    __syncthreads();
    if (lane == 63) smem[wid] = v;
    __syncthreads();
    if (wid == 0) {
        T s = lane < nw ? smem[lane] : T(0);
#pragma unroll
        for (int o = 1; o < 16; o <<= 1) {
            T t = __shfl_up(s, o, 64);
            if (lane >= o) s += t;
// ... 258 lines not shown
}
__device__ __forceinline__ long long fix_quant(const double v, const double magic) {
    return __double_as_longlong(v + magic) - __double_as_longlong(magic);
}
template <bool W, bool GQ>
__global__ __launch_bounds__(512) void k_hist_fix(QuantBuffers qb, const Tile *__restrict__ tiles, int ntiles, NodeDev *nodes,
                                              double *hist, unsigned long long *hsize, unsigned int *hcount, const int from_end) {
    constexpr int NQ = GQ ? (W ? 14 : 10) : (W ? 4 : 3);
    constexpr int NQS = GQ ? kNQ_GQ : kNQ_LQ;
    extern __shared__ unsigned long long lds64[];
    unsigned long long *h = lds64;
    unsigned long long *siz = h + NQ * kBuckets;
    unsigned int *cnt = (unsigned int *)(siz + kBuckets);
    for (int i = threadIdx.x; i < NQ * kBuckets; i += blockDim.x) h[i] = 0ULL;
    for (int i = threadIdx.x; i < kBuckets; i += blockDim.x) { cnt[i] = 0u; siz[i] = 0ULL; }
    __syncthreads();

    const int per = (ntiles + (int)gridDim.x - 1) / (int)gridDim.x;
    const int bid = from_end ? (int)gridDim.x - 1 - (int)blockIdx.x : (int)blockIdx.x;
    const int tfirst = bid * per, tlast = min(ntiles, tfirst + per);
    int since_flush = 0;
    for (int ti = tfirst; ti < tlast; ti++) {
        const Tile t = tiles[ti];
        NodeDev &nd = nodes[t.node];
        const double a0 = nd.axis[0], a1 = nd.axis[1], a2 = nd.axis[2];
        double mn, mx;
        node_minmax(nd, mn, mx);
        const bool degenerate = (mx - mn < kDelta);
        const double sc = 1 / (mx - mn);
        const FixK flin = make_fixk(nd.klin), fquad = make_fixk(nd.kquad);
        const double *px = qb.buf[nd.buf], *py = px + qb.N, *pz = py + qb.N, *pw = pz + qb.N;
        const unsigned long long gslot0 = nd.gslot0;
        if (threadIdx.x == 0) nd.degenerate = degenerate ? 1 : 0;

        auto one = [&](const size_t p, const double x, const double y, const double z, const double w) {
            unsigned b;
            if (degenerate) {
                b = (unsigned)((p - nd.begin + gslot0) % kBuckets);
            } else {
                double ratio = (project(x, y, z, a0, a1, a2) - mn) * sc;
                unsigned long long bq = (unsigned long long)((double)kBuckets * ratio);
                b = bq < (unsigned long long)(kBuckets - 1) ? (unsigned)bq : (unsigned)(kBuckets - 1);
            }
            qb.bkt[p] = (unsigned short)b;
            double pv[NQ], pm[NQ];
#define HPART(q, val, K) pv[q] = (val); pm[q] = (K).magic
            if constexpr (!GQ) {
                HPART(0, x * w, flin); HPART(1, y * w, flin); HPART(2, z * w, flin);
                if constexpr (W) { HPART(3, w, flin); }
            } else {
                HPART(0, x, flin); HPART(1, y, flin); HPART(2, z, flin);
                HPART(3, (x * x + y * y) + z * z, fquad);
                HPART(4, x * x, fquad); HPART(5, x * y, fquad); HPART(6, y * y, fquad);
                HPART(7, x * z, fquad); HPART(8, y * z, fquad); HPART(9, z * z, fquad);
                if constexpr (W) { HPART(10, x * w, flin); HPART(11, y * w, flin); HPART(12, z * w, flin); HPART(13, w, flin); }
            }
#undef HPART
            unsigned long long wi = 0ULL;
            if constexpr (W && !GQ) wi = (unsigned long long)w;
            bool direct = true;
            if (__ballot(true) == ~0ULL) {
                unsigned long long left = ~0ULL;
#pragma unroll 1
                for (int g = 0; g < 3 && left != 0ULL; g++) {
                    const int first = __builtin_ctzll(left);
                    const unsigned b0 = (unsigned)__builtin_amdgcn_readlane((int)b, first);
                    const bool mine = direct && b == b0;
                    const unsigned long long m = __ballot(mine);
                    if (__popcll(m) < kHistCombineMin) break;
#pragma unroll
                    for (int k2 = 0; k2 < NQ; k2++) {
                        const double vq = (pv[k2] + pm[k2]) - pm[k2];
                        const double sum = wave_sum_dpp63(mine ? vq : 0.0);
                        if ((threadIdx.x & 63) == 63) atomicAdd(&h[k2 * kBuckets + b0], (unsigned long long)fix_quant(sum, pm[k2]));
                    }
                    if constexpr (W && !GQ) {
                        unsigned long long sw2 = mine ? wi : 0ULL;
#pragma unroll
                        for (int o = 32; o > 0; o >>= 1) sw2 += __shfl_down(sw2, o, 64);
                        if ((threadIdx.x & 63) == 0) atomicAdd(&siz[b0], sw2);
                    }
                    if ((threadIdx.x & 63) == 0) atomicAdd(&cnt[b0], (unsigned)__popcll(m));
                    if (mine) direct = false;
                    left &= ~m;
                }
            }
            if (direct) {
                atomicAdd(&cnt[b], 1u);
#pragma unroll
                for (int k2 = 0; k2 < NQ; k2++) atomicAdd(&h[k2 * kBuckets + b], (unsigned long long)fix_quant(pv[k2], pm[k2]));
                if constexpr (W && !GQ) atomicAdd(&siz[b], wi);
            }
        };
        unsigned i = threadIdx.x;
        for (; i + 512 < t.count; i += 1024) {
            const size_t p0 = t.start + i, p1 = p0 + 512;
            const double x0 = px[p0], y0 = py[p0], z0 = pz[p0], x1 = px[p1], y1 = py[p1], z1 = pz[p1];
            double w0 = 1.0, w1 = 1.0;
            if constexpr (W) { w0 = pw[p0]; w1 = pw[p1]; }
            one(p0, x0, y0, z0, w0);
            one(p1, x1, y1, z1, w1);
        }
        for (; i < t.count; i += 512) {
            const size_t p = t.start + i;
            double w = 1.0;
            if constexpr (W) w = pw[p];
            one(p, px[p], py[p], pz[p], w);
        }
        since_flush++;
        const bool flush = (ti + 1 == tlast) || tiles[ti + 1].node != t.node || since_flush >= 16;
        if (!flush) continue;
        since_flush = 0;
        __syncthreads();
        const size_t slot = (size_t)nd.slot;
        double *gh = hist + slot * (size_t)(NQS * 2 * kBuckets);
        for (int i2 = threadIdx.x; i2 < NQ * kBuckets; i2 += blockDim.x) {
            const long long S = (long long)h[i2];
            if (S != 0) {
                const int q = i2 / kBuckets, bb = i2 % kBuckets;
                const bool quad = GQ && q >= 3 && q <= 9;
                const FixK &f = quad ? fquad : flin;
                const long long Sh = (S + (1LL << (f.s - 1))) >> f.s, Sl = S - (Sh << f.s);
                if (Sh != 0) unsafeAtomicAdd(&gh[(q * 2 + 0) * kBuckets + bb], (double)Sh * f.ghi);
                if (Sl != 0) unsafeAtomicAdd(&gh[(q * 2 + 1) * kBuckets + bb], (double)Sl * f.glo);
                h[i2] = 0ULL;
            }
        }
        for (int b = threadIdx.x; b < kBuckets; b += blockDim.x) {
            unsigned c = cnt[b];
            if (c) { atomicAdd(&hcount[slot * kBuckets + b], c); cnt[b] = 0u; }
            if constexpr (W && !GQ) { const unsigned long long s2 = siz[b]; if (s2) { atomicAdd(&hsize[slot * kBuckets + b], s2); siz[b] = 0ULL; } }
        }
        __syncthreads();
    }
}

template <bool W>
__global__ __launch_bounds__(512) void k_cut(NodeDev *nodes, const int *__restrict__ round_nodes, const double *__restrict__ hist,
                                             const unsigned long long *__restrict__ hsize, const unsigned int *__restrict__ hcount,
                                             unsigned char *lut, const int fault, const RoundDyn *__restrict__ dyn) {
    if (dyn && (int)blockIdx.x >= dyn->nr) return;
    __shared__ double sd[4 * 16];
    __shared__ unsigned long long su[2 * 16];
    __shared__ double best_v[8];
    __shared__ int best_i[8];
    __shared__ double tot[8];
    __shared__ unsigned long long tots[2];
    __shared__ int s_split;
    const int b = threadIdx.x;
    NodeDev &nd = nodes[round_nodes[blockIdx.x]];
    const size_t slot = (size_t)nd.slot;
    const double *gh = hist + slot * (size_t)(kNQ_LQ * 2 * kBuckets);
    constexpr int NQ = W ? 4 : 3;
    double p[NQ][2];
    {
        double v0[NQ], v1[NQ];
#pragma unroll
        for (int q = 0; q < NQ; q++) { v0[q] = gh[(q * 2 + 0) * kBuckets + b]; v1[q] = gh[(q * 2 + 1) * kBuckets + b]; }
        block_scan_incl_vec<double, NQ>(v0, sd);
        block_scan_incl_vec<double, NQ>(v1, sd);
#pragma unroll
        for (int q = 0; q < NQ; q++) { p[q][0] = v0[q]; p[q][1] = v1[q]; }
    }
    unsigned long long cs[2] = {(unsigned long long)hcount[slot * kBuckets + b], W ? hsize[slot * kBuckets + b] : 0ULL};
    block_scan_incl_vec<unsigned long long, 2>(cs, su);
    const unsigned long long cnt = cs[0], siz = W ? cs[1] : cs[0];
    __syncthreads();
    if (b == kBuckets - 1) {
#pragma unroll
        for (int q = 0; q < NQ; q++) { tot[q * 2] = p[q][0]; tot[q * 2 + 1] = p[q][1]; }
        tots[0] = cnt; tots[1] = siz;
    }
    __syncthreads();
    double obj = 0;
    {
        const double sl = (double)siz, sr = (double)tots[1] - sl;
#pragma unroll
        for (int j = 0; j < 3; j++) {
            double csl = p[j][0] + p[j][1];
            double csr = (tot[j * 2] + tot[j * 2 + 1]) - csl;
            double v = 0;
            if (sl != 0) v += (csl * csl) / sl;
            if (sr != 0) v += (csr * csr) / sr;
            obj += v;
        }
    }
    double bv = obj; int bi = b;
#pragma unroll
    for (int o = 32; o > 0; o >>= 1) {
        double ov = __shfl_down(bv, o, 64); int oi = __shfl_down(bi, o, 64);
        if (ov > bv || (ov == bv && (fault == 3 ? oi > bi : oi < bi))) { bv = ov; bi = oi; }
    }
    if ((b & 63) == 0) { best_v[b >> 6] = bv; best_i[b >> 6] = bi; }
    __syncthreads();
    if (b == 0) {
        for (int w = 1; w < 8; w++)
            if (best_v[w] > bv || (best_v[w] == bv && (fault == 3 ? best_i[w] > bi : best_i[w] < bi))) { bv = best_v[w]; bi = best_i[w]; }
        if (fault == 1) {
            unsigned long long upto = 0;
            for (int i = 0; i <= bi; i++) upto += hcount[slot * kBuckets + i];
            int b2 = bi + 1;
            while (b2 < kBuckets - 1 && hcount[slot * kBuckets + b2] == 0u) b2++;
            if (b2 < kBuckets - 1 && upto + hcount[slot * kBuckets + b2] < tots[0]) bi = b2;
        }
        s_split = bi;
    }
    __syncthreads();
    const int split = s_split;
    lut[slot * kBuckets + b] = b > split ? 1 : 0;
    if (b == split) {
        nd.split = split;
        const unsigned long long nL = cnt, nR = tots[0] - cnt;
        nd.cbegin[0] = nd.begin; nd.cbegin[1] = nd.begin + nL; nd.cbegin[2] = nd.begin + nd.n;
        for (int side = 0; side < 2; side++) {
            NodeDev &ch = nodes[nd.child0 + side];
            ch.begin = side == 0 ? nd.begin : nd.begin + nL;
            ch.n = side == 0 ? nL : nR;
            ch.gn = ch.n;
            ch.buf = 1 - nd.buf;
            ch.slot = -1; ch.child0 = -1; ch.nchild = 0;
            ch.klin = nd.klin; ch.kquad = nd.kquad;
            ch.psplit = split | (nd.degenerate ? 0x10000 : 0);
            double s0[NQ], s1[NQ];
#pragma unroll
            for (int q = 0; q < NQ; q++) {
                s0[q] = side == 0 ? p[q][0] : tot[q * 2] - p[q][0];
                s1[q] = side == 0 ? p[q][1] : tot[q * 2 + 1] - p[q][1];
            }
            double sw = W ? (s0[NQ - 1] + s1[NQ - 1]) : (double)ch.n;
            ch.sw = sw;
            const double inv = 1 / sw;
            for (int j = 0; j < 3; j++) ch.mean[j] = (s0[j] + s1[j]) * inv;
            ch.axis[0] = ch.axis[1] = ch.axis[2] = 0;
        }
    }
    for (int i = b; i < 2 * kNodeResetElems; i += kBuckets)
        node_reset_element(nodes[nd.child0 + i / kNodeResetElems], i % kNodeResetElems);
}

__global__ __launch_bounds__(256) void k_count(QuantBuffers qb, const Tile *__restrict__ tiles, const NodeDev *__restrict__ nodes,
                                               const unsigned char *__restrict__ lut, unsigned int *tilecnt, const int from_end,
                                               const RoundDyn *__restrict__ dyn) {
    __shared__ unsigned int c[kMaxChildren];
    __shared__ unsigned char sl[kBuckets];
    const unsigned nt = dyn ? (unsigned)dyn->ntP : gridDim.x;
    if (blockIdx.x >= nt) return;
    const unsigned tix = from_end ? nt - 1u - blockIdx.x : blockIdx.x;
    const Tile t = tiles[tix];
    const NodeDev &nd = nodes[t.node];
    const unsigned char *l = lut + (size_t)nd.slot * kBuckets;
    if (threadIdx.x < kMaxChildren) c[threadIdx.x] = 0;
    const int nch = nd.nchild;
    typedef unsigned short us8 __attribute__((ext_vector_type(8), aligned(2)));
    const int split = nd.split;
    if (nch == 2 && split >= 0) {
        const unsigned i0 = threadIdx.x * 8u;
        unsigned right = 0;
        if (i0 + 8u <= t.count) {
            const us8 v = *reinterpret_cast<const us8 *>(qb.bkt + t.start + i0);
#pragma unroll
            for (int j = 0; j < 8; j++) right += (int)v[j] > split ? 1u : 0u;
        } else {
            for (unsigned i = i0; i < t.count && i < i0 + 8u; i++) right += (int)qb.bkt[t.start + i] > split ? 1u : 0u;
        }
        __syncthreads();
        right = wave_sum_u32(right);
        if ((threadIdx.x & 63) == 0 && right) atomicAdd(&c[1], right);
        __syncthreads();
        if (threadIdx.x == 0) c[0] = t.count - c[1];
        __syncthreads();
    } else if (nch == 2) {
        for (int b = threadIdx.x; b < kBuckets; b += blockDim.x) sl[b] = l[b];
        __syncthreads();
        const unsigned i0 = threadIdx.x * 8u;
        unsigned right = 0;
        if (i0 + 8u <= t.count) {
            const us8 v = *reinterpret_cast<const us8 *>(qb.bkt + t.start + i0);
#pragma unroll
            for (int j = 0; j < 8; j++) right += sl[v[j]];
        } else {
            for (unsigned i = i0; i < t.count && i < i0 + 8u; i++) right += sl[qb.bkt[t.start + i]];
        }
        right = wave_sum_u32(right);
        if ((threadIdx.x & 63) == 0 && right) atomicAdd(&c[1], right);
        __syncthreads();
        if (threadIdx.x == 0) c[0] = t.count - c[1];
        __syncthreads();
    } else {
        __syncthreads();
        for (unsigned i = threadIdx.x; i < ((t.count + 255u) & ~255u); i += blockDim.x) {
            int child = i < t.count ? (int)l[qb.bkt[t.start + i]] : 255;
            for (int k = 0; k < nch; k++) {
                unsigned long long m = __ballot(child == k);
                if ((threadIdx.x & 63) == 0 && m) atomicAdd(&c[k], (unsigned)__popcll(m));
            }
        }
        __syncthreads();
    }
    if (threadIdx.x < kMaxChildren) tilecnt[(size_t)tix * kMaxChildren + threadIdx.x] = c[threadIdx.x];
}
__global__ __launch_bounds__(1024) void k_scan(const int *__restrict__ round_nodes, const int *__restrict__ node_tile0, NodeDev *nodes,
                                              const unsigned int *__restrict__ tilecnt, unsigned long long *tileoff,
                                              const RoundDyn *__restrict__ dyn) {
    if (dyn && (int)blockIdx.x >= dyn->nr) return;
    __shared__ unsigned long long su[16];
    __shared__ unsigned long long total;
    NodeDev &nd = nodes[round_nodes[blockIdx.x]];
    const int t0 = node_tile0[blockIdx.x], t1 = node_tile0[blockIdx.x + 1];
    const int C = (t1 - t0 + (int)blockDim.x - 1) / (int)blockDim.x;
    const int a = t0 + (int)threadIdx.x * C, b = min(t1, a + C);
    unsigned long long base = nd.begin;
    const int nch = nd.nchild;
    if (nch == 2) {
        __shared__ unsigned long long sv[2 * 16];
        __shared__ unsigned long long tot2[2];
        unsigned long long sum[2] = {0, 0};
        for (int g = a; g < b; g += 8) {
            uint2 v[8];
#pragma unroll
            for (int q = 0; q < 8; q++) v[q] = g + q < b ? *reinterpret_cast<const uint2 *>(tilecnt + (size_t)(g + q) * kMaxChildren) : make_uint2(0u, 0u);
#pragma unroll
            for (int q = 0; q < 8; q++) { sum[0] += v[q].x; sum[1] += v[q].y; }
        }
        unsigned long long inc[2] = {sum[0], sum[1]};
        block_scan_incl_vec<unsigned long long, 2>(inc, sv);
        if (threadIdx.x == blockDim.x - 1) { tot2[0] = inc[0]; tot2[1] = inc[1]; }
        __syncthreads();
        const unsigned long long base1 = base + tot2[0];
        unsigned long long run0 = base + inc[0] - sum[0], run1 = base1 + inc[1] - sum[1];
        for (int g = a; g < b; g += 8) {
            uint2 v[8];
#pragma unroll
            for (int q = 0; q < 8; q++) v[q] = g + q < b ? *reinterpret_cast<const uint2 *>(tilecnt + (size_t)(g + q) * kMaxChildren) : make_uint2(0u, 0u);
#pragma unroll
            for (int q = 0; q < 8; q++) {
                if (g + q < b) *reinterpret_cast<ulonglong2 *>(tileoff + (size_t)(g + q) * kMaxChildren) = make_ulonglong2(run0, run1);
                run0 += v[q].x; run1 += v[q].y;
            }
        }
        if (threadIdx.x == 0) { nd.cbegin[0] = base; nd.cbegin[1] = base1; nd.cbegin[2] = base1 + tot2[1]; }
        return;
    }
    for (int k = 0; k < nch; k++) {
        unsigned long long sum = 0;
        for (int g = a; g < b; g += 8) {
            unsigned v[8];
#pragma unroll
            for (int q = 0; q < 8; q++) v[q] = g + q < b ? tilecnt[(size_t)(g + q) * kMaxChildren + k] : 0u;
#pragma unroll
            for (int q = 0; q < 8; q++) sum += v[q];
        }
        const unsigned long long inc = block_scan_incl<unsigned long long>(sum, su);
        if (threadIdx.x == blockDim.x - 1) total = inc;
        unsigned long long run = base + inc - sum;
        for (int g = a; g < b; g += 8) {
            unsigned v[8];
#pragma unroll
            for (int q = 0; q < 8; q++) v[q] = g + q < b ? tilecnt[(size_t)(g + q) * kMaxChildren + k] : 0u;
#pragma unroll
            for (int q = 0; q < 8; q++) {
                if (g + q < b) tileoff[(size_t)(g + q) * kMaxChildren + k] = run;
                run += v[q];
            }
        }
        if (threadIdx.x == 0) nd.cbegin[k] = base;
        __syncthreads();
        base += total;
        __syncthreads();
    }
    if (threadIdx.x == 0) nd.cbegin[nch] = base;
}

template <bool W>
__global__ __launch_bounds__(256, 5) void k_scatter(QuantBuffers qb, const Tile *__restrict__ tiles, int ntiles, NodeDev *nodes,
                                                    const unsigned char *__restrict__ lut, const unsigned long long *__restrict__ tileoff,
                                                    const int from_end) {
    constexpr int R = kTileP / 256;
    __shared__ unsigned long long off[R][4][kMaxChildren];
    const int lane = threadIdx.x & 63, wid = threadIdx.x >> 6;
    const unsigned long long ltmask = (1ULL << lane) - 1ULL;
    if ((from_end & 4) && nodes[0].nchild == 2) return;
    const int per = (ntiles + (int)gridDim.x - 1) / (int)gridDim.x;
    const int bid = (from_end & 1) ? (int)gridDim.x - 1 - (int)blockIdx.x : (int)blockIdx.x;
    const int tfirst = bid * per, tlast = min(ntiles, tfirst + per);
    for (int ti = tfirst; ti < tlast; ti++) {
        const Tile t = tiles[ti];
        const NodeDev &nd = nodes[t.node];
        const unsigned char *l = lut + (size_t)nd.slot * kBuckets;
        const int nch = nd.nchild;
        unsigned cr[R];
#pragma unroll
        for (int r = 0; r < R; r++) {
            unsigned i = r * 256 + threadIdx.x;
            int ch = 255;
            if (i < t.count) ch = (int)l[qb.bkt[t.start + i]];
            unsigned rk = 0;
            for (int k = 0; k < nch; k++) {
                unsigned long long m = __ballot(ch == k);
                if (ch == k) rk = (unsigned)__popcll(m & ltmask);
                if (lane == 0) off[r][wid][k] = (unsigned long long)__popcll(m);
            }
            cr[r] = (unsigned)ch | (rk << 8);
        }
        __syncthreads();
        if ((int)threadIdx.x < nch) {
            unsigned long long run = tileoff[(size_t)ti * kMaxChildren + threadIdx.x];
            for (int r = 0; r < R; r++)
                for (int w = 0; w < 4; w++) { unsigned long long c = off[r][w][threadIdx.x]; off[r][w][threadIdx.x] = run; run += c; }
        }
        __syncthreads();
        const double *sx = qb.buf[nd.buf], *sy = sx + qb.N, *sz = sy + qb.N, *sw = sz + qb.N;
        double *dx = qb.buf[1 - nd.buf], *dy = dx + qb.N, *dz = dy + qb.N, *dw = dz + qb.N;
#pragma unroll
        for (int r = 0; r < R; r++) {
            const int ch = (int)(cr[r] & 255u);
            if (ch != 255) {
                const size_t src = t.start + r * 256 + threadIdx.x;
                const size_t dst = off[r][wid][ch] + (cr[r] >> 8);
                const double x = sx[src], y = sy[src], z = sz[src];
                double w = 1.0;
                if constexpr (W) w = sw[src];
                dx[dst] = x; dy[dst] = y; dz[dst] = z;
                if constexpr (W) dw[dst] = w;
            }
        }
        __syncthreads();
    }
}

template <bool W, bool INV>
__global__ __launch_bounds__(256, (W || INV) ? 2 : 3) void k_scatter_bin(QuantBuffers qb, const Tile *__restrict__ tiles, int ntiles, NodeDev *nodes,
                                                                        const NodeDev *__restrict__ nodes_ro,
                                                                        const unsigned long long *__restrict__ tileoff, const int from_end,
                                                                        const RoundDyn *__restrict__ dyn) {
    constexpr int R = kTileP / 256;
    static_assert(R * 4 == 32, "one 32-lane group per child");
    __shared__ unsigned int wcnt[2][2][R * 4];
    __shared__ double sm[28 * 4];
    const int lane = threadIdx.x & 63, wid = __builtin_amdgcn_readfirstlane((int)(threadIdx.x >> 6));
    const unsigned long long ltmask = (1ULL << lane) - 1ULL;
    int nblk = (int)gridDim.x;
    if ((from_end & 2) && nodes_ro[0].nchild != 2) return;
    if (dyn) {
        ntiles = dyn->ntP;
        nblk = min(ntiles, nblk);
        if ((int)blockIdx.x >= nblk) return;
    }
    const int per = (ntiles + nblk - 1) / nblk;
    const int bid = (from_end & 1) ? nblk - 1 - (int)blockIdx.x : (int)blockIdx.x;
    const int tfirst = bid * per, tlast = min(ntiles, tfirst + per);
    if (tfirst >= tlast) return;
    constexpr int NP = INV ? 14 : 7;
    double pl[NP], pr[NP];
#pragma unroll
    for (int i = 0; i < NP; i++) { pl[i] = 0; pr[i] = 0; }

    auto fetch_buckets = [&](const Tile &tt, const int ti, unsigned (&b)[R], unsigned long long &toff) {
        const unsigned last = tt.count - 1u;
#pragma unroll
        for (int r = 0; r < R; r++) b[r] = qb.bkt[tt.start + min((unsigned)(r * 256) + threadIdx.x, last)];
        toff = tileoff[(size_t)ti * kMaxChildren + (lane >> 5)];
    };
    auto classify = [&](const Tile &tt, const unsigned (&b)[R], const int split, const int par, unsigned (&cr)[R]) {
#pragma unroll
        for (int r = 0; r < R; r++) {
            const bool valid = (unsigned)(r * 256) + threadIdx.x < tt.count;
            const bool right = (int)b[r] > split;
            const unsigned long long mR = __ballot(valid && right), mL = __ballot(valid && !right);
            const unsigned rk = (unsigned)__popcll((right ? mR : mL) & ltmask);
            cr[r] = (valid ? (right ? 1u : 0u) : 2u) | (rk << 8);
            if (lane == 0) { wcnt[par][0][r * 4 + wid] = (unsigned)__popcll(mL); wcnt[par][1][r * 4 + wid] = (unsigned)__popcll(mR); }
        }
    };
    auto lane64 = [](const unsigned long long v, const int l) {
        return ((unsigned long long)(unsigned)__builtin_amdgcn_readlane((int)(unsigned)(v >> 32), l) << 32) |
               (unsigned)__builtin_amdgcn_readlane((int)(unsigned)v, l);
    };
    Tile t = tiles[tfirst];
    unsigned cr[R];
    unsigned long long baseL, baseR;
    {
        unsigned b0[R];
        unsigned long long toff;
        fetch_buckets(t, tfirst, b0, toff);
        classify(t, b0, nodes_ro[t.node].split, 0, cr);
        baseL = lane64(toff, 0); baseR = lane64(toff, 32);
    }
    for (int ti = tfirst; ti < tlast; ti++) {
        const int par = (ti - tfirst) & 1;
        const NodeDev &nd = nodes_ro[t.node];
        const int child0 = nd.child0;
        const double *sx = qb.buf[nd.buf], *sy = sx + qb.N, *sz = sy + qb.N, *sw = sz + qb.N;
        double *dx = qb.buf[1 - nd.buf], *dy = dx + qb.N, *dz = dy + qb.N, *dw = dz + qb.N;
        double x[R], y[R], z[R], w[R];
        {
            const unsigned last = t.count - 1u;
#pragma unroll
            for (int r = 0; r < R; r++) {
                const size_t src = t.start + min((unsigned)(r * 256) + threadIdx.x, last);
                x[r] = sx[src]; y[r] = sy[src]; z[r] = sz[src];
                w[r] = 1.0;
                if constexpr (W) w[r] = sw[src];
            }
        }
        const bool more = ti + 1 < tlast;
        const int tnx = more ? ti + 1 : ti;
        const Tile tn = tiles[tnx];
        unsigned bkn[R];
        unsigned long long toffn;
        fetch_buckets(tn, tnx, bkn, toffn);
        __syncthreads();
        const unsigned c = wcnt[par][lane >> 5][lane & 31];
        const unsigned incl = wave_scan_incl_u32(c);
        const unsigned tot0 = (unsigned)__builtin_amdgcn_readlane((int)incl, 31);
        const unsigned excl = incl - c - (lane >= 32 ? tot0 : 0u);
        const NodeDev &c0 = nodes_ro[child0], &c1 = nodes_ro[child0 + 1];
        const double m0L = c0.mean[0], m1L = c0.mean[1], m2L = c0.mean[2], m0R = c1.mean[0], m1R = c1.mean[1], m2R = c1.mean[2];
        BinK kinv{0.0, 0.0};
        if constexpr (INV) kinv = nd.kquad;
        const size_t slack = (size_t)(W ? 4 : 3) * qb.N + (size_t)lane;
#pragma unroll
        for (int r = 0; r < R; r++) {
            const unsigned eL = (unsigned)__builtin_amdgcn_readlane((int)excl, r * 4 + wid);
            const unsigned eR = (unsigned)__builtin_amdgcn_readlane((int)excl, 32 + r * 4 + wid);
            const unsigned ch = cr[r] & 255u;
            const bool right = ch == 1u, none = ch == 2u;
            const size_t dst = (right ? baseR + eR : baseL + eL) + (cr[r] >> 8);
            dx[none ? slack : dst] = x[r]; dy[none ? slack - qb.N : dst] = y[r]; dz[none ? slack - 2 * qb.N : dst] = z[r];
            if constexpr (W) dw[none ? slack - 3 * qb.N : dst] = w[r];
            const double rf = right ? 1.0 : 0.0, lf = ch == 0u ? 1.0 : 0.0;
            const double ex = x[r] - (right ? m0R : m0L), ey = y[r] - (right ? m1R : m1L), ez = z[r] - (right ? m2R : m2L);
            const double wx = w[r] * ex, wy = w[r] * ey, wz = w[r] * ez;
            const double q[7] = {wx * ex, wy * ex, wz * ex, wy * ey, wz * ey, wz * ez, ((ex * ex + ey * ey) + ez * ez) * w[r]};
            if constexpr (INV) {
#pragma unroll
                for (int i = 0; i < 7; i++) {
                    double v0, v1;
                    bin_split(q[i], kinv, v0, v1);
                    pl[2 * i] = __builtin_fma(v0, lf, pl[2 * i]); pl[2 * i + 1] = __builtin_fma(v1, lf, pl[2 * i + 1]);
                    pr[2 * i] = __builtin_fma(v0, rf, pr[2 * i]); pr[2 * i + 1] = __builtin_fma(v1, rf, pr[2 * i + 1]);
                }
            } else {
#pragma unroll
                for (int i = 0; i < 7; i++) { pl[i] = __builtin_fma(q[i], lf, pl[i]); pr[i] = __builtin_fma(q[i], rf, pr[i]); }
            }
        }
        const bool flush = !more || tn.node != t.node;
        if (flush) {
            const BinK kq = nd.kquad;
            double a[28];
            if constexpr (INV) {
#pragma unroll
                for (int i = 0; i < 14; i++) { a[i] = pl[i]; a[14 + i] = pr[i]; pl[i] = 0; pr[i] = 0; }
            } else {
#pragma unroll
                for (int i = 0; i < 7; i++) {
                    bin_split(pl[i], kq, a[2 * i], a[2 * i + 1]);
                    bin_split(pr[i], kq, a[14 + 2 * i], a[14 + 2 * i + 1]);
                    pl[i] = 0; pr[i] = 0;
                }
            }
            block_sum<28>(a, sm);
            if (threadIdx.x == 0) {
                for (int side = 0; side < 2; side++) {
                    NodeDev &chn = nodes[child0 + side];
                    for (int i = 0; i < 7; i++) {
                        if (a[14 * side + 2 * i] != 0.0) unsafeAtomicAdd(&chn.acc[blockIdx.x & (kSlots - 1)][i][0], a[14 * side + 2 * i]);
                        if (a[14 * side + 2 * i + 1] != 0.0) unsafeAtomicAdd(&chn.acc[blockIdx.x & (kSlots - 1)][i][1], a[14 * side + 2 * i + 1]);
                    }
                }
            }
        }
        if (more) {
            classify(tn, bkn, nodes_ro[tn.node].split, par ^ 1, cr);
            baseL = lane64(toffn, 0); baseR = lane64(toffn, 32);
        }
        t = tn;
    }
}

template <bool W>
__device__ __forceinline__ void cov_accumulate(const double *px, const double *py, const double *pz, const double *pw,
                                               size_t lo, size_t hi, const double m0, const double m1, const double m2,
                                               const BinK kq, double (&a)[14]) {
    for (size_t p = lo + threadIdx.x; p < hi; p += blockDim.x) {
        double dx = px[p] - m0, dy = py[p] - m1, dz = pz[p] - m2;
        double w = 1.0;
        if constexpr (W) w = pw[p];
        double wx = w * dx, wy = w * dy, wz = w * dz;
        bin_add(wx * dx, kq, a[0], a[1]);
        bin_add(wy * dx, kq, a[2], a[3]);
        bin_add(wz * dx, kq, a[4], a[5]);
        bin_add(wy * dy, kq, a[6], a[7]);
        bin_add(wz * dy, kq, a[8], a[9]);
        bin_add(wz * dz, kq, a[10], a[11]);
        bin_add(((dx * dx + dy * dy) + dz * dz) * w, kq, a[12], a[13]);
    }
}

template <bool W>
__global__ __launch_bounds__(256) void k_cov_children(QuantBuffers qb, const Tile *__restrict__ tiles, NodeDev *nodes, const int from_end) {
    __shared__ double sm[14 * 4];
    if ((from_end & 4) && nodes[0].nchild == 2) return;
    const Tile t = tiles[(from_end & 1) ? gridDim.x - 1u - blockIdx.x : blockIdx.x];
    const NodeDev &nd = nodes[t.node];
    const double *px = qb.buf[1 - nd.buf], *py = px + qb.N, *pz = py + qb.N, *pw = pz + qb.N;
    const size_t t_lo = t.start, t_hi = t.start + t.count;
    for (int k = 0; k < nd.nchild; k++) {
        size_t lo = nd.cbegin[k] > t_lo ? nd.cbegin[k] : t_lo;
        size_t hi = nd.cbegin[k + 1] < t_hi ? nd.cbegin[k + 1] : t_hi;
        if (lo >= hi) continue;
        NodeDev &ch = nodes[nd.child0 + k];
        double a[14];
#pragma unroll
        for (int i = 0; i < 14; i++) a[i] = 0;
        cov_accumulate<W>(px, py, pz, pw, lo, hi, ch.mean[0], ch.mean[1], ch.mean[2], nd.kquad, a);
        block_sum<14>(a, sm);
        if (threadIdx.x == 0)
            for (int q = 0; q < 7; q++) { unsafeAtomicAdd(&ch.acc[blockIdx.x & (kSlots - 1)][q][0], a[2 * q]); unsafeAtomicAdd(&ch.acc[blockIdx.x & (kSlots - 1)][q][1], a[2 * q + 1]); }
    }
}

template <bool W>
__global__ __launch_bounds__(256) void k_cov_nodes(QuantBuffers qb, const double *planar, const Tile *__restrict__ tiles, NodeDev *nodes,
                                                   const int from_end) {
    __shared__ double sm[14 * 4];
    const Tile t = tiles[from_end ? gridDim.x - 1u - blockIdx.x : blockIdx.x];
    NodeDev &nd = nodes[t.node];
    const double *px = planar ? planar : qb.buf[nd.buf], *py = px + qb.N, *pz = py + qb.N, *pw = pz + qb.N;
    double a[14];
#pragma unroll
    for (int i = 0; i < 14; i++) a[i] = 0;
    cov_accumulate<W>(px, py, pz, pw, t.start, t.start + t.count, nd.mean[0], nd.mean[1], nd.mean[2], nd.kquad, a);
// ... 201 lines not shown
```

Baseline: 3119.

## Hoist global loads above early exits and pass kmeans start centroids by kernel arg

```diff
diff --git a/patolette_amd/csrc/kmeans.h b/patolette_amd/csrc/kmeans.h
--- a/patolette_amd/csrc/kmeans.h
+++ b/patolette_amd/csrc/kmeans.h
@@ -33,7 +33,8 @@
 void kmeans_gather_slice(const double *d_planar, size_t n_local, bool weighted, const int *d_perm, size_t nx, size_t begin,
                          KMeansWork &w, hipStream_t s);
 struct KmSums { double bound_x, bound_w; };
+constexpr int kKmStartMax = 256;
 void kmeans_iterate(KMeansWork &w, size_t nx, int k, bool weighted, int niter, hipStream_t s, size_t expect_longest = 0,
-                    const KmSums *sums = nullptr);
+                    const KmSums *sums = nullptr, const float *start = nullptr);
 
 }
diff --git a/patolette_amd/csrc/kmeans.hip b/patolette_amd/csrc/kmeans.hip
--- a/patolette_amd/csrc/kmeans.hip
+++ b/patolette_amd/csrc/kmeans.hip
@@ -48,10 +48,22 @@
     __hip_atomic_store(pp + 6, r.w, __ATOMIC_RELAXED, __HIP_MEMORY_SCOPE_AGENT);
 }
 constexpr int kKmFlagWords = 2 + 256;
-__global__ void k_km_prep(const float *__restrict__ cent, int k, float4 *c4, unsigned int *flags) {
+__global__ void k_km_prep(const float *__restrict__ cent, int k, float4 *c4, unsigned int *flags, unsigned int *prev, size_t nprev) {
     int j = blockIdx.x * blockDim.x + threadIdx.x;
     if (j < k) km_store_c4(c4, k, j, cent[3 * j], cent[3 * j + 1], cent[3 * j + 2]);
     if (flags && j < kKmFlagWords) flags[j] = j == 0 ? 0u : 1u;
+    for (size_t q = (size_t)j; q < nprev; q += (size_t)gridDim.x * blockDim.x) prev[q] = 0u;
+}
+struct KmStart { float v[3 * kKmStartMax]; };
+__global__ void k_km_prep_start(const KmStart start, float *cent, int k, float4 *c4, unsigned int *flags, unsigned int *prev, size_t nprev) {
+    int j = blockIdx.x * blockDim.x + threadIdx.x;
+    if (j < k) {
+        const float v0 = start.v[3 * j], v1 = start.v[3 * j + 1], v2 = start.v[3 * j + 2];
+        cent[3 * j] = v0; cent[3 * j + 1] = v1; cent[3 * j + 2] = v2;
+        km_store_c4(c4, k, j, v0, v1, v2);
+    }
+    if (flags && j < kKmFlagWords) flags[j] = j == 0 ? 0u : 1u;
+    for (size_t q = (size_t)j; q < nprev; q += (size_t)gridDim.x * blockDim.x) prev[q] = 0u;
 }
 
 typedef float f4_t __attribute__((ext_vector_type(4)));
@@ -1589,24 +1601,28 @@
 __global__ __launch_bounds__(1024) void k_km_assign_sort(KmSamples s, size_t nx, const float4 *__restrict__ c4, int k, const bool weighted,
                                                          float4 *__restrict__ sorted_rec, unsigned short *__restrict__ offs,
                                                          unsigned char *__restrict__ prev, unsigned int *flags) {
-    if (flags[0]) return;
     __shared__ unsigned char cnt[16][256];
     __shared__ unsigned short stepbase[16][256];
     __shared__ unsigned int wsum[16];
     __shared__ float4 c4s[256];
     const int lane = threadIdx.x & 63, step = threadIdx.x >> 6;
     KM_TRACE0(0, 0);
-    for (int i = threadIdx.x; i < 16 * 256 / 4; i += 1024) reinterpret_cast<unsigned int *>(&cnt[0][0])[i] = 0u;
-    if ((int)threadIdx.x < k) c4s[threadIdx.x] = c4[threadIdx.x];
+    const size_t blk0 = (size_t)blockIdx.x * kKmSortBlock;
+    const size_t i = blk0 + (size_t)step * 64 + lane;
+    const bool v = i < nx;
+    const unsigned fixed = flags[0];
+    float4 tab = make_float4(0.f, 0.f, 0.f, 0.f);
+    if ((int)threadIdx.x < k) tab = c4[threadIdx.x];
+    float4 rec = make_float4(0.f, 0.f, 0.f, 0.f);
+    int old = 0;
+    if (v) { rec.x = s.x[i]; rec.y = s.y[i]; rec.z = s.z[i]; if (weighted) rec.w = s.w[i]; old = prev[i]; }
+    if (fixed) return;
+    for (int q = threadIdx.x; q < 16 * 256 / 4; q += 1024) reinterpret_cast<unsigned int *>(&cnt[0][0])[q] = 0u;
+    if ((int)threadIdx.x < k) c4s[threadIdx.x] = tab;
     __syncthreads();
     KM_TRACE0(0, 1);
     const scalar_c4_t t4 = (scalar_c4_t)(unsigned long long)c4;
     const scalar_c8_t t8 = (scalar_c8_t)(unsigned long long)(c4 + k);
-    const size_t blk0 = (size_t)blockIdx.x * kKmSortBlock;
-    const size_t i = blk0 + (size_t)step * 64 + lane;
-    const bool v = i < nx;
-    float4 rec = make_float4(0.f, 0.f, 0.f, 0.f);
-    if (v) { rec.x = s.x[i]; rec.y = s.y[i]; rec.z = s.z[i]; if (weighted) rec.w = s.w[i]; }
 #ifdef PAMD_KM_TRACE
     asm volatile("s_waitcnt vmcnt(0)" ::: "memory");
     KM_TRACE0(0, 2);
@@ -1615,7 +1631,6 @@
     int a = km_assign_min3(rec.x, rec.y, rec.z, t4, t8, c4s, k);
     if (!v) a = 0;
     if (v) {
-        const int old = prev[i];
         if (old != a) { prev[i] = (unsigned char)a; flags[1 + old] = 1u; flags[1 + a] = 1u; }
     }
     const unsigned long long m = match_mask(a, 8, __ballot(v));
@@ -1655,7 +1670,12 @@
 __global__ __launch_bounds__(256) void k_km_update_lists(const float4 *__restrict__ sorted_rec, const unsigned short *__restrict__ offs,
                                                         unsigned long long nx, int k, float *cent, float *hassign, float4 *c4,
                                                         unsigned int *ticket, DevMT *mt, unsigned int *flags) {
-    if (flags[0]) return;
+    const unsigned long long nblocks_all = (nx + kKmSortBlock - 1) / kKmSortBlock;
+    const unsigned fixed = flags[0], dirty = flags[1 + blockIdx.x];
+    unsigned off_pair = 0;
+    if (threadIdx.x < nblocks_all) __builtin_memcpy(&off_pair, offs + (size_t)threadIdx.x * 257 + blockIdx.x, sizeof(off_pair));
+    asm volatile("" :: "s"(fixed), "s"(dirty));
+    if (fixed) return;
     __shared__ float4 stage[4][2][64];
     extern __shared__ __attribute__((aligned(16))) float members[];
     __shared__ float res[4];
@@ -1686,16 +1706,25 @@
         else if (wid == 2) acc = km_chain_over<W, 2>(rec, n, stage[2], lane, acc);
         else if (W) acc = km_chain_over<W, 3>(rec, n, stage[3], lane, acc);
     };
-    const bool clean = flags[1 + kidx] == 0u;
-    const unsigned long long nblocks = clean ? 0ULL : (nx + kKmSortBlock - 1) / kKmSortBlock;
+    const bool clean = dirty == 0u;
+    const unsigned long long nblocks = clean ? 0ULL : nblocks_all;
     for (unsigned long long c0 = 0; c0 < nblocks; c0 += 256) {
         const unsigned long long b = c0 + threadIdx.x;
         unsigned o0 = 0, nb = 0;
-        if (b < nblocks) { o0 = offs[b * 257 + kidx]; nb = (unsigned)offs[b * 257 + kidx + 1] - o0; }
+        if (b < nblocks) {
+            if (c0 == 0) { o0 = off_pair & 0xFFFFu; nb = (off_pair >> 16) - o0; }
+            else { o0 = offs[b * 257 + kidx]; nb = (unsigned)offs[b * 257 + kidx + 1] - o0; }
+        }
+        constexpr unsigned kLongRun = 32;
+        constexpr int kPre = 16;
+        static_assert(kLongRun % kPre == 0, "a short run is its first kPre records and whole batches of kPre");
+        const bool is_long = nb > kLongRun;
+        const float4 *src = sorted_rec + b * kKmSortBlock + o0;
+        float4 pre[kPre];
+#pragma unroll
+        for (int u = 0; u < kPre; u++) pre[u] = (!is_long && (unsigned)u < nb) ? src[u] : make_float4(0.f, 0.f, 0.f, 0.f);
         unsigned chunk_total = 0;
         const unsigned excl = block_scan_incl_u32(nb, wsum, &chunk_total) - nb;
-        constexpr unsigned kLongRun = 32;
-        const bool is_long = nb > kLongRun;
         if (threadIdx.x == 0) n_long = 0u;
         __syncthreads();
         if (is_long) { const unsigned e = atomicAdd(&n_long, 1u); long_src[e] = (unsigned)(b * kKmSortBlock) + o0; long_lo[e] = excl; long_nb[e] = nb; }
@@ -1706,13 +1735,15 @@
             const unsigned take = min((unsigned)kKmDirectCap - fill, chunk_total - done);
             if (!is_long) {
                 const unsigned lo = max(excl, done), hi = min(excl + nb, done + take);
-                const float4 *src = sorted_rec + b * kKmSortBlock + o0;
-                for (unsigned q = lo; q < hi; q += 4) {
-                    float4 r4[4];
-#pragma unroll
-                    for (int u = 0; u < 4; u++) r4[u] = q + u < hi ? src[q + u - excl] : make_float4(0.f, 0.f, 0.f, 0.f);
-#pragma unroll
-                    for (int u = 0; u < 4; u++) if (q + u < hi) { const unsigned i = fill + q + u - done; mx[i] = r4[u].x; my[i] = r4[u].y; mz[i] = r4[u].z; mw[i] = r4[u].w; }
+                auto put = [&](const unsigned q, const float4 r) { const unsigned i = fill + q - done; mx[i] = r.x; my[i] = r.y; mz[i] = r.z; mw[i] = r.w; };
+#pragma unroll
+                for (int u = 0; u < kPre; u++) { const unsigned q = excl + u; if (q >= lo && q < hi) put(q, pre[u]); }
+                for (unsigned r0 = kPre; r0 < nb; r0 += kPre) {
+                    float4 r4[kPre];
+#pragma unroll
+                    for (int u = 0; u < kPre; u++) { const unsigned q = excl + r0 + u; r4[u] = (q >= lo && q < hi) ? src[r0 + u] : make_float4(0.f, 0.f, 0.f, 0.f); }
+#pragma unroll
+                    for (int u = 0; u < kPre; u++) { const unsigned q = excl + r0 + u; if (q >= lo && q < hi) put(q, r4[u]); }
                 }
             }
             if (nl) {
@@ -1870,7 +1901,8 @@
     HIP_CHECK(hipGetLastError());
 }
 
-void kmeans_iterate(KMeansWork &w, size_t nx, int k, bool weighted, int niter, hipStream_t s, size_t expect_longest, const KmSums *sums) {
+void kmeans_iterate(KMeansWork &w, size_t nx, int k, bool weighted, int niter, hipStream_t s, size_t expect_longest, const KmSums *sums,
+                    const float *start) {
     KmSamples ks{w.sx.p, w.sy.p, w.sz.p, w.sw.p};
     KmFix fix{};
     int ablocks = 1;
@@ -1930,7 +1962,6 @@
         HIP_CHECK(hipFuncSetAttribute((const void *)k_km_update<false, false>, hipFuncAttributeMaxDynamicSharedMemorySize, 4 * 4096 * 4));
     });
     if (!w.mt_seeded) { hipLaunchKernelGGL(k_km_mt_seed, 1, 1, 0, s, w.mt.p); w.mt_seeded = true; }
-    { KTIME("k_km_prep", s, 28.0 * k); hipLaunchKernelGGL(k_km_prep, (std::max(k, kKmFlagWords) + 255) / 256, 256, 0, s, w.cent.p, k, w.c4.p, w.flags.p); }
     const size_t lut_min = getenv("PAMD_KM_LUT_MIN") ? (size_t)atoll(getenv("PAMD_KM_LUT_MIN")) : ((size_t)1 << 21);
     const bool use_lut = nx >= lut_min && k >= 16 && k <= 256;
     const size_t g64_min = getenv("PAMD_KM_G64_MIN") ? (size_t)atoll(getenv("PAMD_KM_G64_MIN")) : ((size_t)1 << 23);
@@ -1950,12 +1981,21 @@
     const size_t list_longest = getenv("PAMD_KM_LIST_LONGEST") ? (size_t)atoll(getenv("PAMD_KM_LIST_LONGEST")) : (size_t)16384;
     const bool use_direct = !sums && !use_lut && k <= 256 && nx <= direct_max && nx < ((size_t)1 << 32) && expect_longest < list_longest;
     if (use_direct) {
-        HIP_CHECK(hipMemsetAsync(w.assign.p, 0, nx, s));
         static PerDeviceOnce attr4;
         attr4.once([&] {
             HIP_CHECK(hipFuncSetAttribute((const void *)k_km_update_lists<true>, hipFuncAttributeMaxDynamicSharedMemorySize, kKmDirectCap * 20));
             HIP_CHECK(hipFuncSetAttribute((const void *)k_km_update_lists<false>, hipFuncAttributeMaxDynamicSharedMemorySize, kKmDirectCap * 20));
         });
+    }
+    {
+        const size_t pwords = use_direct ? (nx + 3) / 4 : 0;
+        const int pblocks = (int)std::min<size_t>(std::max<size_t>((std::max(k, kKmFlagWords) + 255) / 256, ceil_div(pwords, (size_t)1024)), 64);
+        KTIME("k_km_prep", s, 28.0 * k + 4.0 * pwords);
+        if (start && k <= kKmStartMax) {
+            KmStart st{};
+            std::memcpy(st.v, start, 3 * (size_t)k * sizeof(float));
+            hipLaunchKernelGGL(k_km_prep_start, pblocks, 256, 0, s, st, w.cent.p, k, w.c4.p, w.flags.p, (unsigned int *)w.assign.p, pwords);
+        } else hipLaunchKernelGGL(k_km_prep, pblocks, 256, 0, s, w.cent.p, k, w.c4.p, w.flags.p, (unsigned int *)w.assign.p, pwords);
     }
     const bool use_mid = use_lut && G == 64 && k % 8 == 0;
     if (use_mid) w.mid.reserve(32 * 32 * 32);
diff --git a/patolette_amd/csrc/pipeline.hip b/patolette_amd/csrc/pipeline.hip
--- a/patolette_amd/csrc/pipeline.hip
+++ b/patolette_amd/csrc/pipeline.hip
@@ -235,10 +235,15 @@
 __global__ __launch_bounds__(256) void k_lq_children(NodeDev *nodes, LqCtl *c, const int call, int init_kbase,
                                                      const int init_first, int init_nnodes, const int init_K, const GqOut *gq) {
     const bool init = init_kbase > 0;
-    if (!init && c->h.done) return;
+    const int wave = (int)blockIdx.x * 4 + (int)(threadIdx.x >> 6), lane = threadIdx.x & 63;
+    int done_in = 0, ncids_in = 0, id_in = 0, parent_in = -1, nleaves_in = 0;
+    if (!init) {
+        done_in = c->h.done; ncids_in = c->ncids[call & 1]; nleaves_in = c->nleaves;
+        if (wave < 2 * kLqRoundCap) { id_in = c->cids[call & 1][wave]; parent_in = c->round_ids[wave >> 1]; }
+    }
+    if (!init && done_in) return;
     if (init && gq) { init_kbase = gq->kbase; init_nnodes = init_first + init_kbase; }
-    const int ncids = init ? init_kbase : c->ncids[call & 1];
-    const int wave = (int)blockIdx.x * 4 + (int)(threadIdx.x >> 6), lane = threadIdx.x & 63;
+    const int ncids = init ? init_kbase : ncids_in;
     if (init && blockIdx.x == 0 && threadIdx.x == 0) {
         c->K = init_K; c->M = init_K - init_kbase; c->nleaves = 0; c->ncids[0] = init_kbase; c->dyn = RoundDyn{0, 0, 0, 0};
         c->h.done = 0; c->h.error = 0; c->h.rounds = 0; c->h.nnodes = init_nnodes; c->h.neval = 0; c->h.split_evals = 0ULL; c->h.split_px = 0ULL;
@@ -249,10 +254,12 @@
     }
     if (init && gq && gq->error) return;
     if (wave >= ncids) return;
-    const int id = init ? init_first + wave : c->cids[call & 1][wave];
+    const int id = init ? init_first + wave : id_in;
     if (init && lane == 0) c->cids[0][wave] = id;
     NodeDev &d = nodes[id];
     const double *acc = &d.acc[0][0][0];
+    const unsigned long long gn = d.gn;
+    const double sw = d.sw, mean0 = d.mean[0], mean1 = d.mean[1], mean2 = d.mean[2];
     double sum = 0;
     if (lane < 14) {
         double v[kSlots];
@@ -268,8 +275,7 @@
         cov[q] = __hiloint2double(__builtin_amdgcn_readlane(__double2hiint(pair), 2 * q), __builtin_amdgcn_readlane(__double2loint(pair), 2 * q));
     if (lane != 0) return;
     double ub = cov[6];
-    const bool single = d.gn <= 1ULL;
-    const double sw = d.sw;
+    const bool single = gn <= 1ULL;
     if (single || !(sw > 0)) ub = 0;
     else {
         double c6[6];
@@ -280,9 +286,9 @@
     for (int q = 0; q < 6; q++) d.cov6[q] = cov[q];
     d.dist = cov[6]; d.ub = ub; d.axis_state = 0;
     c->nrec[id] = LqRec{single ? 0.0 : ub, -1, single ? 1 : 0};
-    c->nparent[id] = init ? -1 : c->round_ids[wave >> 1];
-    c->ncen[id] = LqCen{{d.mean[0], d.mean[1], d.mean[2]}, (double)d.gn};
-    c->leaves[(init ? 0 : c->nleaves) + wave] = id;
+    c->nparent[id] = init ? -1 : parent_in;
+    c->ncen[id] = LqCen{{mean0, mean1, mean2}, (double)gn};
+    c->leaves[(init ? 0 : nleaves_in) + wave] = id;
 }
 
 __device__ __forceinline__ int block_excl_scan_256(const int v, int *sw , int &total) {
@@ -297,19 +303,37 @@
     return base + inc - v;
 }
 
+__device__ __forceinline__ void block_excl_scan2_256(const int a, const int b, int *sw, int &pa, int &pb, int &ta, int &tb) {
+    const int lane = threadIdx.x & 63, wid = threadIdx.x >> 6;
+    const int ia = (int)wave_scan_incl_u32((unsigned)a), ib = (int)wave_scan_incl_u32((unsigned)b);
+    __syncthreads();
+    if (lane == 63) { sw[wid] = ia; sw[4 + wid] = ib; }
+    __syncthreads();
+    int ba = 0, bb = 0;
+    for (int w = 0; w < wid; w++) { ba += sw[w]; bb += sw[4 + w]; }
+    ta = sw[0] + sw[1] + sw[2] + sw[3]; tb = sw[4] + sw[5] + sw[6] + sw[7];
+    pa = ba + ia - a; pb = bb + ib - b;
+}
+
 __device__ __forceinline__ unsigned long long lq_key(const double p) { return p > 0.0 ? (unsigned long long)__double_as_longlong(p) : 0ULL; }
 
 constexpr double kSpecBeta = 0.25;
 
 __global__ __launch_bounds__(256) void k_lq_select(NodeDev *nodes, LqCtl *c, const int call, const int e_lin, const int e_quad) {
-    if (c->h.done) return;
     const int tid = threadIdx.x, lane = tid & 63;
     const int cur = call & 1, nxt = cur ^ 1;
+    const int done_in = c->h.done;
     const int ncids = c->ncids[cur];
+    const int w_in = ((int)blockIdx.x - 1) * 4 + (tid >> 6);
+    int cid_in = 0;
+    if (blockIdx.x > 0 && w_in < 2 * kLqRoundCap) cid_in = c->cids[cur][w_in];
+    int M_in = 0, nn_in = 0, nr_prev_in = 0, neval_in = 0, nleaves_in = 0, rounds_in = 0;
+    if (blockIdx.x == 0) { M_in = c->M; nn_in = c->h.nnodes; nr_prev_in = c->dyn.nr; neval_in = c->h.neval; nleaves_in = c->nleaves; rounds_in = c->h.rounds; }
+    if (done_in) return;
     if (blockIdx.x > 0) {
-        const int w = ((int)blockIdx.x - 1) * 4 + (tid >> 6);
+        const int w = w_in;
         if (w >= ncids) return;
-        NodeDev &d = nodes[c->cids[cur][w]];
+        NodeDev &d = nodes[cid_in];
         if (d.gn <= 1ULL || !(d.sw > 0)) { if (lane == 0) d.axis_state = d.gn <= 1ULL ? 0 : -1; return; }
         double c6[6];
         for (int q = 0; q < 6; q++) c6[q] = d.cov6[q] / d.sw;
@@ -322,14 +346,14 @@
         }
         return;
     }
-    __shared__ int sw[5];
+    __shared__ int sw[8];
     __shared__ unsigned int hist[256];
     __shared__ unsigned long long s_prefix, s_px;
     __shared__ int s_need, s_neval, s_first;
     __shared__ double s_umax[4];
-    const int M = c->M;
-    const int nn = c->h.nnodes;
-    const int nr_prev = c->dyn.nr;
+    const int M = M_in;
+    const int nn = nn_in;
+    const int nr_prev = nr_prev_in;
     int evald = 0;
     for (int i = tid; i < nr_prev; i += 256) {
         const int id = c->round_ids[i];
@@ -347,21 +371,56 @@
     __syncthreads();
     if (evald) atomicAdd(&s_neval, evald);
     __syncthreads();
-    const int neval = c->h.neval + s_neval;
+    const int neval = neval_in + s_neval;
+    const int nleaves = nleaves_in + ncids;
+    auto leaf_prio = [&](const int id) -> double {
+        const LqRec r = c->nrec[id];
+        const int par = c->nparent[id];
+        if (r.kn || (par >= 0 && nodes[par].axis_state < 0)) return -1.0;
+        const double pp = par < 0 ? INFINITY : c->np[par];
+        return r.val < pp ? r.val : pp;
+    };
+    constexpr int kLeafKeep = 4;
+    int leaf_id[kLeafKeep]; double leaf_pr[kLeafKeep];
+#pragma unroll
+    for (int j = 0; j < kLeafKeep; j++) {
+        const int i = tid + 256 * j;
+        leaf_id[j] = -1; leaf_pr[j] = -1.0;
+        if (i < nleaves) { leaf_id[j] = c->leaves[i]; leaf_pr[j] = leaf_prio(leaf_id[j]); }
+    }
     double tau = 0.0;
     if (neval >= M && M > 0) {
         unsigned long long prefix = 0ULL;
         int need = M;
+        constexpr int kKeep = 4;
+        unsigned long long kept[kKeep];
+        unsigned kept_ok = 0u;
         for (int pass = 0; pass < 3; pass++) {
             const int shift = 56 - 8 * pass;
             hist[tid] = 0u;
             __syncthreads();
-            for (int i = tid; i < nn; i += 256) {
+            auto tally = [&](const unsigned long long k) {
+                if (pass == 0 || (k >> (shift + 8)) == (prefix >> (shift + 8))) atomicAdd(&hist[(k >> shift) & 255ULL], 1u);
+            };
+            if (pass == 0) {
+                LqRec r[kKeep]; double pr[kKeep];
+#pragma unroll
+                for (int j = 0; j < kKeep; j++) {
+                    const int i = tid + 256 * j;
+                    r[j] = LqRec{0.0, -1, 0}; pr[j] = 0.0;
+                    if (i < nn) { r[j] = c->nrec[i]; pr[j] = c->np[i]; }
+                }
+#pragma unroll
+                for (int j = 0; j < kKeep; j++) {
+                    kept[j] = lq_key(pr[j]);
+                    if (r[j].kn && r[j].left >= 0) kept_ok |= 1u << j;
+                }
+            }
+#pragma unroll
+            for (int j = 0; j < kKeep; j++) if (kept_ok & (1u << j)) tally(kept[j]);
+            for (int i = tid + 256 * kKeep; i < nn; i += 256) {
                 const LqRec r = c->nrec[i];
-                if (r.kn && r.left >= 0) {
-                    const unsigned long long k = lq_key(c->np[i]);
-                    if (pass == 0 || (k >> (shift + 8)) == (prefix >> (shift + 8))) atomicAdd(&hist[(k >> shift) & 255ULL], 1u);
-                }
+                if (r.kn && r.left >= 0) tally(lq_key(c->np[i]));
             }
             __syncthreads();
             {
@@ -382,18 +441,12 @@
         tau = __longlong_as_double((long long)prefix);
     }
     const double thr = fmax(kDelta, tau * (1.0 - 1e-9));
-    const int nleaves = c->nleaves + ncids;
-    auto leaf_prio = [&](const int id) -> double {
-        const LqRec r = c->nrec[id];
-        const int par = c->nparent[id];
-        if (r.kn || (par >= 0 && nodes[par].axis_state < 0)) return -1.0;
-        const double pp = par < 0 ? INFINITY : c->np[par];
-        return r.val < pp ? r.val : pp;
-    };
     double thr2 = thr;
-    if (c->h.rounds < 48) {
+    if (rounds_in < 48) {
         double u = -1.0;
-        for (int i = tid; i < nleaves; i += 256) { const double pr = leaf_prio(c->leaves[i]); u = pr > u ? pr : u; }
+#pragma unroll
+        for (int j = 0; j < kLeafKeep; j++) u = leaf_pr[j] > u ? leaf_pr[j] : u;
+        for (int i = tid + 256 * kLeafKeep; i < nleaves; i += 256) { const double pr = leaf_prio(c->leaves[i]); u = pr > u ? pr : u; }
 #pragma unroll
         for (int o = 32; o > 0; o >>= 1) { const double v = __shfl_xor(u, o, 64); u = v > u ? v : u; }
         __syncthreads();
@@ -407,15 +460,21 @@
         const int i = base + tid;
         int id = -1, sel = 0, keep = 0;
         if (i < nleaves) {
-            id = c->leaves[i];
-            const double pr = leaf_prio(id);
+            double pr;
+            if (base < 256 * kLeafKeep) {
+                id = leaf_id[0]; pr = leaf_pr[0];
+#pragma unroll
+                for (int j = 1; j < kLeafKeep; j++) if (base == 256 * j) { id = leaf_id[j]; pr = leaf_pr[j]; }
+            } else { id = c->leaves[i]; pr = leaf_prio(id); }
             sel = pr >= thr2 ? 1 : 0;
             keep = (!sel && pr >= thr) ? 1 : 0;
         }
-        int tsel, tkeep;
-        const int psel = block_excl_scan_256(sel, sw, tsel);
-        if (nr + tsel > kLqRoundCap && sel && nr + psel >= kLqRoundCap) { sel = 0; keep = 1; }
-        const int pkeep = block_excl_scan_256(keep, sw, tkeep);
+        int tsel, tkeep, psel, pkeep;
+        block_excl_scan2_256(sel, keep, sw, psel, pkeep, tsel, tkeep);
+        if (nr + tsel > kLqRoundCap) {
+            if (sel && nr + psel >= kLqRoundCap) { sel = 0; keep = 1; }
+            pkeep = block_excl_scan_256(keep, sw, tkeep);
+        }
         if (sel) c->round_ids[nr + psel] = id;
         __syncthreads();
         if (keep) c->leaves[nkeep + pkeep] = id;
@@ -448,9 +507,8 @@
             n = d.n;
             ta = (int)((n + kTileA - 1) / kTileA); tp = (int)((n + kTileP - 1) / kTileP);
         }
-        int totA, totP;
-        const int pa = block_excl_scan_256(ta, sw, totA);
-        const int pp = block_excl_scan_256(tp, sw, totP);
+        int totA, totP, pa, pp;
+        block_excl_scan2_256(ta, tp, sw, pa, pp, totA, totP);
         if (r < nr) { c->tA0[r] = runA + pa; c->tP0[r] = runP + pp; }
         runA += totA; runP += totP;
         for (int o = 32; o > 0; o >>= 1) n += __shfl_xor(n, o, 64);
@@ -458,7 +516,7 @@
     }
     __syncthreads();
     if (tid == 0) {
-        const int round = c->h.rounds;
+        const int round = rounds_in;
         const unsigned long long rpx = s_px;
         c->tA0[nr] = runA; c->tP0[nr] = runP;
         c->nleaves = nkeep; c->ncids[nxt] = 2 * nr;
@@ -1898,9 +1956,12 @@
         } else {
             kmeans_gather(E.cvt.p, N, weighted, dperm, nx, E.km, s);
             E.h_cent.reserve(3 * k);
-            std::memcpy(E.h_cent.p, cent.data(), 3 * k * sizeof(float));
-            HIP_CHECK(hipMemcpyAsync(E.km.cent.p, E.h_cent.p, 3 * k * sizeof(float), hipMemcpyHostToDevice, s));
-            kmeans_iterate(E.km, nx, (int)k, weighted, niter, s, expect_longest(nx), sums);
+            const bool by_arg = k <= (size_t)kKmStartMax;
+            if (!by_arg) {
+                std::memcpy(E.h_cent.p, cent.data(), 3 * k * sizeof(float));
+                HIP_CHECK(hipMemcpyAsync(E.km.cent.p, E.h_cent.p, 3 * k * sizeof(float), hipMemcpyHostToDevice, s));
+            }
+            kmeans_iterate(E.km, nx, (int)k, weighted, niter, s, expect_longest(nx), sums, by_arg ? cent.data() : nullptr);
             HIP_CHECK(hipMemcpyAsync(E.h_cent.p, E.km.cent.p, 3 * k * sizeof(float), hipMemcpyDeviceToHost, s));
             E.sync();
             std::memcpy(cent.data(), E.h_cent.p, 3 * k * sizeof(float));
diff --git a/patolette_amd/csrc/quant.hip b/patolette_amd/csrc/quant.hip
--- a/patolette_amd/csrc/quant.hip
+++ b/patolette_amd/csrc/quant.hip
@@ -584,11 +584,13 @@
 __global__ __launch_bounds__(1024) void k_scan(const int *__restrict__ round_nodes, const int *__restrict__ node_tile0, NodeDev *nodes,
                                               const unsigned int *__restrict__ tilecnt, unsigned long long *tileoff,
                                               const RoundDyn *__restrict__ dyn) {
-    if (dyn && (int)blockIdx.x >= dyn->nr) return;
+    const int nr_in = dyn ? dyn->nr : 0, node_in = round_nodes[blockIdx.x];
+    const int t0 = node_tile0[blockIdx.x], t1 = node_tile0[blockIdx.x + 1];
+    asm volatile("" :: "s"(nr_in), "s"(node_in), "s"(t0), "s"(t1));
+    if (dyn && (int)blockIdx.x >= nr_in) return;
     __shared__ unsigned long long su[16];
     __shared__ unsigned long long total;
-    NodeDev &nd = nodes[round_nodes[blockIdx.x]];
-    const int t0 = node_tile0[blockIdx.x], t1 = node_tile0[blockIdx.x + 1];
+    NodeDev &nd = nodes[node_in];
     const int C = (t1 - t0 + (int)blockDim.x - 1) / (int)blockDim.x;
     const int a = t0 + (int)threadIdx.x * C, b = min(t1, a + C);
     unsigned long long base = nd.begin;
@@ -597,7 +599,12 @@
         __shared__ unsigned long long sv[2 * 16];
         __shared__ unsigned long long tot2[2];
         unsigned long long sum[2] = {0, 0};
-        for (int g = a; g < b; g += 8) {
+        uint2 vk[8];
+#pragma unroll
+        for (int q = 0; q < 8; q++) vk[q] = a + q < b ? *reinterpret_cast<const uint2 *>(tilecnt + (size_t)(a + q) * kMaxChildren) : make_uint2(0u, 0u);
+#pragma unroll
+        for (int q = 0; q < 8; q++) { sum[0] += vk[q].x; sum[1] += vk[q].y; }
+        for (int g = a + 8; g < b; g += 8) {
             uint2 v[8];
 #pragma unroll
             for (int q = 0; q < 8; q++) v[q] = g + q < b ? *reinterpret_cast<const uint2 *>(tilecnt + (size_t)(g + q) * kMaxChildren) : make_uint2(0u, 0u);
@@ -610,7 +617,12 @@
         __syncthreads();
         const unsigned long long base1 = base + tot2[0];
         unsigned long long run0 = base + inc[0] - sum[0], run1 = base1 + inc[1] - sum[1];
-        for (int g = a; g < b; g += 8) {
+#pragma unroll
+        for (int q = 0; q < 8; q++) {
+            if (a + q < b) *reinterpret_cast<ulonglong2 *>(tileoff + (size_t)(a + q) * kMaxChildren) = make_ulonglong2(run0, run1);
+            run0 += vk[q].x; run1 += vk[q].y;
+        }
+        for (int g = a + 8; g < b; g += 8) {
             uint2 v[8];
 #pragma unroll
             for (int q = 0; q < 8; q++) v[q] = g + q < b ? *reinterpret_cast<const uint2 *>(tilecnt + (size_t)(g + q) * kMaxChildren) : make_uint2(0u, 0u);
```

New measurement: 3120 (median of 3 runs). About the same (+0.0%).
